# GeekAlexis/FastMOT

Measured on AMD Instinct MI355X. Metric: end-to-end tracker FPS @1080p/50 dets, higher is better.
Workload: dtype f16

## Files before the change

### fastmot_amd/csrc/common.h

```cpp
#pragma once
#include <hip/hip_runtime.h>
#include <atomic>
#include <cstdarg>
#include <cstdint>
#include <cstdio>
#include <cstring>
#include <string>
#include <vector>
#include "../../include/fastmot_hip.h"
#ifdef FM_DIAG
#include "../../include/fastmot_hip_diag.h"
#endif

#define FM_ERR_HIP (-1)
#define FM_ERR_ARG (-2)
#define FM_ERR_STATE (-3)

void fm_set_error(const char* fmt, ...);

#define FM_HIP(call)                                                                        \
    do {                                                                                    \
        hipError_t e_ = (call);                                                             \
        if (e_ != hipSuccess) {                                                             \
            fm_set_error("%s:%d %s -> %s", __FILE__, __LINE__, #call, hipGetErrorString(e_)); \
            return FM_ERR_HIP;                                                              \
        }                                                                                   \
    } while (0)

#define FM_CHECK_ARG(cond)                                                     \
    do {                                                                       \
        if (!(cond)) {                                                         \
            fm_set_error("%s:%d bad argument: %s", __FILE__, __LINE__, #cond); \
            return FM_ERR_ARG;                                                 \
        }                                                                      \
    } while (0)

bool fm_lap_host(const double* cost, int nr, int nc, long rs, long cs, int32_t* col4row_out);
#define FM_ZERO_COPY_TRACKS (ctx->opt_zero_copy_tracks)

struct DevBuf {
    void* d = nullptr;
    void* h = nullptr;
    size_t cap = 0;
    bool pinned_mirror = true;
    int reserve(size_t bytes) {
        if (bytes <= cap) return 0;
        size_t ncap = cap ? cap : 4096;
        while (ncap < bytes) ncap *= 2;
        if (d) (void)hipFree(d);
        if (h) (void)hipHostFree(h);
        d = h = nullptr;
        cap = 0;
        FM_HIP(hipMalloc(&d, ncap));
        if (pinned_mirror) FM_HIP(hipHostMalloc(&h, ncap, hipHostMallocDefault));
        cap = ncap;
        return 0;
    }
    void release() {
        if (d) (void)hipFree(d);
        if (h) (void)hipHostFree(h);
        d = h = nullptr;
        cap = 0;
    }
    template <typename T> T* dev() { return reinterpret_cast<T*>(d); }
    template <typename T> T* host() { return reinterpret_cast<T*>(h); }
};

struct KFConst {
    double F_pos_self;
    double F_pos_other;
    double F_vel;
    double q_pp, q_pv, q_vv;
    double std_factor_acc, std_offset_acc;
    double fac_det[2], fac_klt[2], min_det[2], min_klt[2];
    double init_pos_weight, init_vel_weight;
};

struct NetState;
struct DetState;
struct ExtState;
struct FlowState;
struct EncState;
struct OvlState;
struct YuvState;
struct GalleryState;
constexpr int FM_GALLERY_CHANNELS = 2;

struct fm_ctx {
    int device = 0;
    int opt_zero_copy_tracks = 2048;
    int opt_host_lap_elems = 262144;
    int opt_use_graphs = 1;
    int opt_fused_input = 1;
    int opt_net_timing = 0;
    int opt_nms_general = 0;
    int opt_lk_variant = 0;
    void* predict_worker = nullptr;
    hipStream_t s_main = nullptr;
    hipStream_t s_det = nullptr;
    hipStream_t s_up = nullptr;
    hipStream_t s_ext = nullptr;
    hipStream_t s_ext_x[FM_MAX_EXTRA_EXTRACTORS] = {};
    hipEvent_t ev_ext_in = nullptr, ev_ext_x_done[FM_MAX_EXTRA_EXTRACTORS] = {};
    hipStream_t s_flow = nullptr;
    hipStream_t s_flow2 = nullptr;
    hipEvent_t ev_pyr = nullptr;
    bool pyr_pending = false;
    hipEvent_t ev_prep = nullptr, ev_bg = nullptr;
    hipEvent_t ev_feat = nullptr;
    hipEvent_t ev_ext_net = nullptr;
    hipEvent_t ev_ext_done = nullptr;
    hipEvent_t ev_pair = nullptr;
    bool ext_net_recorded = false;
    size_t as_in_bytes = 0;
    bool as_in_device = true;
    bool as_mirror = false;

    int slot_cap = 0;
    double* mean = nullptr;
    double* cov = nullptr;
    int feat_dim = 512;
    float* feat_sum = nullptr;
    float* feat_avg = nullptr;
    int32_t* feat_cnt = nullptr;
    KFConst kf{};
    bool kf_set = false;
    double frame_rect[4] = {0, 0, 0, 0};

    float* emb = nullptr;
    float* emb_host = nullptr;
    int emb_cap = 0;
    int emb_n = 0;

    int as_nT = 0, as_nD = 0, as_metric = 0;
    size_t as_off[6] = {0, 0, 0, 0, 0, 0};
    DevBuf as_in;
    DevBuf as_pair;
    DevBuf as_stage_in;
    DevBuf as_cost;
    DevBuf as_work;
    DevBuf as_out;
    DevBuf io0, io1;
    DevBuf occ_in, occ_out;
    DevBuf feat_in;

    int frame_w = 0, frame_h = 0, ring_size = 0;
    uint8_t* frame_cur = nullptr;
    uint8_t* frame_own = nullptr;
    uint8_t* frame_own2 = nullptr;
    uint8_t* frame_next = nullptr;
    uint8_t* frame_pinned2 = nullptr;
    hipEvent_t ev_next_upload = nullptr;
    uint8_t* frame_ahead[FM_MAX_DET_BATCH + 1] = {};
    uint8_t* frame_up[FM_MAX_DET_BATCH + 1] = {};
    uint8_t* frame_up_pinned[FM_MAX_DET_BATCH + 1] = {};
    hipEvent_t ev_up[FM_MAX_DET_BATCH + 1] = {};
    uint8_t* frame_ring = nullptr;
    uint8_t* frame_pinned = nullptr;

    DetState* det = nullptr;
    ExtState* ext = nullptr;
    NetState* det_net = nullptr;
    NetState* ext_net = nullptr;
    NetState* ext_net_x[FM_MAX_EXTRA_EXTRACTORS] = {};
    FlowState* flow = nullptr;
    EncState* enc = nullptr;
    OvlState* ovl = nullptr;
    YuvState* yuv = nullptr;
    GalleryState* gallery[2] = {nullptr, nullptr};

    std::vector<hipEvent_t> trace_ev;
    std::vector<int> trace_tag;
    std::atomic<int> trace_n{0};
    std::atomic<bool> trace_on{false};
    std::atomic<int> trace_busy{0};
    hipEvent_t trace_base = nullptr;

    uint8_t* frame_nv12[FM_MAX_DET_BATCH + 2] = {};
    uint8_t* frame_planar[FM_MAX_DET_BATCH + 2] = {};
    uint8_t* frame_packed[FM_MAX_DET_BATCH + 2] = {};
    uint8_t* frame_bayer[FM_MAX_DET_BATCH + 2] = {};

    uint8_t* frame_jpeg[FM_MAX_DET_BATCH + 2] = {};
    uint8_t* frame_jpeg_pinned[FM_MAX_DET_BATCH + 2] = {};
    hipEvent_t ev_jpeg[FM_MAX_DET_BATCH + 2] = {};

    struct SrcStage {
        uint8_t* bgr = nullptr;
        uint8_t* dev = nullptr;
        uint8_t* pinned = nullptr;
        size_t bgr_cap = 0, dev_cap = 0, pinned_cap = 0;
        hipEvent_t ev = nullptr;
    };
    SrcStage frame_src[FM_MAX_DET_BATCH + 2];

    int32_t* remap_xy = nullptr;
    int remap_sw = 0, remap_sh = 0;
    uint32_t remap_border = 0;
};

inline void fm_trace_mark(fm_ctx* ctx, hipStream_t s, int tag) {
    if (!ctx->trace_on.load(std::memory_order_acquire)) return;
    ctx->trace_busy.fetch_add(1);
    if (ctx->trace_on.load()) {
        const int i = ctx->trace_n.fetch_add(1);
        if (i < (int)ctx->trace_ev.size()) {
            ctx->trace_tag[i] = tag;
            (void)hipEventRecord(ctx->trace_ev[i], s);
        }
    }
    ctx->trace_busy.fetch_sub(1);
}

int fm_ensure_slots(fm_ctx* ctx, int max_slot_plus_1);
int fm_nv12_to_bgr(const uint8_t* nv12, uint8_t* bgr, int w, int h, int matrix, hipStream_t s);
inline bool fm_yuv_chroma_dims(int w, int h, int chroma, int* cw, int* ch) {
    switch (chroma) {
    case FM_YUV_420: *cw = (w + 1) / 2, *ch = (h + 1) / 2; return true;
    case FM_YUV_422: *cw = (w + 1) / 2, *ch = h; return true;
    case FM_YUV_444: *cw = w, *ch = h; return true;
    case FM_YUV_MONO: *cw = *ch = 0; return true;
    }
    return false;
}
int fm_planar_to_bgr(const uint8_t* planes, uint8_t* bgr, int w, int h, int chroma, int matrix, hipStream_t s);
inline size_t fm_packed_row_bytes(int w, int format) {
    if (format < FM_PACKED_RGB || format > FM_PACKED_YVYU) return 0;
    if (format >= FM_PACKED_YUY2) return 4 * (size_t)((w + 1) / 2);
    return (size_t)w * (format <= FM_PACKED_BGR ? 3 : 4);
}
inline bool fm_packed_matrix_ok(int matrix) {
    return matrix == FM_PACKED_BT601 || matrix == FM_PACKED_BT709 || matrix == FM_PACKED_BT601_FULL || matrix == FM_PACKED_BT709_FULL;
}
int fm_packed_to_bgr(const uint8_t* src, uint8_t* bgr, int w, int h, int format, int matrix, hipStream_t s);
inline int fm_bayer_sample_bytes(int depth) {
    return depth == 8 ? 1 : depth == 10 || depth == 12 || depth == 14 || depth == 16 ? 2 : 0;
}
inline bool fm_bayer_gain_ok(int gain) { return gain >= 1 && gain <= 4096; }
int fm_bayer_to_bgr(const uint8_t* src, uint8_t* bgr, int w, int h, int pattern, int depth, int method, int black, int gain_r, int gain_g,
                    int gain_b, hipStream_t s);
void fm_yuv_free(fm_ctx* ctx);
int fm_resize_bgr(const uint8_t* src, int sw, int sh, uint8_t* dst, int dw, int dh, hipStream_t s);
int fm_remap_bgr(const uint8_t* src, int sw, int sh, const int32_t* xy, uint8_t* dst, int dw, int dh, uint32_t border, hipStream_t s);
void fm_frame_src_free(fm_ctx* ctx);
void fm_frame_remap_free(fm_ctx* ctx);
int fm_jpeg_to_bgr(const uint8_t* stage, uint8_t* bgr, const struct fm_jpeg_info* info, hipStream_t s);
int fm_jpeg_layout(int width, int height, int ncomp, int hsamp0, int vsamp0, struct fm_jpeg_info* out);
size_t fm_jpeg_sample_offset(long long coef_count);
void fm_ext_invalidate_export(fm_ctx* ctx);
void fm_predict_worker_free(fm_ctx* ctx);
void fm_gallery_free(fm_ctx* ctx);
void fm_jpegenc_free(fm_ctx* ctx);
int fm_jpegenc_ensure(fm_ctx* ctx, int mcus_x, int mcus_y);
hipStream_t fm_jpegenc_stream(fm_ctx* ctx);
int fm_jpegenc_encode_device(fm_ctx* ctx, const uint8_t* src, int width, int height, int quality, uint8_t* out, size_t capacity,
                             size_t* length);
void fm_overlay_free(fm_ctx* ctx);
```

### fastmot_amd/csrc/ctx.hip

```cpp
#include "common.h"
void convd_set_cfg(int code);
#include <sched.h>
#include <cstring>
#include <cstdlib>
#include <cmath>

static thread_local char g_err[1024] = "";

void fm_set_error(const char* fmt, ...) {
    va_list ap;
    va_start(ap, fmt);
    vsnprintf(g_err, sizeof(g_err), fmt, ap);
    va_end(ap);
}

extern "C" const char* fm_last_error(void) { return g_err; }

extern "C" int fm_ctx_set_option(fm_ctx* ctx, const char* key, int value) {
    FM_CHECK_ARG(ctx && key && value >= 0);
    if (!strcmp(key, "zero_copy_tracks")) ctx->opt_zero_copy_tracks = value;
    else if (!strcmp(key, "host_lap_elems")) ctx->opt_host_lap_elems = value;
    else if (!strcmp(key, "use_graphs")) ctx->opt_use_graphs = value;
    else if (!strcmp(key, "convd_cfg")) convd_set_cfg(value);
    else if (!strcmp(key, "nms_path")) {
        ctx->opt_nms_general = value != 0;
    }
    else if (!strcmp(key, "fused_input")) ctx->opt_fused_input = value != 0;
    else if (!strcmp(key, "net_timing")) ctx->opt_net_timing = value;
    else if (!strcmp(key, "lk_variant")) {
#ifndef FM_DIAG
        if (value != 0) {
            fm_set_error("option 'lk_variant' needs a diagnostic build of the library (-DFM_DIAG)");
            return FM_ERR_ARG;
        }
#endif
        ctx->opt_lk_variant = value;
    }
    else {
        fm_set_error("unknown option '%s'", key);
        return FM_ERR_ARG;
    }
    return 0;
}

extern "C" int fm_trace_start(fm_ctx* ctx, int cap, int64_t* host_ns) {
    FM_CHECK_ARG(ctx && cap > 0 && host_ns && !ctx->trace_on.load() && ctx->trace_ev.empty());
    FM_HIP(hipDeviceSynchronize());
    std::vector<hipEvent_t> evs(cap);
    for (auto& e : evs) FM_HIP(hipEventCreate(&e));
    if (!ctx->trace_base) FM_HIP(hipEventCreate(&ctx->trace_base));
    FM_HIP(hipEventRecord(ctx->trace_base, ctx->s_main));
    FM_HIP(hipEventSynchronize(ctx->trace_base));
    timespec ts;
    clock_gettime(CLOCK_MONOTONIC, &ts);
    *host_ns = (int64_t)ts.tv_sec * 1000000000ll + ts.tv_nsec;
    ctx->trace_tag.assign(cap, 0);
    ctx->trace_n = 0;
    ctx->trace_ev = std::move(evs);
    ctx->trace_on.store(true, std::memory_order_release);
    return 0;
}

extern "C" int fm_trace_read(fm_ctx* ctx, int cap, int32_t* tags, float* ms, int* n) {
    FM_CHECK_ARG(ctx && tags && ms && n);
    ctx->trace_on.store(false, std::memory_order_seq_cst);
    while (ctx->trace_busy.load(std::memory_order_seq_cst) > 0) sched_yield();
    FM_HIP(hipDeviceSynchronize());
    std::vector<hipEvent_t> evs = std::move(ctx->trace_ev);
    ctx->trace_ev.clear();
    int k = ctx->trace_n.load();
    if (k > (int)evs.size()) k = (int)evs.size();
    if (k > cap) k = cap;
    for (int i = 0; i < k; ++i) {
        tags[i] = ctx->trace_tag[i];
        FM_HIP(hipEventElapsedTime(&ms[i], ctx->trace_base, evs[i]));
    }
    *n = k;
    for (auto& e : evs) (void)hipEventDestroy(e);
    return 0;
}

extern "C" int fm_ctx_bind_thread(fm_ctx* ctx) {
    FM_CHECK_ARG(ctx);
    FM_HIP(hipSetDevice(ctx->device));
    return 0;
}

extern "C" int fm_device_pci_bus_id(int device, char* buf, int buflen) {
    FM_CHECK_ARG(buf && buflen >= 16);
    FM_HIP(hipDeviceGetPCIBusId(buf, buflen, device));
    return 0;
}

extern "C" int fm_device_count(void) {
    int n = 0;
    FM_HIP(hipGetDeviceCount(&n));
    return n;
}

void fm_net_free(NetState* n);
void fm_det_free(DetState* d);
void fm_ext_free(ExtState* e);
void fm_flow_free(FlowState* f);

extern "C" int fm_ctx_create(int device, fm_ctx** out) {
    FM_CHECK_ARG(out != nullptr);
    int n = 0;
    FM_HIP(hipGetDeviceCount(&n));
    if (device < 0 || device >= n) {
        fm_set_error("device %d out of range (%d visible)", device, n);
        return FM_ERR_ARG;
    }
    FM_HIP(hipSetDevice(device));
    fm_ctx* ctx = new fm_ctx();
    ctx->device = device;
    if (const char* e = getenv("FASTMOT_ZERO_COPY")) ctx->opt_zero_copy_tracks = atoi(e);
    if (const char* e = getenv("FASTMOT_HOST_LAP")) ctx->opt_host_lap_elems = atoi(e);
    if (const char* e = getenv("FASTMOT_GRAPHS")) ctx->opt_use_graphs = atoi(e);
    if (const char* e = getenv("FASTMOT_FUSED_INPUT")) ctx->opt_fused_input = atoi(e) != 0;
    int prio_lo = 0, prio_hi = 0;
    FM_HIP(hipDeviceGetStreamPriorityRange(&prio_lo, &prio_hi));
    const int prio_det = prio_lo, prio_ext = prio_hi;
    FM_HIP(hipStreamCreateWithPriority(&ctx->s_main, hipStreamNonBlocking, prio_hi));
    FM_HIP(hipStreamCreateWithPriority(&ctx->s_det, hipStreamNonBlocking, prio_det));
    FM_HIP(hipStreamCreateWithPriority(&ctx->s_up, hipStreamNonBlocking, prio_lo));
    FM_HIP(hipStreamCreateWithPriority(&ctx->s_ext, hipStreamNonBlocking, prio_ext));
    FM_HIP(hipEventCreateWithFlags(&ctx->ev_ext_in, hipEventDisableTiming));
    for (int i = 0; i < FM_MAX_EXTRA_EXTRACTORS; ++i) {
        FM_HIP(hipStreamCreateWithPriority(&ctx->s_ext_x[i], hipStreamNonBlocking, prio_hi));
        FM_HIP(hipEventCreateWithFlags(&ctx->ev_ext_x_done[i], hipEventDisableTiming));
    }
    FM_HIP(hipStreamCreateWithPriority(&ctx->s_flow, hipStreamNonBlocking, prio_hi));
    FM_HIP(hipStreamCreateWithPriority(&ctx->s_flow2, hipStreamNonBlocking, prio_hi));
    FM_HIP(hipEventCreateWithFlags(&ctx->ev_pyr, hipEventDisableTiming));
    FM_HIP(hipEventCreateWithFlags(&ctx->ev_prep, hipEventDisableTiming));
    FM_HIP(hipEventCreateWithFlags(&ctx->ev_bg, hipEventDisableTiming));
    FM_HIP(hipEventCreateWithFlags(&ctx->ev_feat, hipEventDisableTiming));
    FM_HIP(hipEventCreateWithFlags(&ctx->ev_ext_net, hipEventDisableTiming));
    FM_HIP(hipEventCreateWithFlags(&ctx->ev_pair, hipEventDisableTiming));
    FM_HIP(hipEventCreateWithFlags(&ctx->ev_ext_done, hipEventDisableTiming));
    int rc = fm_ensure_slots(ctx, 1024);
    if (rc) return rc;
    *out = ctx;
    return 0;
}

extern "C" int fm_ctx_destroy(fm_ctx* ctx) {
    if (!ctx) return 0;
    (void)hipSetDevice(ctx->device);
    fm_predict_worker_free(ctx);
    fm_gallery_free(ctx);
    (void)hipDeviceSynchronize();
    if (ctx->det) fm_det_free(ctx->det);
    if (ctx->ext) fm_ext_free(ctx->ext);
    for (void* p : {(void*)ctx->frame_own, (void*)ctx->frame_own2, (void*)ctx->frame_ring})
        if (p) (void)hipFree(p);
    if (ctx->frame_pinned) (void)hipHostFree(ctx->frame_pinned);
    if (ctx->frame_pinned2) (void)hipHostFree(ctx->frame_pinned2);
    for (int k = 2; k <= FM_MAX_DET_BATCH; ++k) {
        if (ctx->frame_up[k]) (void)hipFree(ctx->frame_up[k]);
        if (ctx->frame_up_pinned[k]) (void)hipHostFree(ctx->frame_up_pinned[k]);
        if (ctx->ev_up[k]) (void)hipEventDestroy(ctx->ev_up[k]);
    }
    for (uint8_t* p : ctx->frame_nv12)
        if (p) (void)hipFree(p);
    for (uint8_t* p : ctx->frame_planar)
        if (p) (void)hipFree(p);
    for (uint8_t* p : ctx->frame_packed)
        if (p) (void)hipFree(p);
    for (uint8_t* p : ctx->frame_bayer)
        if (p) (void)hipFree(p);
    for (uint8_t* p : ctx->frame_jpeg)
        if (p) (void)hipFree(p);
    for (uint8_t* p : ctx->frame_jpeg_pinned)
        if (p) (void)hipHostFree(p);
    for (hipEvent_t e : ctx->ev_jpeg)
        if (e) (void)hipEventDestroy(e);
    fm_frame_src_free(ctx);
    fm_frame_remap_free(ctx);
    fm_overlay_free(ctx);
    fm_yuv_free(ctx);
    fm_jpegenc_free(ctx);
    if (ctx->det_net) fm_net_free(ctx->det_net);
    if (ctx->ext_net) fm_net_free(ctx->ext_net);
    for (NetState* x : ctx->ext_net_x)
        if (x) fm_net_free(x);
    if (ctx->flow) fm_flow_free(ctx->flow);
    for (void* p : {(void*)ctx->mean, (void*)ctx->cov, (void*)ctx->feat_sum, (void*)ctx->feat_avg,
                    (void*)ctx->feat_cnt, (void*)ctx->emb})
        if (p) (void)hipFree(p);
    if (ctx->emb_host) (void)hipHostFree(ctx->emb_host);
    for (DevBuf* b : {&ctx->as_in, &ctx->as_pair, &ctx->as_stage_in, &ctx->as_cost, &ctx->as_work,
                      &ctx->as_out, &ctx->io0, &ctx->io1, &ctx->feat_in, &ctx->occ_in, &ctx->occ_out})
        b->release();
    for (hipStream_t s : {ctx->s_main, ctx->s_det, ctx->s_up, ctx->s_ext, ctx->s_flow, ctx->s_flow2})
        if (s) (void)hipStreamDestroy(s);
    for (hipEvent_t e : {ctx->ev_feat, ctx->ev_ext_in, ctx->ev_pyr, ctx->ev_prep, ctx->ev_bg, ctx->ev_ext_net, ctx->ev_pair, ctx->ev_ext_done})
        if (e) (void)hipEventDestroy(e);
    for (int i = 0; i < FM_MAX_EXTRA_EXTRACTORS; ++i) {
        if (ctx->s_ext_x[i]) (void)hipStreamDestroy(ctx->s_ext_x[i]);
        if (ctx->ev_ext_x_done[i]) (void)hipEventDestroy(ctx->ev_ext_x_done[i]);
    }
    delete ctx;
    return 0;
}

extern "C" int fm_ctx_synchronize(fm_ctx* ctx) {
    FM_CHECK_ARG(ctx);
    FM_HIP(hipStreamSynchronize(ctx->s_main));
    FM_HIP(hipStreamSynchronize(ctx->s_det));
    FM_HIP(hipStreamSynchronize(ctx->s_up));
    FM_HIP(hipStreamSynchronize(ctx->s_ext));
    for (hipStream_t x : ctx->s_ext_x) FM_HIP(hipStreamSynchronize(x));
    FM_HIP(hipStreamSynchronize(ctx->s_flow));
    FM_HIP(hipStreamSynchronize(ctx->s_flow2));
    return 0;
}

extern "C" int fm_device_info(fm_ctx* ctx, char* buf, int buflen) {
    FM_CHECK_ARG(ctx && buf && buflen > 0);
    hipDeviceProp_t p;
    FM_HIP(hipGetDeviceProperties(&p, ctx->device));
    snprintf(buf, buflen, "%s:%s:%d:%d:%zu", p.name, p.gcnArchName, p.multiProcessorCount,
             p.clockRate / 1000, (size_t)p.totalGlobalMem);
    return 0;
}

template <typename T>
static int grow(T** ptr, size_t old_elems, size_t new_elems, hipStream_t s, bool zero) {
    T* np_ = nullptr;
    FM_HIP(hipMalloc(&np_, new_elems * sizeof(T)));
    if (zero) FM_HIP(hipMemsetAsync(np_, 0, new_elems * sizeof(T), s));
    if (*ptr && old_elems)
        FM_HIP(hipMemcpyAsync(np_, *ptr, old_elems * sizeof(T), hipMemcpyDeviceToDevice, s));
    FM_HIP(hipStreamSynchronize(s));
    if (*ptr) FM_HIP(hipFree(*ptr));
    *ptr = np_;
    return 0;
}

int fm_ensure_slots(fm_ctx* ctx, int need) {
    if (need <= ctx->slot_cap) return 0;
    int ncap = ctx->slot_cap ? ctx->slot_cap : 1024;
    while (ncap < need) ncap *= 2;
    size_t o = ctx->slot_cap, n = ncap;
    int rc;
    if ((rc = grow(&ctx->mean, o * 8, n * 8, ctx->s_main, true))) return rc;
    if ((rc = grow(&ctx->cov, o * 64, n * 64, ctx->s_main, true))) return rc;
    if ((rc = grow(&ctx->feat_sum, o * ctx->feat_dim, n * ctx->feat_dim, ctx->s_main, true))) return rc;
    if ((rc = grow(&ctx->feat_avg, o * ctx->feat_dim, n * ctx->feat_dim, ctx->s_main, true))) return rc;
    if ((rc = grow(&ctx->feat_cnt, o, n, ctx->s_main, true))) return rc;
    ctx->slot_cap = ncap;
    return 0;
}

extern "C" int fm_kf_configure(fm_ctx* ctx, const fm_kf_params* p) {
    FM_CHECK_ARG(ctx && p);
    FM_CHECK_ARG(p->dt > 0 && p->vel_half_life > 0);
    KFConst& k = ctx->kf;
    const double dt = p->dt;
    k.F_pos_self = p->vel_coupling * dt;
    k.F_pos_other = (1. - p->vel_coupling) * dt;
    k.F_vel = std::pow(0.5, dt / p->vel_half_life);
    k.q_pp = 0.25 * std::pow(dt, 4);
    k.q_pv = 0.5 * std::pow(dt, 3);
    k.q_vv = dt * dt;
    k.std_factor_acc = p->std_factor_acc;
    k.std_offset_acc = p->std_offset_acc;
    for (int i = 0; i < 2; ++i) {
        k.fac_det[i] = p->std_factor_det[i];
        k.fac_klt[i] = p->std_factor_klt[i];
        k.min_det[i] = p->min_std_det[i];
        k.min_klt[i] = p->min_std_klt[i];
    }
    k.init_pos_weight = p->init_pos_weight;
    k.init_vel_weight = p->init_vel_weight;
    ctx->kf_set = true;
    return 0;
}

extern "C" int fm_set_frame_rect(fm_ctx* ctx, const double tlbr[4]) {
    FM_CHECK_ARG(ctx && tlbr);
    memcpy(ctx->frame_rect, tlbr, sizeof(double) * 4);
    return 0;
}

static int max_slot(int n, const int32_t* slots) {
    int m = -1;
    for (int i = 0; i < n; ++i) {
        if (slots[i] < 0) return -2;
        if (slots[i] > m) m = slots[i];
    }
    return m;
}

extern "C" int fm_trk_get_state(fm_ctx* ctx, int n, const int32_t* slots, double* mean, double* cov) {
    FM_CHECK_ARG(ctx && n >= 0);
    if (n == 0) return 0;
    FM_CHECK_ARG(slots && mean && cov);
    int m = max_slot(n, slots);
    FM_CHECK_ARG(m >= 0 && m < ctx->slot_cap);
    FM_HIP(hipStreamSynchronize(ctx->s_main));
    for (int i = 0; i < n; ++i) {
        FM_HIP(hipMemcpy(mean + (size_t)i * 8, ctx->mean + (size_t)slots[i] * 8, 64, hipMemcpyDeviceToHost));
        FM_HIP(hipMemcpy(cov + (size_t)i * 64, ctx->cov + (size_t)slots[i] * 64, 512, hipMemcpyDeviceToHost));
    }
    return 0;
}

extern "C" int fm_trk_set_state(fm_ctx* ctx, int n, const int32_t* slots, const double* mean, const double* cov) {
    FM_CHECK_ARG(ctx && n >= 0);
    if (n == 0) return 0;
    FM_CHECK_ARG(slots && mean && cov);
    int m = max_slot(n, slots);
    FM_CHECK_ARG(m >= 0);
    int rc = fm_ensure_slots(ctx, m + 1);
    if (rc) return rc;
    FM_HIP(hipStreamSynchronize(ctx->s_main));
    for (int i = 0; i < n; ++i) {
        FM_HIP(hipMemcpy(ctx->mean + (size_t)slots[i] * 8, mean + (size_t)i * 8, 64, hipMemcpyHostToDevice));
        FM_HIP(hipMemcpy(ctx->cov + (size_t)slots[i] * 64, cov + (size_t)i * 64, 512, hipMemcpyHostToDevice));
    }
    return 0;
}

extern "C" int fm_trk_copy_state(fm_ctx* ctx, int dst, int src) {
    FM_CHECK_ARG(ctx && dst >= 0 && src >= 0 && src < ctx->slot_cap);
    int rc = fm_ensure_slots(ctx, dst + 1);
    if (rc) return rc;
    FM_HIP(hipMemcpyAsync(ctx->mean + (size_t)dst * 8, ctx->mean + (size_t)src * 8, 64,
                          hipMemcpyDeviceToDevice, ctx->s_main));
    FM_HIP(hipMemcpyAsync(ctx->cov + (size_t)dst * 64, ctx->cov + (size_t)src * 64, 512,
                          hipMemcpyDeviceToDevice, ctx->s_main));
    return 0;
}

void fm_net_drop_graphs(NetState* net);

extern "C" int fm_feat_configure(fm_ctx* ctx, int dim) {
    FM_CHECK_ARG(ctx && dim > 0 && dim % 4 == 0);
    if (dim == ctx->feat_dim) return 0;
    FM_HIP(hipStreamSynchronize(ctx->s_main));
    if (ctx->feat_sum) FM_HIP(hipFree(ctx->feat_sum));
    if (ctx->feat_avg) FM_HIP(hipFree(ctx->feat_avg));
    ctx->feat_sum = ctx->feat_avg = nullptr;
    ctx->feat_dim = dim;
    size_t n = (size_t)ctx->slot_cap * dim;
    FM_HIP(hipMalloc(&ctx->feat_sum, n * sizeof(float)));
    FM_HIP(hipMalloc(&ctx->feat_avg, n * sizeof(float)));
    FM_HIP(hipMemset(ctx->feat_sum, 0, n * sizeof(float)));
    FM_HIP(hipMemset(ctx->feat_avg, 0, n * sizeof(float)));
    FM_HIP(hipMemset(ctx->feat_cnt, 0, (size_t)ctx->slot_cap * sizeof(int32_t)));
    fm_net_drop_graphs(ctx->ext_net);
    for (NetState* x : ctx->ext_net_x) fm_net_drop_graphs(x);
    if (ctx->emb) FM_HIP(hipFree(ctx->emb));
    if (ctx->emb_host) FM_HIP(hipHostFree(ctx->emb_host));
    ctx->emb = ctx->emb_host = nullptr;
    ctx->emb_cap = ctx->emb_n = 0;
    return 0;
}

void fm_net_drop_graphs(NetState* net);

int fm_emb_reserve(fm_ctx* ctx, int n) {
    if (n <= ctx->emb_cap) return 0;
    int ncap = ctx->emb_cap ? ctx->emb_cap : 64;
    while (ncap < n) ncap *= 2;
    fm_net_drop_graphs(ctx->ext_net);
    for (NetState* x : ctx->ext_net_x) fm_net_drop_graphs(x);
    if (ctx->emb) FM_HIP(hipFree(ctx->emb));
    if (ctx->emb_host) FM_HIP(hipHostFree(ctx->emb_host));
    ctx->emb = ctx->emb_host = nullptr;
    ctx->emb_cap = 0;
    FM_HIP(hipMalloc(&ctx->emb, (size_t)ncap * ctx->feat_dim * sizeof(float)));
    FM_HIP(hipHostMalloc(&ctx->emb_host, (size_t)ncap * ctx->feat_dim * sizeof(float), hipHostMallocDefault));
    ctx->emb_cap = ncap;
    return 0;
}

extern "C" int fm_emb_upload(fm_ctx* ctx, int n, const float* emb) {
    FM_CHECK_ARG(ctx && n >= 0);
    if (emb == nullptr) {
        FM_CHECK_ARG(n <= ctx->emb_cap || n == 0);
        ctx->emb_n = n;
        return 0;
    }
    FM_HIP(hipStreamSynchronize(ctx->s_main));
    fm_ext_invalidate_export(ctx);
    ctx->ext_net_recorded = false;
    int rc = fm_emb_reserve(ctx, n);
    if (rc) return rc;
    if (n)
        FM_HIP(hipMemcpyAsync(ctx->emb, emb, (size_t)n * ctx->feat_dim * sizeof(float),
                              hipMemcpyHostToDevice, ctx->s_main));
    ctx->emb_n = n;
    return 0;
}

__global__ void feat_update_kernel(int n, const int32_t* __restrict__ slots,
                                   const int32_t* __restrict__ rows, const float* __restrict__ emb,
                                   float* __restrict__ fsum, float* __restrict__ favg,
                                   int32_t* __restrict__ fcnt, int dim) {
    const int wave = (blockIdx.x * blockDim.x + threadIdx.x) >> 6;
    const int lane = threadIdx.x & 63;
    if (wave >= n) return;
    const int slot = slots[wave];
    const float* v = emb + (size_t)rows[wave] * dim;
    float* s = fsum + (size_t)slot * dim;
    float* a = favg + (size_t)slot * dim;
    const int cnt = fcnt[slot] + 1;
    if (cnt == 1) {
        for (int k = lane; k < dim; k += 64) {
            const float x = v[k];
            s[k] = x;
            a[k] = x;
        }
    } else {
        const float div = (float)(1.0 / (double)cnt);
        float nrm = 0.f;
        for (int k = lane; k < dim; k += 64) {
            const float x = s[k] + v[k];
            s[k] = x;
// ... 134 lines not shown
```

### fastmot_amd/csrc/detect.hip

```cpp
#include "pixel_source.h"
#include "remap_pixel.h"
#include <cmath>
#include <mutex>
#include <utility>

struct DetState {
    fm_yolo_cfg cfg{};
    bool configured = false;
    int cap = 8192;
    static constexpr int NSLOT = FM_MAX_DET_BATCH + 2;
    float* cand[NSLOT] = {};
    float* sorted[NSLOT] = {};
    int32_t* counters[NSLOT] = {};
    uint64_t* mask[NSLOT] = {};
    fm_det48* dets[NSLOT] = {};
    bool used[NSLOT] = {};
    hipEvent_t ev_dec[NSLOT] = {};
    int post_pending = -1;
    int post_pending_n = 0;
    bool general_post = false;
    static constexpr int GREEDY_RETRY = 1024;
    int general_passes = 0;
    int greedy_kmax = 2048, greedy_shrink = 0;
    bool sorted_valid[NSLOT] = {};
// ... 1582 lines not shown
    fm_trace_mark(ctx, cs, 30);
    int rc = enqueue_planar(ctx, k, buf, f, ahead_pinned(ctx, k), ev, cs, false);
    if (rc) return rc;
    fm_trace_mark(ctx, cs, 31);
    if (!ev) FM_HIP(hipEventCreateWithFlags(&ev, hipEventDisableTiming));
    FM_HIP(hipEventRecord(ev, cs));
    if (ctx->det && (rc = flush_post(ctx, ctx->det))) return rc;
    ahead_frame(ctx, k) = buf;
    return 0;
}

extern "C" int fm_frame_ring_store_planar(fm_ctx* ctx, int index, const struct fm_frame_planar* f) {
    FM_CHECK_ARG(ctx && index >= 0 && index < ctx->ring_size && planar_ok(f));
    FM_CHECK_ARG(remap_takes(ctx, f->width, f->height));
    int rc = enqueue_planar(ctx, FM_MAX_DET_BATCH + 1, ctx->frame_ring + (size_t)ctx->frame_w * ctx->frame_h * 3 * index, f, nullptr,
                            nullptr, nullptr, true);
    if (rc) return rc;
    FM_HIP(hipStreamSynchronize(nullptr));
    return 0;
}

static bool packed_ok(const struct fm_frame_packed* f) {
    if (!f || f->width < 1 || f->height < 1 || f->width > FM_SRC_MAX_DIM || f->height > FM_SRC_MAX_DIM) return false;
    const size_t rb = fm_packed_row_bytes(f->width, f->format);
    return rb && fm_packed_matrix_ok(f->matrix) && f->data && f->pitch > 0 && (size_t)f->pitch >= rb;
}

static int enqueue_packed(fm_ctx* ctx, int entry, uint8_t* dst, const struct fm_frame_packed* f, hipStream_t s, bool blocking) {
    const int w = f->width, h = f->height;
    const size_t rb = fm_packed_row_bytes(w, f->format), total = rb * h, npx = (size_t)w * h;
    const bool on_size = src_on_size(ctx, w, h);
    fm_ctx::SrcStage& st = ctx->frame_src[entry];
    uint8_t* stage = nullptr;
    int rc;
    if (on_size) {
        uint8_t*& p = ctx->frame_packed[entry];
        if (!p) FM_HIP(hipMalloc(&p, npx * 4));
        stage = p;
    } else {
        if ((rc = src_reserve(st.bgr, st.bgr_cap, npx * 3 + FM_FRAME_SLACK, false, s))) return rc;
        if ((rc = src_reserve(st.dev, st.dev_cap, total, false, s))) return rc;
        stage = st.dev;
    }
    if (blocking) {
        FM_HIP(hipMemcpy2D(stage, rb, f->data, f->pitch, rb, h, hipMemcpyHostToDevice));
    } else if ((size_t)f->pitch == rb && is_pinned_range(f->data, total)) {
        FM_HIP(hipMemcpyAsync(stage, f->data, total, hipMemcpyHostToDevice, s));
    } else {
        if ((rc = src_pinned(st, total, s))) return rc;
        for (int r = 0; r < h; ++r) memcpy(st.pinned + (size_t)r * rb, f->data + (size_t)r * f->pitch, rb);
        FM_HIP(hipMemcpyAsync(stage, st.pinned, total, hipMemcpyHostToDevice, s));
        if ((rc = src_pinned_copied(st, s))) return rc;
    }
    fm_trace_mark(ctx, s, 48);
    if (on_size) return fm_packed_to_bgr(stage, dst, w, h, f->format, f->matrix, s);
    if ((rc = fm_packed_to_bgr(stage, st.bgr, w, h, f->format, f->matrix, s))) return rc;
    return enqueue_src_tail(ctx, st.bgr, w, h, dst, s);
}

extern "C" int fm_frame_upload_packed(fm_ctx* ctx, const struct fm_frame_packed* f) {
    FM_CHECK_ARG(ctx && ctx->frame_own && packed_ok(f));
    FM_CHECK_ARG(remap_takes(ctx, f->width, f->height));
    FM_HIP(hipStreamSynchronize(ctx->s_det));
    FM_HIP(hipStreamSynchronize(ctx->s_ext));
    FM_HIP(hipStreamSynchronize(ctx->s_flow));
    FM_HIP(hipStreamSynchronize(ctx->s_flow2));
    int rc = enqueue_packed(ctx, 0, ctx->frame_own, f, ctx->s_det, false);
    if (rc) return rc;
    FM_HIP(hipStreamSynchronize(ctx->s_det));
    ctx->frame_cur = ctx->frame_own;
    return 0;
}

extern "C" int fm_frame_upload_ahead_packed(fm_ctx* ctx, int k, const struct fm_frame_packed* f) {
    FM_CHECK_ARG(ctx && ctx->frame_own2 && k >= 1 && k <= FM_MAX_DET_BATCH && packed_ok(f));
    FM_CHECK_ARG(remap_takes(ctx, f->width, f->height));
    const size_t bytes = (size_t)ctx->frame_w * ctx->frame_h * 3;
    if (!ahead_buf(ctx, k)) {
        FM_HIP(hipMalloc(&ahead_buf(ctx, k), bytes + FM_FRAME_SLACK));
        FM_HIP(hipHostMalloc(&ahead_pinned(ctx, k), bytes, hipHostMallocDefault));
    }
    uint8_t* const buf = ahead_buf(ctx, k);
    hipEvent_t& ev = ahead_event(ctx, k);
    hipStream_t cs = ctx->s_ext;
    fm_trace_mark(ctx, cs, 30);
    int rc = enqueue_packed(ctx, k, buf, f, cs, false);
    if (rc) return rc;
    fm_trace_mark(ctx, cs, 31);
    if (!ev) FM_HIP(hipEventCreateWithFlags(&ev, hipEventDisableTiming));
    FM_HIP(hipEventRecord(ev, cs));
    if (ctx->det && (rc = flush_post(ctx, ctx->det))) return rc;
    ahead_frame(ctx, k) = buf;
    return 0;
}

extern "C" int fm_frame_ring_store_packed(fm_ctx* ctx, int index, const struct fm_frame_packed* f) {
    FM_CHECK_ARG(ctx && index >= 0 && index < ctx->ring_size && packed_ok(f));
    FM_CHECK_ARG(remap_takes(ctx, f->width, f->height));
    int rc = enqueue_packed(ctx, FM_MAX_DET_BATCH + 1, ctx->frame_ring + (size_t)ctx->frame_w * ctx->frame_h * 3 * index, f, nullptr, true);
    if (rc) return rc;
    FM_HIP(hipStreamSynchronize(nullptr));
    return 0;
}

static bool bayer_ok(const struct fm_frame_bayer* f) {
    if (!f || f->width < 2 || f->height < 2 || f->width > FM_SRC_MAX_DIM || f->height > FM_SRC_MAX_DIM) return false;
    const int bps = fm_bayer_sample_bytes(f->depth);
    if (!bps || f->pattern < FM_BAYER_RGGB || f->pattern > FM_BAYER_BGGR) return false;
    if (f->method != FM_BAYER_BILINEAR && f->method != FM_BAYER_MHC) return false;
    if (f->black < 0 || f->black >= (1 << f->depth)) return false;
    if (!fm_bayer_gain_ok(f->gain_r) || !fm_bayer_gain_ok(f->gain_g) || !fm_bayer_gain_ok(f->gain_b)) return false;
    return f->data && f->pitch > 0 && (size_t)f->pitch >= (size_t)f->width * bps;
}

static int enqueue_bayer(fm_ctx* ctx, int entry, uint8_t* dst, const struct fm_frame_bayer* f, hipStream_t s, bool blocking) {
    const int w = f->width, h = f->height;
    const size_t rb = (size_t)w * fm_bayer_sample_bytes(f->depth), total = rb * h, npx = (size_t)w * h;
    const bool on_size = src_on_size(ctx, w, h);
    fm_ctx::SrcStage& st = ctx->frame_src[entry];
    uint8_t* stage = nullptr;
    int rc;
    if (on_size) {
        uint8_t*& p = ctx->frame_bayer[entry];
        if (!p) FM_HIP(hipMalloc(&p, npx * 2));
        stage = p;
    } else {
        if ((rc = src_reserve(st.bgr, st.bgr_cap, npx * 3 + FM_FRAME_SLACK, false, s))) return rc;
        if ((rc = src_reserve(st.dev, st.dev_cap, total, false, s))) return rc;
        stage = st.dev;
    }
    if (blocking) {
        FM_HIP(hipMemcpy2D(stage, rb, f->data, f->pitch, rb, h, hipMemcpyHostToDevice));
    } else if ((size_t)f->pitch == rb && is_pinned_range(f->data, total)) {
        FM_HIP(hipMemcpyAsync(stage, f->data, total, hipMemcpyHostToDevice, s));
    } else {
        if ((rc = src_pinned(st, total, s))) return rc;
        for (int r = 0; r < h; ++r) memcpy(st.pinned + (size_t)r * rb, f->data + (size_t)r * f->pitch, rb);
        FM_HIP(hipMemcpyAsync(stage, st.pinned, total, hipMemcpyHostToDevice, s));
        if ((rc = src_pinned_copied(st, s))) return rc;
    }
    fm_trace_mark(ctx, s, 49);
    uint8_t* const out = on_size ? dst : st.bgr;
    if ((rc = fm_bayer_to_bgr(stage, out, w, h, f->pattern, f->depth, f->method, f->black, f->gain_r, f->gain_g, f->gain_b, s))) return rc;
    if (on_size) return 0;
    return enqueue_src_tail(ctx, st.bgr, w, h, dst, s);
}

extern "C" int fm_frame_upload_bayer(fm_ctx* ctx, const struct fm_frame_bayer* f) {
    FM_CHECK_ARG(ctx && ctx->frame_own && bayer_ok(f));
    FM_CHECK_ARG(remap_takes(ctx, f->width, f->height));
    FM_HIP(hipStreamSynchronize(ctx->s_det));
    FM_HIP(hipStreamSynchronize(ctx->s_ext));
    FM_HIP(hipStreamSynchronize(ctx->s_flow));
    FM_HIP(hipStreamSynchronize(ctx->s_flow2));
    int rc = enqueue_bayer(ctx, 0, ctx->frame_own, f, ctx->s_det, false);
    if (rc) return rc;
    FM_HIP(hipStreamSynchronize(ctx->s_det));
    ctx->frame_cur = ctx->frame_own;
    return 0;
}

extern "C" int fm_frame_upload_ahead_bayer(fm_ctx* ctx, int k, const struct fm_frame_bayer* f) {
    FM_CHECK_ARG(ctx && ctx->frame_own2 && k >= 1 && k <= FM_MAX_DET_BATCH && bayer_ok(f));
    FM_CHECK_ARG(remap_takes(ctx, f->width, f->height));
    const size_t bytes = (size_t)ctx->frame_w * ctx->frame_h * 3;
    if (!ahead_buf(ctx, k)) {
        FM_HIP(hipMalloc(&ahead_buf(ctx, k), bytes + FM_FRAME_SLACK));
        FM_HIP(hipHostMalloc(&ahead_pinned(ctx, k), bytes, hipHostMallocDefault));
    }
    uint8_t* const buf = ahead_buf(ctx, k);
    hipEvent_t& ev = ahead_event(ctx, k);
    hipStream_t cs = ctx->s_ext;
    fm_trace_mark(ctx, cs, 30);
    int rc = enqueue_bayer(ctx, k, buf, f, cs, false);
    if (rc) return rc;
    fm_trace_mark(ctx, cs, 31);
    if (!ev) FM_HIP(hipEventCreateWithFlags(&ev, hipEventDisableTiming));
    FM_HIP(hipEventRecord(ev, cs));
    if (ctx->det && (rc = flush_post(ctx, ctx->det))) return rc;
    ahead_frame(ctx, k) = buf;
    return 0;
}

extern "C" int fm_frame_ring_store_bayer(fm_ctx* ctx, int index, const struct fm_frame_bayer* f) {
    FM_CHECK_ARG(ctx && index >= 0 && index < ctx->ring_size && bayer_ok(f));
    FM_CHECK_ARG(remap_takes(ctx, f->width, f->height));
    int rc = enqueue_bayer(ctx, FM_MAX_DET_BATCH + 1, ctx->frame_ring + (size_t)ctx->frame_w * ctx->frame_h * 3 * index, f, nullptr, true);
    if (rc) return rc;
    FM_HIP(hipStreamSynchronize(nullptr));
    return 0;
}

extern "C" int fm_detect_configure(fm_ctx* ctx, const fm_yolo_cfg* cfg) {
    FM_CHECK_ARG(ctx && cfg);
    FM_CHECK_ARG(cfg->n_heads >= 0 && cfg->n_heads <= FM_MAX_HEADS && cfg->num_classes > 0 && cfg->num_classes <= 128);
    {
        long long rows = 0;
        for (int i = 0; i < cfg->n_heads; ++i) {
            FM_CHECK_ARG(cfg->n_anchors[i] > 0 && cfg->n_anchors[i] <= FM_MAX_ANCHORS && cfg->grid_w[i] > 0 && cfg->grid_h[i] > 0);
            rows += (long long)cfg->grid_w[i] * cfg->grid_h[i] * cfg->n_anchors[i];
        }
        FM_CHECK_ARG(rows < (1ll << FM_SORT_INDEX_BITS));
    }
    int rc = ensure_det(ctx);
    if (rc) return rc;
    DetState* d = ctx->det;
    FM_HIP(hipStreamSynchronize(ctx->s_det));
    FM_HIP(hipStreamSynchronize(ctx->s_up));
    d->post_pending = -1;
    d->post_pending_n = 0;
    d->rd = d->wr;
    d->pending = 0;
    d->cfg = *cfg;
    d->general_post = ctx->opt_nms_general != 0;
    if ((rc = alloc_post(d, cfg->max_candidates > 0 ? cfg->max_candidates : 8192))) return rc;
    FM_HIP(hipMemcpy(d->label_mask, cfg->label_mask, 128, hipMemcpyHostToDevice));
    d->configured = true;
    return 0;
}

static StemSrc det_source(fm_ctx* ctx, DetState* d, const uint8_t* const* frames, int n) {
    const fm_yolo_cfg& c = d->cfg;
    StemSrc src{};
    src.kind = 1; src.fw = ctx->frame_w; src.fh = ctx->frame_h;
    src.roi_x = c.roi_x; src.roi_y = c.roi_y; src.roi_w = c.roi_w; src.roi_h = c.roi_h;
    for (int i = 0; i < n; ++i) {
        src.frame[i] = frames[i];
        src.zero4[i] = d->counters[(d->wr + i) % DetState::NSLOT];
    }
    return src;
}

static int enqueue_preprocess(fm_ctx* ctx, DetState* d, NetState* net, const StemSrc& src, int n) {
    const fm_yolo_cfg& c = d->cfg;
    for (int i = 0; i < n; ++i) FM_CHECK_ARG(src.frame[i] != nullptr);
    FM_CHECK_ARG(c.input_tensor >= 0 && c.input_tensor < (int)net->tensors.size());
    const fm_tensor& t = net->tensors[c.input_tensor];
    FM_CHECK_ARG(t.h == c.in_h && t.w == c.in_w && !t.f32);
    hipLaunchKernelGGL(preprocess_kernel, dim3((c.in_w + 255) / 256, c.in_h, n), dim3(256), 0, ctx->s_det,
                       src, (f16*)net->bufs[c.input_tensor], c.in_w, c.in_h, t.c);
    FM_HIP(hipGetLastError());
    return 0;
}

extern "C" int fm_detect_preprocess_only(fm_ctx* ctx) {
    FM_CHECK_ARG(ctx && ctx->det && ctx->det->configured && ctx->det_net);
    const uint8_t* f = ctx->frame_cur;
    return enqueue_preprocess(ctx, ctx->det, ctx->det_net, det_source(ctx, ctx->det, &f, 1), 1);
}

static int detect_pass(fm_ctx* ctx, const uint8_t* const* frames, const hipEvent_t* uploads, int n);

extern "C" int fm_detect_async(fm_ctx* ctx) {
    FM_CHECK_ARG(ctx);
    const uint8_t* f = ctx->frame_cur;
    const hipEvent_t none = nullptr;
    return detect_pass(ctx, &f, &none, 1);
}

extern "C" int fm_detect_async_next(fm_ctx* ctx) {
    FM_CHECK_ARG(ctx && ctx->frame_next);
    return fm_detect_async_ahead(ctx, 1);
}

extern "C" int fm_detect_async_ahead(fm_ctx* ctx, int n) {
    FM_CHECK_ARG(ctx && ctx->det_net && n >= 1 && n <= FM_MAX_DET_BATCH);
    if (n > ctx->det_net->max_batch) {
        fm_set_error("detector look-ahead of %d frames > the detector network's max_batch %d", n, ctx->det_net->max_batch);
        return FM_ERR_ARG;
    }
    const uint8_t* frames[FM_MAX_DET_BATCH];
    hipEvent_t uploads[FM_MAX_DET_BATCH];
    for (int k = 1; k <= n; ++k) {
        frames[k - 1] = ahead_frame(ctx, k);
        if (!frames[k - 1]) {
            fm_set_error("look-ahead slot %d holds no frame (fm_frame_upload_ahead / fm_frame_ring_select_ahead)", k);
            return FM_ERR_ARG;
        }
        uploads[k - 1] = frames[k - 1] == ahead_buf(ctx, k) ? ahead_event(ctx, k) : nullptr;
    }
    return detect_pass(ctx, frames, uploads, n);
}

static int detect_pass(fm_ctx* ctx, const uint8_t* const* frames, const hipEvent_t* uploads, int n) {
    FM_CHECK_ARG(ctx && ctx->det && ctx->det->configured && ctx->det_net);
    DetState* d = ctx->det;
    NetState* net = ctx->det_net;
    const fm_yolo_cfg& c = d->cfg;
    FM_CHECK_ARG(n >= 1 && n <= FM_MAX_DET_BATCH && n <= net->max_batch);
    hipStream_t s = ctx->s_det;
    fm_trace_mark(ctx, s, 10);
    for (int i = 0; i < n; ++i)
        if (uploads[i]) FM_HIP(hipStreamWaitEvent(s, uploads[i], 0));
    int rc = acquire_slots(ctx, d, s, n);
    if (rc) return rc;
    fm_trace_mark(ctx, s, 14);
    const StemSrc src = det_source(ctx, d, frames, n);
    const bool fused = ctx->opt_fused_input && fm_net_stem_fusable(net, c.input_tensor);
    const bool timing = ctx->opt_net_timing > 0 && d->n_passes++ % ctx->opt_net_timing == 0;
    for (int i = 0; i < n; ++i) d->timed[(d->wr + i) % DetState::NSLOT] = timing && i == 0;
    if (fused) {
        if (timing) FM_HIP(hipEventRecord(d->ev0[d->wr], s));
        fm_trace_mark(ctx, s, 11);
        if ((rc = fm_net_run_stem_from(ctx, net, src, n))) return rc;
        fm_trace_mark(ctx, s, 15);
        net->first = 1;
        rc = fm_net_run_internal(ctx, FM_NET_DETECTOR, n);
        net->first = 0;
        if (rc) return rc;
    } else {
        if ((rc = enqueue_preprocess(ctx, d, net, src, n))) return rc;
        if (timing) FM_HIP(hipEventRecord(d->ev0[d->wr], s));
        fm_trace_mark(ctx, s, 11);
        if ((rc = fm_net_run_internal(ctx, FM_NET_DETECTOR, n))) return rc;
    }
    if (timing) FM_HIP(hipEventRecord(d->ev1[d->wr], s));
    fm_trace_mark(ctx, s, 12);
    FilterArgs fa = filter_args(d, d->wr);
    HeadSet hs{};
    for (int i = 0; i < n; ++i) {
        const int slot = (d->wr + i) % DetState::NSLOT;
        hs.cand[i] = d->cand[slot];
        hs.counters[i] = d->counters[slot];
    }
    int base = 0, blocks = 0;
    for (int i = 0; i < FM_MAX_HEADS + 1; ++i) hs.first_block[i] = 0x7fffffff;
    for (int i = 0; i < c.n_heads; ++i) {
        FM_CHECK_ARG(c.head_tensor[i] >= 0 && c.head_tensor[i] < (int)net->tensors.size());
        const fm_tensor& t = net->tensors[c.head_tensor[i]];
        FM_CHECK_ARG(t.f32 && t.h == c.grid_h[i] && t.w == c.grid_w[i] && c.n_anchors[i] <= FM_MAX_ANCHORS);
        HeadArgs& h = hs.h[i];
        h.data = (const float*)net->bufs[c.head_tensor[i]];
        h.cs = t.c; h.gw = c.grid_w[i]; h.gh = c.grid_h[i]; h.na = c.n_anchors[i];
        h.base_index = base;
        memcpy(h.anchors, c.anchors[i], sizeof(float) * 2 * FM_MAX_ANCHORS);
        h.scale_xy = c.scale_xy[i];
        const int cnt = h.gw * h.gh * h.na;
        hs.first_block[i] = blocks;
        blocks += (cnt + 255) / 256;
        base += cnt;
    }
    if (blocks) hipLaunchKernelGGL(decode_kernel, dim3(blocks, n), dim3(256), 0, s, hs, fa, c.in_w, c.in_h, c.new_coords);
    FM_HIP(hipGetLastError());
    fm_trace_mark(ctx, s, 13);
    return enqueue_post(ctx, d, s, n);
}

extern "C" int fm_detect_sync(fm_ctx* ctx, fm_det48* out, int cap, int* n) {
    FM_CHECK_ARG(ctx && ctx->det && ctx->det->configured && out && n);
    return collect(ctx, ctx->det, ctx->s_det, out, cap, n);
}

extern "C" int fm_filter_dets(fm_ctx* ctx, const float* rows, int n, fm_det48* out, int cap, int* n_out) {
    FM_CHECK_ARG(ctx && ctx->det && ctx->det->configured && n >= 0 && out && n_out);
    FM_CHECK_ARG(n < (1 << FM_SORT_INDEX_BITS));
    DetState* d = ctx->det;
    hipStream_t s = ctx->s_det;
    FM_HIP(hipStreamSynchronize(s));
    FM_HIP(hipStreamSynchronize(ctx->s_up));
    d->post_pending = -1;
    d->post_pending_n = 0;
    d->rd = d->wr;
    d->pending = 0;
    if (n > d->rows_cap) {
        if (d->rows_in) FM_HIP(hipFree(d->rows_in));
        d->rows_in = nullptr;
        FM_HIP(hipMalloc(&d->rows_in, sizeof(float) * 7 * (size_t)n));
        d->rows_cap = n;
    }
    if (n) FM_HIP(hipMemcpyAsync(d->rows_in, rows, sizeof(float) * 7 * (size_t)n, hipMemcpyHostToDevice, s));
    FM_HIP(hipMemsetAsync(d->counters[d->wr], 0, sizeof(int32_t) * 4, s));
    if (n) hipLaunchKernelGGL(rows_filter_kernel, dim3((n + 255) / 256), dim3(256), 0, s, d->rows_in, n, filter_args(d, d->wr));
    int rc = enqueue_post(ctx, d, s);
    if (rc) return rc;
    return collect(ctx, d, s, out, cap, n_out);
}

extern "C" int fm_detect_last_counts(fm_ctx* ctx, int* n_candidates, int* n_detections) {
    FM_CHECK_ARG(ctx && ctx->det && n_candidates && n_detections);
    const DetState* d = ctx->det;
    if (d->last < 0) {
        *n_candidates = *n_detections = 0;
        return 0;
    }
    *n_candidates = d->counters_host[d->last][0];
    *n_detections = d->counters_host[d->last][2];
    return 0;
}

extern "C" int fm_detect_raw_candidates(fm_ctx* ctx, float* rows, int cap, int* n) {
    FM_CHECK_ARG(ctx && ctx->det && rows && n);
    DetState* d = ctx->det;
    int rc_f = flush_post(ctx, d);
    if (rc_f) return rc_f;
    FM_HIP(hipStreamSynchronize(ctx->s_det));
    FM_HIP(hipStreamSynchronize(ctx->s_up));
    const int slot = (d->wr + DetState::NSLOT - 1) % DetState::NSLOT;
    int32_t cnt[4];
    FM_HIP(hipMemcpy(cnt, d->counters[slot], sizeof(cnt), hipMemcpyDeviceToHost));
    const int k = cnt[0] < d->cap ? cnt[0] : d->cap;
    FM_CHECK_ARG(k <= cap);
    FM_HIP(hipMemcpy(rows, d->sorted[slot], sizeof(float) * 8 * k, hipMemcpyDeviceToHost));
    *n = k;
    return 0;
}

extern "C" int fm_detect_net_ms(fm_ctx* ctx, float* ms) {
    FM_CHECK_ARG(ctx && ctx->det && ms && ctx->det->last >= 0);
    const int slot = ctx->det->last;
    if (!ctx->det->timed[slot]) { *ms = -1.f; return 0; }
    FM_HIP(hipEventSynchronize(ctx->det->ev1[slot]));
    FM_HIP(hipEventElapsedTime(ms, ctx->det->ev0[slot], ctx->det->ev1[slot]));
    return 0;
}
```

### fastmot_amd/csrc/extract.hip

```cpp
#include "pixel_source.h"
#include <cmath>

struct ExtState {
    int input_tensor = -1, in_w = 0, in_h = 0;
    double* boxes = nullptr;
    double* boxes_host = nullptr;
    int cap = 0;
    DevBuf emb_out;
    int exported_n = -1;
    bool mirror_export = false;
};

void fm_ext_invalidate_export(fm_ctx* ctx) {
    if (ctx->ext) ctx->ext->exported_n = -1;
}

void fm_ext_free(ExtState* e) {
    if (!e) return;
    e->emb_out.release();
    if (e->boxes) (void)hipFree(e->boxes);
    if (e->boxes_host) (void)hipHostFree(e->boxes_host);
    delete e;
}

namespace {

__global__ __launch_bounds__(256) void export_kernel(const float4* __restrict__ src, float4* __restrict__ dst, int n4) {
    for (int i = blockIdx.x * 256 + threadIdx.x; i < n4; i += gridDim.x * 256) dst[i] = src[i];
}

__global__ void crop_resize_kernel(const uint8_t* __restrict__ frame, int fw, int fh,
                                   const double* __restrict__ boxes, int n, f16* __restrict__ out,
                                   int ow, int oh, int cs) {
    const int x = blockIdx.x * blockDim.x + threadIdx.x;
    const int y = blockIdx.y, b = blockIdx.z;
    if (x >= ow) return;
    f16x8 o;
    crop_input_pixel(frame, fw, fh, boxes + (size_t)b * 4, x, y, ow, oh, o);
    *reinterpret_cast<f16x8*>(out + (((size_t)b * oh + y) * ow + x) * cs) = o;
}

}

extern "C" int fm_extract_configure(fm_ctx* ctx, int input_tensor, int in_w, int in_h) {
    FM_CHECK_ARG(ctx && ctx->ext_net && input_tensor >= 0 && input_tensor < (int)ctx->ext_net->tensors.size());
    const fm_tensor& t = ctx->ext_net->tensors[input_tensor];
    FM_CHECK_ARG(t.h == in_h && t.w == in_w && !t.f32);
    if (!ctx->ext) ctx->ext = new ExtState();
    ctx->ext->input_tensor = input_tensor;
    ctx->ext->in_w = in_w;
    ctx->ext->in_h = in_h;
    return 0;
}

int fm_emb_reserve(fm_ctx* ctx, int n);

static int export_embeddings(fm_ctx* ctx, ExtState* e, int n, hipStream_t s) {
    const size_t bytes = sizeof(float) * (size_t)n * ctx->feat_dim;
    e->exported_n = -1;
    if (ctx->emb_host) {
        e->exported_n = n;
        e->mirror_export = true;
        FM_HIP(hipEventRecord(ctx->ev_ext_done, s));
        return 0;
    }
    e->mirror_export = false;
    if (bytes > e->emb_out.cap) {
        FM_HIP(hipStreamSynchronize(s));
        int rc = e->emb_out.reserve(bytes);
        if (rc) return rc;
    }
    const int n4 = (int)(bytes / 16);
    hipLaunchKernelGGL(export_kernel, dim3((n4 + 255) / 256 < 64 ? (n4 + 255) / 256 : 64), dim3(256), 0, s,
                       (const float4*)ctx->emb, (float4*)e->emb_out.h, n4);
    FM_HIP(hipGetLastError());
    e->exported_n = n;
    FM_HIP(hipEventRecord(ctx->ev_ext_done, s));
    return 0;
}

static int front_end(fm_ctx* ctx, ExtState* e, NetState* ni, hipStream_t si, int off, int b, int cs) {
    ni->first = 0;
    if (ctx->opt_fused_input && fm_net_stem_fusable(ni, e->input_tensor)) {
        StemSrc src{};
        src.kind = 2; src.frame[0] = ctx->frame_cur; src.fw = ctx->frame_w; src.fh = ctx->frame_h;
        src.boxes = e->boxes_host + (size_t)off * 4;
        int rc = fm_net_run_stem_from(ctx, ni, src, b);
        if (rc) return rc;
        ni->first = 1;
        return 0;
    }
    hipLaunchKernelGGL(crop_resize_kernel, dim3((e->in_w + 127) / 128, e->in_h, b), dim3(128), 0, si,
                       ctx->frame_cur, ctx->frame_w, ctx->frame_h, e->boxes + (size_t)off * 4, b,
                       (f16*)ni->bufs[e->input_tensor], e->in_w, e->in_h, cs);
    FM_HIP(hipGetLastError());
    return 0;
}

extern "C" int fm_extract_async(fm_ctx* ctx, int n, const double* tlbr) {
    FM_CHECK_ARG(ctx && ctx->ext && ctx->ext_net && n >= 0 && ctx->frame_cur);
    ctx->emb_n = 0;
    ctx->ext_net_recorded = false;
    int rc_exp = 0;
    if (ctx->ext) ctx->ext->exported_n = -1;
    if (n == 0) return 0;
    FM_CHECK_ARG(tlbr);
    ExtState* e = ctx->ext;
    NetState* net = ctx->ext_net;
    hipStream_t s = ctx->s_ext;
    if (n > e->cap) {
        FM_HIP(hipStreamSynchronize(s));
        if (e->boxes) FM_HIP(hipFree(e->boxes));
        if (e->boxes_host) FM_HIP(hipHostFree(e->boxes_host));
        e->boxes = e->boxes_host = nullptr;
        int cap = e->cap ? e->cap : 64;
        while (cap < n) cap *= 2;
        FM_HIP(hipMalloc(&e->boxes, sizeof(double) * 4 * cap));
        FM_HIP(hipHostMalloc(&e->boxes_host, sizeof(double) * 4 * cap, hipHostMallocDefault));
        e->cap = cap;
    }
    if (hipEventQuery(ctx->ev_feat) != hipSuccess) {
        (void)hipGetLastError();
        FM_HIP(hipStreamWaitEvent(s, ctx->ev_feat, 0));
    }
    if (n > ctx->emb_cap) {
        FM_HIP(hipStreamSynchronize(ctx->s_main));
        FM_HIP(hipStreamSynchronize(s));
        int rc = fm_emb_reserve(ctx, n);
        if (rc) return rc;
    }
    FM_HIP(hipStreamSynchronize(s));
    memcpy(e->boxes_host, tlbr, sizeof(double) * 4 * n);
    const bool zero_copy_boxes = ctx->opt_fused_input && fm_net_stem_fusable(net, e->input_tensor);
    if (!zero_copy_boxes)
        FM_HIP(hipMemcpyAsync(e->boxes, e->boxes_host, sizeof(double) * 4 * n, hipMemcpyHostToDevice, s));
    fm_trace_mark(ctx, s, 32);
    const fm_tensor& t = net->tensors[e->input_tensor];
    int parts = 1;
    while (parts <= FM_MAX_EXTRA_EXTRACTORS && ctx->ext_net_x[parts - 1]) ++parts;
    while (parts > 1 && n < 4 * parts) --parts;
    if (parts > 1 && (n + parts - 1) / parts <= net->max_batch) {
        FM_HIP(hipEventRecord(ctx->ev_ext_in, s));
        int off = 0;
        for (int i = 0; i < parts; ++i) {
            const int b = n / parts + (i < n % parts ? 1 : 0);
            NetState* ni = i == 0 ? net : ctx->ext_net_x[i - 1];
            hipStream_t si = i == 0 ? s : ctx->s_ext_x[i - 1];
            FM_CHECK_ARG(b <= ni->max_batch);
            if (i) FM_HIP(hipStreamWaitEvent(si, ctx->ev_ext_in, 0));
            int rc = front_end(ctx, e, ni, si, off, b, t.c);
            if (rc) return rc;
            ni->emb_offset = off;
            rc = fm_net_run_internal(ctx, i == 0 ? FM_NET_EXTRACTOR : FM_NET_EXTRACTOR_B + i - 1, b);
            ni->emb_offset = 0;
            ni->first = 0;
            if (rc) return rc;
            if (i) {
                FM_HIP(hipEventRecord(ctx->ev_ext_x_done[i - 1], si));
                FM_HIP(hipStreamWaitEvent(s, ctx->ev_ext_x_done[i - 1], 0));
            }
            off += b;
        }
        FM_HIP(hipEventRecord(ctx->ev_ext_net, s));
        ctx->ext_net_recorded = true;
        if ((rc_exp = export_embeddings(ctx, e, n, s))) return rc_exp;
        fm_trace_mark(ctx, s, 33);
        ctx->emb_n = n;
        return 0;
    }
    for (int off = 0; off < n; off += net->max_batch) {
        const int b = n - off < net->max_batch ? n - off : net->max_batch;
        int rc = front_end(ctx, e, net, s, off, b, t.c);
        if (rc) return rc;
        fm_trace_mark(ctx, s, 34);
        net->emb_offset = off;
        rc = fm_net_run_internal(ctx, FM_NET_EXTRACTOR, b);
        net->emb_offset = 0;
        net->first = 0;
        if (rc) return rc;
    }
    fm_trace_mark(ctx, s, 35);
    FM_HIP(hipEventRecord(ctx->ev_ext_net, s));
    ctx->ext_net_recorded = true;
    if ((rc_exp = export_embeddings(ctx, e, n, s))) return rc_exp;
    fm_trace_mark(ctx, s, 33);
    ctx->emb_n = n;
    return 0;
}

extern "C" int fm_extract_sync(fm_ctx* ctx, int n, float* emb) {
    FM_CHECK_ARG(ctx && n >= 0 && n <= ctx->emb_cap);
    if (n == 0) {
        FM_HIP(hipStreamSynchronize(ctx->s_ext));
        return 0;
    }
    FM_CHECK_ARG(emb && ctx->ext);
    const size_t bytes = sizeof(float) * (size_t)n * ctx->feat_dim;
    if (ctx->ext->exported_n != n) {
        int rc = ctx->ext->emb_out.reserve(bytes);
        if (rc) return rc;
        FM_HIP(hipMemcpyAsync(ctx->ext->emb_out.h, ctx->emb, bytes, hipMemcpyDeviceToHost, ctx->s_ext));
        FM_HIP(hipStreamSynchronize(ctx->s_ext));
    } else {
        FM_HIP(hipEventSynchronize(ctx->ev_ext_done));
        if (ctx->ext->mirror_export) {
            memcpy(emb, ctx->emb_host, bytes);
            return 0;
        }
    }
    memcpy(emb, ctx->ext->emb_out.h, bytes);
    return 0;
}

extern "C" int fm_extract_read_input(fm_ctx* ctx, int n, float* out) {
    FM_CHECK_ARG(ctx && ctx->ext && ctx->ext_net && n > 0 && n <= ctx->ext_net->max_batch && out);
    ExtState* e = ctx->ext;
    NetState* net = ctx->ext_net;
    const fm_tensor& t = net->tensors[e->input_tensor];
    if (ctx->opt_fused_input && fm_net_stem_fusable(net, e->input_tensor)) {
        FM_CHECK_ARG(ctx->frame_cur && n <= e->cap);
        hipLaunchKernelGGL(crop_resize_kernel, dim3((e->in_w + 127) / 128, e->in_h, n), dim3(128), 0, ctx->s_ext,
                           ctx->frame_cur, ctx->frame_w, ctx->frame_h, e->boxes_host, n, (f16*)net->bufs[e->input_tensor],
                           e->in_w, e->in_h, t.c);
        FM_HIP(hipGetLastError());
    }
    FM_HIP(hipStreamSynchronize(ctx->s_ext));
    std::vector<f16> tmp((size_t)n * t.h * t.w * t.c);
    FM_HIP(hipMemcpy(tmp.data(), net->bufs[e->input_tensor], tmp.size() * 2, hipMemcpyDeviceToHost));
    for (size_t p = 0; p < (size_t)n * t.h * t.w; ++p)
        for (int c = 0; c < 3; ++c) out[p * 3 + c] = (float)tmp[p * t.c + c];
    return 0;
}
```

### fastmot_amd/csrc/net.h

```cpp
#pragma once
#include "common.h"
#include <hip/hip_fp16.h>

typedef _Float16 f16;
typedef f16 f16x8 __attribute__((ext_vector_type(8)));
typedef f16 f16x4 __attribute__((ext_vector_type(4)));
typedef float f32x16 __attribute__((ext_vector_type(16)));
typedef float f32x4 __attribute__((ext_vector_type(4)));

enum { ACT_LINEAR = 0, ACT_LEAKY = 1, ACT_MISH = 2, ACT_RELU = 3, ACT_LOGISTIC = 4, ACT_SWISH = 5 };
enum { RES_NONE = 0, RES_AFTER_ACT = 1, RES_BEFORE_ACT = 2 };

struct ConvParams {
    const f16* in;  int in_cs, in_coff;
    const f16* w;
    const float* bias;
    f16* out;       int out_cs, out_coff;
    float* out32;
    const f16* res; int res_cs, res_coff;
    int N, H, W, Cin, Ho, Wo, Cout, KH, KW, stride, pad;
    int K, Kpad, P;
    int cout_store;
    int act, res_mode;
    int grid_p, grid_c, grid_z, weight_major;
    int up;
    int batch_inv;
};

int launch_conv(const ConvParams& p, float* ws, size_t ws_floats, hipStream_t s);

struct NetState {
    int which = 0, max_batch = 0;
    std::vector<fm_tensor> tensors;
    std::vector<void*> bufs;
    std::vector<fm_layer> layers;
    char* weights = nullptr;
    size_t weight_bytes = 0;
    float* gates = nullptr;
    int n_gates = 0, gate_c = 0;
    hipStream_t stream = nullptr;
    char* arena = nullptr;
    float* ws = nullptr;
    size_t ws_floats = 0;
    std::vector<std::pair<long, hipGraphExec_t>> graphs;
    bool use_graphs = true;
    int emb_offset = 0;
    int batch_offset = 0;
    int first = 0;
};

NetState* fm_net_get(fm_ctx* ctx, int which);
int fm_net_run_internal(fm_ctx* ctx, int which, int batch);

__device__ __forceinline__ void unpack8(const uint4& v, float* f) {
    const f16x8 h = *reinterpret_cast<const f16x8*>(&v);
#pragma unroll
    for (int e = 0; e < 8; ++e) f[e] = (float)h[e];
}
__device__ __forceinline__ uint4 pack8(const float* f) {
    f16x8 h;
#pragma unroll
    for (int e = 0; e < 8; ++e) h[e] = (f16)f[e];
    return *reinterpret_cast<const uint4*>(&h);
}

__device__ __forceinline__ int idiv_small(int i, int d, float inv) {
    (void)d;
    return (int)(((float)i + 0.5f) * inv);
}

template <int HI>
__device__ __forceinline__ float fma_mix_h(uint32_t packed, float k, float acc) {
    float d;
    if constexpr (HI) asm("v_fma_mix_f32 %0, %1, %2, %3 op_sel:[1,0,0] op_sel_hi:[1,0,0]" : "=v"(d) : "v"(packed), "v"(k), "v"(acc));
    else asm("v_fma_mix_f32 %0, %1, %2, %3 op_sel:[0,0,0] op_sel_hi:[1,0,0]" : "=v"(d) : "v"(packed), "v"(k), "v"(acc));
    return d;
}
template <int HI>
__device__ __forceinline__ float fma_mix_hh(uint32_t packed, uint32_t kpacked, float acc) {
    float d;
    if constexpr (HI) asm("v_fma_mix_f32 %0, %1, %2, %3 op_sel:[1,1,0] op_sel_hi:[1,1,0]" : "=v"(d) : "v"(packed), "v"(kpacked), "v"(acc));
    else asm("v_fma_mix_f32 %0, %1, %2, %3 op_sel:[0,0,0] op_sel_hi:[1,1,0]" : "=v"(d) : "v"(packed), "v"(kpacked), "v"(acc));
    return d;
}
template <int N>
__device__ __forceinline__ void fma_mix_nh(const uint32_t* raw, const uint32_t* k, float* acc) {
#pragma unroll
    for (int e = 0; e < N; e += 2) {
        acc[e] = fma_mix_hh<0>(raw[e >> 1], k[e >> 1], acc[e]);
        acc[e + 1] = fma_mix_hh<1>(raw[e >> 1], k[e >> 1], acc[e + 1]);
    }
}
template <int N>
__device__ __forceinline__ void fma_mix_n(const uint32_t* raw, const float* k, float* acc) {
#pragma unroll
    for (int e = 0; e < N; e += 2) {
        acc[e] = fma_mix_h<0>(raw[e >> 1], k[e], acc[e]);
        acc[e + 1] = fma_mix_h<1>(raw[e >> 1], k[e + 1], acc[e + 1]);
    }
}

__device__ __forceinline__ void store_out(const ConvParams& p, long pix, int co, f16x4 o) {
    if (p.up == 2) {
        const int hw = p.Ho * p.Wo, rem = (int)(pix % hw);
        const size_t o00 = ((size_t)(pix / hw) * 2 * p.Ho + 2 * (rem / p.Wo)) * (2 * p.Wo) + 2 * (rem % p.Wo);
        f16* dst = p.out + o00 * p.out_cs + p.out_coff + co;
        *reinterpret_cast<f16x4*>(dst) = o;
        *reinterpret_cast<f16x4*>(dst + p.out_cs) = o;
        *reinterpret_cast<f16x4*>(dst + (size_t)2 * p.Wo * p.out_cs) = o;
        *reinterpret_cast<f16x4*>(dst + (size_t)(2 * p.Wo + 1) * p.out_cs) = o;
    } else {
        *reinterpret_cast<f16x4*>(p.out + (size_t)pix * p.out_cs + p.out_coff + co) = o;
    }
}

__device__ __forceinline__ float act_rcp(float x) { return __builtin_amdgcn_rcpf(x); }
__device__ __forceinline__ float act_leaky(float x) { return x > 0.f ? x : 0.1f * x; }
__device__ __forceinline__ float act_relu(float x) { return x > 0.f ? x : 0.f; }
__device__ __forceinline__ float act_mish(float x) {
    const float n = __expf(x);
    const float t = n * (n + 2.f);
    return x > 20.f ? x : x * (t * act_rcp(t + 2.f));
}
__device__ __forceinline__ float act_logistic(float x) { return act_rcp(1.f + __expf(-x)); }
__device__ __forceinline__ float act_swish(float x) { return x * act_rcp(1.f + __expf(-x)); }

__device__ __forceinline__ float apply_act(float x, int act) {
    switch (act) {
        case ACT_LEAKY: return act_leaky(x);
        case ACT_MISH: return act_mish(x);
        case ACT_RELU: return act_relu(x);
        case ACT_LOGISTIC: return act_logistic(x);
        case ACT_SWISH: return act_swish(x);
        default: return x;
    }
}

template <int N>
__device__ __forceinline__ void apply_act_n(float* v, int act) {
    switch (act) {
        case ACT_LEAKY:
#pragma unroll
            for (int e = 0; e < N; ++e) v[e] = act_leaky(v[e]);
            break;
        case ACT_MISH:
#pragma unroll
            for (int e = 0; e < N; ++e) v[e] = act_mish(v[e]);
            break;
        case ACT_RELU:
#pragma unroll
            for (int e = 0; e < N; ++e) v[e] = act_relu(v[e]);
            break;
        case ACT_LOGISTIC:
#pragma unroll
            for (int e = 0; e < N; ++e) v[e] = act_logistic(v[e]);
            break;
        case ACT_SWISH:
#pragma unroll
            for (int e = 0; e < N; ++e) v[e] = act_swish(v[e]);
            break;
        default: break;
    }
}
```

### fastmot_amd/csrc/net.hip

```cpp
#include "pixel_source.h"
#include <algorithm>
#include <memory>

int launch_dwconv3(const f16* in, int in_cs, int in_coff, f16* out, int out_cs, int out_coff, const f16* w,
                   const float* bias, int N, int H, int W, int C, int act, hipStream_t s);
int launch_liteconv(int G, const f16* const* in, const int* in_cs, const int* in_coff, f16* out, int out_cs,
                    int out_coff, const f16* wpw, int kpad, const f16* wdw, const float* bias, int N, int H,
                    int W, int C, int act, float* gap_out, hipStream_t s);
void liteconv_tiling(int C, int W, int H, int* th, int* tw, int* tiles_x, int* tiles_y);
int launch_litechain(const f16* in, int in_cs, int in_coff, f16* out, int out_cs, int out_coff, const f16* wpw,
                     int kpad, const f16* wdw, const float* bias, int N, int H, int W, int C, int act,
                     float* const* gap, hipStream_t s);
int launch_gated_sum(int nstreams, const f16* const* in, const int* in_cs, const int* in_coff, int N, int HW,
                     int C, int hid, const f16* w1, const float* b1, const f16* w2, const float* b2, f16* out,
                     int out_cs, int out_coff, const float* const* part, int tiles, hipStream_t s);
constexpr int GATE_SLOT_TILES = 32;
int launch_pair11(const f16* xa, int xa_cs, int xa_coff, const f16* xc, int xc_cs, int xc_coff, f16* out, int out_cs,
                  int out_coff, const f16* w1, const float* b1, const f16* w2, const float* b2, long P, int cout, int act1,
                  int act2, hipStream_t s, long p_choice);
bool pair11_supported(int cin, int mid, int extra, int cout);
int launch_ostail(const f16* in, int in_cs, int in_coff, const f16* ph, const float* pf, int N, float* out, float* raw_out,
                  float* mirror, hipStream_t s);
bool ostail_supported(int in_h, int in_w, int cin, int mid, int cout, int feat, int n_halfs, int n_floats);
int launch_stemconv(const f16* in, int in_cs, int in_coff, f16* out, int out_cs, int out_coff, const f16* w,
                    const float* bias, int N, int H, int W, int Ho, int Wo, int k, int stride, int pad, int cout,
                    int act, hipStream_t s);
int launch_spp(const f16* in, int in_cs, int in_coff, f16* out, int out_cs, int out_coff, int N, int H, int W,
               int C, hipStream_t s);
int launch_pool(const f16* in, int in_cs, int in_coff, f16* out, int out_cs, int out_coff, int N, int H,
                int W, int C, int Ho, int Wo, int k, int stride, int pad, int avg, hipStream_t s);
int launch_upsample2(const f16* in, int in_cs, int in_coff, f16* out, int out_cs, int out_coff, int N, int H,
                     int W, int C, hipStream_t s);
int launch_conv_streamed(const ConvParams& p, hipStream_t s);
int launch_convd(const ConvParams& p, hipStream_t s);
bool resblock_supported(int C, int M);
int launch_resblock(const f16* x, int x_cs, int x_coff, f16* out, int out_cs, int out_coff, const f16* w1,
                    const float* b1, const f16* w2, const float* b2, int N, int H, int W, int C, int M, int act1,
                    int act2, hipStream_t s);
int launch_add(const f16* a, int a_cs, int a_coff, const f16* b, int b_cs, int b_coff, f16* out, int out_cs,
               int out_coff, long npix, int C, hipStream_t s);
int launch_copy(const f16* in, int in_cs, int in_coff, f16* out, int out_cs, int out_coff, long npix, int C,
                hipStream_t s);
int launch_gate(const f16* in, int in_cs, int in_coff, int N, int HW, int C, int hid, const f16* w1,
                const float* b1, const f16* w2, const float* b2, float* gate, hipStream_t s);
int launch_gate_sum(int nstreams, const f16* const* in, const int* in_cs, const int* in_coff,
                    const float* const* gate, f16* out, int out_cs, int out_coff, int N, int HW, int C,
                    hipStream_t s);
int launch_head(const f16* in, int in_cs, int in_coff, int N, int HW, int C, int D, const f16* w,
                const float* b, float* out, float* raw_out, hipStream_t s, float* mirror = nullptr);
int fm_emb_reserve(fm_ctx* ctx, int n);


void fm_net_free(NetState* n) {
    if (!n) return;
    for (size_t i = 0; i < n->bufs.size(); ++i)
        if (n->bufs[i] && n->tensors[i].offset < 0) (void)hipFree(n->bufs[i]);
    if (n->arena) (void)hipFree(n->arena);
    if (n->weights) (void)hipFree(n->weights);
    if (n->gates) (void)hipFree(n->gates);
    if (n->ws) (void)hipFree(n->ws);
    for (auto& g : n->graphs) (void)hipGraphExecDestroy(g.second);
    delete n;
}

static NetState*& net_slot(fm_ctx* ctx, int which) {
    return which == FM_NET_DETECTOR ? ctx->det_net : which == FM_NET_EXTRACTOR ? ctx->ext_net
                                                    : ctx->ext_net_x[which - FM_NET_EXTRACTOR_B];
}
NetState* fm_net_get(fm_ctx* ctx, int which) { return net_slot(ctx, which); }
int fm_net_run_internal(fm_ctx* ctx, int which, int batch) { return fm_net_run(ctx, which, batch); }

void fm_net_drop_graphs(NetState* net) {
    if (!net) return;
    (void)hipStreamSynchronize(net->stream);
    for (auto& g : net->graphs) (void)hipGraphExecDestroy(g.second);
    net->graphs.clear();
}

static size_t elem_size(const fm_tensor& t) { return t.f32 ? 4 : 2; }

extern "C" int fm_net_destroy(fm_ctx* ctx, int which) {
    FM_CHECK_ARG(ctx && (which >= 0 && which < FM_NET_EXTRACTOR_B + FM_MAX_EXTRA_EXTRACTORS));
    NetState*& slot = net_slot(ctx, which);
    if (slot) {
        FM_HIP(hipStreamSynchronize(slot->stream));
        fm_net_free(slot);
        slot = nullptr;
    }
    return 0;
}

extern "C" int fm_net_create(fm_ctx* ctx, int which, int max_batch, int n_tensors, const fm_tensor* tensors,
                             int n_layers, const fm_layer* layers, const void* weights, size_t weight_bytes,
                             int n_gates, int gate_channels, size_t arena_bytes) {
    FM_CHECK_ARG(ctx && (which >= 0 && which < FM_NET_EXTRACTOR_B + FM_MAX_EXTRA_EXTRACTORS) && max_batch > 0 && n_tensors > 0 && n_layers > 0);
    FM_CHECK_ARG(tensors && layers && weights && weight_bytes > 0);
    int rc = fm_net_destroy(ctx, which);
    if (rc) return rc;
    std::unique_ptr<NetState, void (*)(NetState*)> net(new NetState(), fm_net_free);
    net->which = which;
    net->max_batch = max_batch;
    net->stream = which == FM_NET_DETECTOR ? ctx->s_det : which == FM_NET_EXTRACTOR ? ctx->s_ext
                                                        : ctx->s_ext_x[which - FM_NET_EXTRACTOR_B];
    net->tensors.assign(tensors, tensors + n_tensors);
    net->layers.assign(layers, layers + n_layers);
    if (arena_bytes) {
        FM_HIP(hipMalloc(&net->arena, arena_bytes));
        FM_HIP(hipMemset(net->arena, 0, arena_bytes));
    }
    for (const fm_tensor& t : net->tensors) {
        FM_CHECK_ARG(t.h > 0 && t.w > 0 && t.c > 0 && t.c % 8 == 0);
        void* b = nullptr;
        const size_t bytes = (size_t)max_batch * t.h * t.w * t.c * elem_size(t);
        if (t.offset >= 0) {
            FM_CHECK_ARG(t.offset % 256 == 0 && (size_t)t.offset + bytes <= arena_bytes);
            b = net->arena + t.offset;
        } else {
            FM_HIP(hipMalloc(&b, bytes));
            FM_HIP(hipMemset(b, 0, bytes));
        }
        net->bufs.push_back(b);
    }
    for (const fm_layer& L : net->layers) {
        FM_CHECK_ARG(L.out >= 0 && L.out < n_tensors && L.n_in >= 1 && L.n_in <= 4);
        for (int i = 0; i < L.n_in; ++i) FM_CHECK_ARG(L.in[i] >= 0 && L.in[i] < n_tensors);
        FM_CHECK_ARG(L.res_mode == FM_RES_NONE || (L.res >= 0 && L.res < n_tensors));
        FM_CHECK_ARG(L.w_off >= 0 && (size_t)L.w_off <= weight_bytes && L.w_off % 16 == 0 && L.b_off % 16 == 0);
        if (L.op == FM_OP_OSTAIL)
            FM_CHECK_ARG(L.stride > 0 && L.pad > 0 && L.b_off >= 0 && (size_t)L.w_off + (size_t)L.stride * 2 <= weight_bytes &&
                         (size_t)L.b_off + (size_t)L.pad * 4 <= weight_bytes);
    }
    FM_HIP(hipMalloc(&net->weights, weight_bytes));
    FM_HIP(hipMemcpy(net->weights, weights, weight_bytes, hipMemcpyHostToDevice));
    net->weight_bytes = weight_bytes;
    net->n_gates = n_gates;
    net->gate_c = gate_channels;
    net->ws_floats = ((size_t)16 << 20) * (which == FM_NET_DETECTOR ? (size_t)std::min(max_batch, FM_MAX_DET_BATCH) : 1);
    FM_HIP(hipMalloc(&net->ws, net->ws_floats * sizeof(float)));
    if (n_gates > 0) {
        FM_CHECK_ARG(gate_channels > 0);
        FM_HIP(hipMalloc(&net->gates, sizeof(float) * (size_t)n_gates * max_batch * gate_channels * GATE_SLOT_TILES));
    }
    if (which != FM_NET_DETECTOR) {
        FM_HIP(hipStreamSynchronize(ctx->s_main));
        if ((rc = fm_emb_reserve(ctx, max_batch))) return rc;
    }
    net_slot(ctx, which) = net.release();
    return 0;
}

static int run_layer(fm_ctx* ctx, NetState* net, const fm_layer& L, int B) {
    const fm_tensor& ti = net->tensors[L.in[0]];
    const fm_tensor& to = net->tensors[L.out];
    hipStream_t s = net->stream;
    float* ws = net->ws;
    const f16* in0 = (const f16*)net->bufs[L.in[0]];
    f16* out = (f16*)net->bufs[L.out];
    switch (L.op) {
        case FM_OP_CONV:
        case FM_OP_CONVS:
        case FM_OP_CONVD: {
            ConvParams p{};
            p.in = in0; p.in_cs = ti.c; p.in_coff = L.in_coff[0];
            p.w = (const f16*)(net->weights + L.w_off);
            p.bias = (const float*)(net->weights + L.b_off);
            p.out = to.f32 ? nullptr : out;
            p.out32 = to.f32 ? (float*)net->bufs[L.out] : nullptr;
            p.out_cs = to.c; p.out_coff = L.out_coff;
            if (L.res_mode != FM_RES_NONE) {
                p.res = (const f16*)net->bufs[L.res];
                p.res_cs = net->tensors[L.res].c;
                p.res_coff = L.res_coff;
            }
            p.up = L.up == 2 ? 2 : 1;
            FM_CHECK_ARG(L.up <= 2 && (p.up == 1 || (!to.f32 && to.h % 2 == 0 && to.w % 2 == 0)));
            p.N = B; p.H = ti.h; p.W = ti.w; p.Cin = L.cin; p.Ho = to.h / p.up; p.Wo = to.w / p.up; p.Cout = L.cout;
            p.KH = p.KW = L.k; p.stride = L.stride; p.pad = L.pad;
            p.K = L.k * L.k * L.cin; p.Kpad = (p.K + 63) & ~63; p.P = B * p.Ho * p.Wo;
            p.cout_store = (L.cout + 7) & ~7;
            p.act = L.act; p.res_mode = L.res_mode;
            p.batch_inv = net->which == FM_NET_DETECTOR ? 1 : 0;
            FM_CHECK_ARG((ti.h + 2 * L.pad - L.k) / L.stride + 1 == p.Ho);
            FM_CHECK_ARG(L.out_coff + p.cout_store <= to.c && L.in_coff[0] + L.cin <= ti.c);
            if (L.op == FM_OP_CONVS) return launch_conv_streamed(p, s);
            if (L.op == FM_OP_CONVD) return launch_convd(p, s);
            return launch_conv(p, ws, net->ws_floats, s);
        }
        case FM_OP_DWCONV3:
            return launch_dwconv3(in0, ti.c, L.in_coff[0], out, to.c, L.out_coff,
                                  (const f16*)(net->weights + L.w_off), (const float*)(net->weights + L.b_off),
                                  B, ti.h, ti.w, L.cin, L.act, s);
        case FM_OP_LITECONV: {
            FM_CHECK_ARG(L.cin == ((L.cout + 7) & ~7) && L.n_in >= 1 && L.n_in <= 4);
            FM_CHECK_ARG(L.out_coff + L.n_in * L.cin <= to.c);
            const f16* ins[4];
            int cs[4], co[4];
            for (int i = 0; i < L.n_in; ++i) {
                const fm_tensor& tg = net->tensors[L.in[i]];
                FM_CHECK_ARG(tg.h == to.h && tg.w == to.w && L.in_coff[i] + L.cin <= tg.c);
                ins[i] = (const f16*)net->bufs[L.in[i]];
                cs[i] = tg.c;
                co[i] = L.in_coff[i];
            }
            float* gap_out = nullptr;
            if (L.gate[0] >= 0) {
                int th, tw, tx, ty;
                liteconv_tiling(L.cin, ti.w, ti.h, &th, &tw, &tx, &ty);
                FM_CHECK_ARG(L.gate[0] < net->n_gates && L.cin <= net->gate_c && tx * ty <= GATE_SLOT_TILES);
                gap_out = net->gates + (size_t)L.gate[0] * net->max_batch * net->gate_c * GATE_SLOT_TILES;
            }
            return launch_liteconv(L.n_in, ins, cs, co, out, to.c, L.out_coff,
                                   (const f16*)(net->weights + L.w_off), (L.cin + 63) & ~63,
                                   (const f16*)(net->weights + L.w2_off), (const float*)(net->weights + L.b_off),
                                   B, ti.h, ti.w, L.cin, L.act, gap_out, s);
        }
        case FM_OP_LITECHAIN: {
            FM_CHECK_ARG(L.cin == ((L.cout + 7) & ~7) && to.h == ti.h && to.w == ti.w && L.in_coff[0] + L.cin <= ti.c &&
                         L.out_coff + 4 * L.cin <= to.c);
            int th, tw, tx, ty;
            liteconv_tiling(L.cin, ti.w, ti.h, &th, &tw, &tx, &ty);
            FM_CHECK_ARG(L.cin <= net->gate_c && tx * ty <= GATE_SLOT_TILES);
            float* gaps[4];
            for (int i = 0; i < 4; ++i) {
                FM_CHECK_ARG(L.gate[i] >= 0 && L.gate[i] < net->n_gates);
                gaps[i] = net->gates + (size_t)L.gate[i] * net->max_batch * net->gate_c * GATE_SLOT_TILES;
            }
            return launch_litechain(in0, ti.c, L.in_coff[0], out, to.c, L.out_coff,
                                    (const f16*)(net->weights + L.w_off), (L.cin + 63) & ~63,
                                    (const f16*)(net->weights + L.w2_off), (const float*)(net->weights + L.b_off),
                                    B, ti.h, ti.w, L.cin, L.act, gaps, s);
        }
        case FM_OP_GATED_SUM: {
            const f16* ins[4];
            int cs[4], co[4];
            FM_CHECK_ARG(L.n_in >= 1 && L.n_in <= 4);
            for (int i = 0; i < L.n_in; ++i) {
                ins[i] = (const f16*)net->bufs[L.in[i]];
                cs[i] = net->tensors[L.in[i]].c;
                co[i] = L.in_coff[i];
            }
            const float* parts[4] = {nullptr, nullptr, nullptr, nullptr};
            int tiles = 0;
            if (L.gate[0] >= 0) {
                int th, tw, tx, ty;
                liteconv_tiling(L.cin, ti.w, ti.h, &th, &tw, &tx, &ty);
                tiles = tx * ty;
                for (int i = 0; i < L.n_in; ++i) {
                    FM_CHECK_ARG(L.gate[i] >= 0 && L.gate[i] < net->n_gates);
                    parts[i] = net->gates + (size_t)L.gate[i] * net->max_batch * net->gate_c * GATE_SLOT_TILES;
                }
            }
            return launch_gated_sum(L.n_in, ins, cs, co, B, ti.h * ti.w, L.cin, L.hid,
                                    (const f16*)(net->weights + L.w_off), (const float*)(net->weights + L.b_off),
                                    (const f16*)(net->weights + L.w2_off), (const float*)(net->weights + L.b2_off),
                                    out, to.c, L.out_coff, L.gate[0] >= 0 ? parts : nullptr, tiles, s);
        }
        case FM_OP_STEMCONV:
            FM_CHECK_ARG(!to.f32 && (ti.h + 2 * L.pad - L.k) / L.stride + 1 == to.h &&
                         (ti.w + 2 * L.pad - L.k) / L.stride + 1 == to.w && L.out_coff + ((L.cout + 7) & ~7) <= to.c);
            return launch_stemconv(in0, ti.c, L.in_coff[0], out, to.c, L.out_coff,
                                   (const f16*)(net->weights + L.w_off), (const float*)(net->weights + L.b_off),
                                   B, ti.h, ti.w, to.h, to.w, L.k, L.stride, L.pad, L.cout, L.act, s);
        case FM_OP_PAIR11: {
            FM_CHECK_ARG(L.n_in == 2 && !to.f32 && pair11_supported(L.cin, L.hid, L.cin, L.cout));
            const fm_tensor& tc = net->tensors[L.in[1]];
            FM_CHECK_ARG(tc.h == ti.h && tc.w == ti.w && to.h == ti.h && to.w == ti.w && L.in_coff[0] + 64 <= ti.c &&
                         L.in_coff[1] + 64 <= tc.c && L.out_coff + L.cout <= to.c);
            return launch_pair11(in0, ti.c, L.in_coff[0], (const f16*)net->bufs[L.in[1]], tc.c, L.in_coff[1], out, to.c, L.out_coff,
                                 (const f16*)(net->weights + L.w_off), (const float*)(net->weights + L.b_off),
                                 (const f16*)(net->weights + L.w2_off), (const float*)(net->weights + L.b2_off),
                                 (long)B * ti.h * ti.w, L.cout, L.gate[0], L.act, s,
                                 net->which == FM_NET_DETECTOR ? (long)ti.h * ti.w : (long)B * ti.h * ti.w);
        }
        case FM_OP_STEM2:
            return launch_stem2_layer(L, StemSrc{}, net, B, s);
        case FM_OP_SPP:
            FM_CHECK_ARG(to.h == ti.h && to.w == ti.w && L.out_coff + 3 * L.cin <= to.c);
            return launch_spp(in0, ti.c, L.in_coff[0], out, to.c, L.out_coff, B, ti.h, ti.w, L.cin, s);
        case FM_OP_MAXPOOL:
        case FM_OP_AVGPOOL:
            return launch_pool(in0, ti.c, L.in_coff[0], out, to.c, L.out_coff, B, ti.h, ti.w, L.cin, to.h, to.w,
                               L.k, L.stride, L.pad, L.op == FM_OP_AVGPOOL, s);
        case FM_OP_UPSAMPLE2:
            FM_CHECK_ARG(to.h == 2 * ti.h && to.w == 2 * ti.w);
            return launch_upsample2(in0, ti.c, L.in_coff[0], out, to.c, L.out_coff, B, ti.h, ti.w, L.cin, s);
        case FM_OP_RESBLOCK:
            FM_CHECK_ARG(!to.f32 && to.h == ti.h && to.w == ti.w && L.cin == L.cout &&
                         L.in_coff[0] + L.cin <= ti.c && L.out_coff + L.cout <= to.c);
            return launch_resblock(in0, ti.c, L.in_coff[0], out, to.c, L.out_coff,
                                   (const f16*)(net->weights + L.w_off), (const float*)(net->weights + L.b_off),
                                   (const f16*)(net->weights + L.w2_off), (const float*)(net->weights + L.b2_off),
                                   B, ti.h, ti.w, L.cin, L.hid, L.act, L.act, s);
        case FM_OP_ADD: {
            FM_CHECK_ARG(L.n_in == 2);
            const fm_tensor& tb = net->tensors[L.in[1]];
            FM_CHECK_ARG(tb.h == ti.h && tb.w == ti.w && to.h == ti.h && to.w == ti.w);
            return launch_add(in0, ti.c, L.in_coff[0], (const f16*)net->bufs[L.in[1]], tb.c, L.in_coff[1], out, to.c,
                              L.out_coff, (long)B * ti.h * ti.w, L.cin, s);
        }
        case FM_OP_COPY:
            return launch_copy(in0, ti.c, L.in_coff[0], out, to.c, L.out_coff, (long)B * ti.h * ti.w, L.cin, s);
        case FM_OP_GATE:
            FM_CHECK_ARG(L.gate[0] >= 0 && L.gate[0] < net->n_gates && L.cin <= net->gate_c);
            return launch_gate(in0, ti.c, L.in_coff[0], B, ti.h * ti.w, L.cin, L.hid,
                               (const f16*)(net->weights + L.w_off), (const float*)(net->weights + L.b_off),
                               (const f16*)(net->weights + L.w2_off), (const float*)(net->weights + L.b2_off),
                               net->gates + (size_t)L.gate[0] * net->max_batch * net->gate_c * GATE_SLOT_TILES, s);
        case FM_OP_GATE_SUM: {
            const f16* ins[4];
            int cs[4], co[4];
            const float* gs[4];
            for (int i = 0; i < L.n_in; ++i) {
                ins[i] = (const f16*)net->bufs[L.in[i]];
                cs[i] = net->tensors[L.in[i]].c;
                co[i] = L.in_coff[i];
                FM_CHECK_ARG(L.gate[i] >= 0 && L.gate[i] < net->n_gates);
                gs[i] = net->gates + (size_t)L.gate[i] * net->max_batch * net->gate_c * GATE_SLOT_TILES;
            }
            return launch_gate_sum(L.n_in, ins, cs, co, gs, out, to.c, L.out_coff, B, ti.h * ti.w, L.cin, s);
        }
        case FM_OP_HEAD:
            FM_CHECK_ARG(L.cout == ctx->feat_dim && net->emb_offset + B <= ctx->emb_cap);
            return launch_head(in0, ti.c, L.in_coff[0], B, ti.h * ti.w, L.cin, L.cout,
                               (const f16*)(net->weights + L.w_off), (const float*)(net->weights + L.b_off),
                               ctx->emb + (size_t)net->emb_offset * ctx->feat_dim, nullptr, s,
                               ctx->emb_host ? ctx->emb_host + (size_t)net->emb_offset * ctx->feat_dim : nullptr);
        case FM_OP_OSTAIL:
            FM_CHECK_ARG(L.cout == ctx->feat_dim && net->emb_offset + B <= ctx->emb_cap && L.in_coff[0] + L.cin <= ti.c &&
                         ostail_supported(ti.h, ti.w, L.cin, L.hid, L.k, L.cout, L.stride, L.pad));
            return launch_ostail(in0, ti.c, L.in_coff[0], (const f16*)(net->weights + L.w_off),
                                 (const float*)(net->weights + L.b_off), B, ctx->emb + (size_t)net->emb_offset * ctx->feat_dim,
                                 nullptr, ctx->emb_host ? ctx->emb_host + (size_t)net->emb_offset * ctx->feat_dim : nullptr, s);
        default:
            fm_set_error("unknown layer op %d", L.op);
            return FM_ERR_ARG;
    }
}

static int run_layers_eager(fm_ctx* ctx, NetState* net, int batch) {
    for (size_t i = (size_t)net->first; i < net->layers.size(); ++i) {
        int rc = run_layer(ctx, net, net->layers[i], batch);
        if (rc) return rc;
    }
    return 0;
}

bool fm_net_stem_fusable(const NetState* net, int input_tensor) {
    if (!net || net->layers.empty()) return false;
    const fm_layer& L = net->layers[0];
    if ((L.op != FM_OP_STEMCONV && L.op != FM_OP_STEM2) || L.n_in != 1 || L.in[0] != input_tensor || L.in_coff[0] != 0) return false;
    for (size_t i = 1; i < net->layers.size(); ++i) {
        const fm_layer& M = net->layers[i];
        for (int k = 0; k < M.n_in; ++k)
            if (M.in[k] == input_tensor) return false;
        if (M.res_mode != FM_RES_NONE && M.res == input_tensor) return false;
        if (M.out == input_tensor) return false;
    }
    return true;
}

int launch_stem2_layer(const fm_layer& L, const StemSrc& src, const NetState* net, int batch, hipStream_t s) {
    const fm_tensor& ti = net->tensors[L.in[0]];
    const fm_tensor& to = net->tensors[L.out];
    const bool three = L.gate[1] > 0;
    const int cout2 = three ? L.gate[1] : L.cout, act2 = three ? L.gate[2] : L.act;
    FM_CHECK_ARG(!to.f32 && L.hid == 32 && stem2_supported(L.hid, cout2) && L.in_coff[0] == 0 && L.out_coff + L.cout <= to.c);
    FM_CHECK_ARG(!three || stem3_supported(cout2, L.cout));
    const char* w2 = net->weights + L.w2_off;
    const char* b2 = net->weights + L.b2_off;
    return launch_stem2(src, (const f16*)net->bufs[L.in[0]], ti.c, (f16*)net->bufs[L.out], to.c, L.out_coff,
                        (const f16*)(net->weights + L.w_off), (const float*)(net->weights + L.b_off), (const f16*)w2,
                        (const float*)b2, batch, ti.h, ti.w, to.h / 1, to.w / 1, cout2, L.gate[0], act2, s, three ? L.cout : 0,
                        three ? (const f16*)(w2 + (size_t)cout2 * 288 * 2) : nullptr,
                        three ? (const float*)(b2 + (size_t)cout2 * 4) : nullptr, L.act);
}

int fm_net_run_stem_from(fm_ctx* ctx, NetState* net, const StemSrc& src, int batch) {
    FM_CHECK_ARG(ctx && net && !net->layers.empty() && batch >= 1 && batch <= net->max_batch);
    const fm_layer& L = net->layers[0];
    FM_CHECK_ARG(L.op == FM_OP_STEMCONV || L.op == FM_OP_STEM2);
    const fm_tensor& ti = net->tensors[L.in[0]];
    const fm_tensor& to = net->tensors[L.out];
    if (L.op == FM_OP_STEM2) {
        FM_CHECK_ARG(src.kind != 2);
        return launch_stem2_layer(L, src, net, batch, net->stream);
    }
    return launch_stemconv_src(src, (const f16*)net->bufs[L.in[0]], ti.c, 0, (f16*)net->bufs[L.out], to.c, L.out_coff,
                               (const f16*)(net->weights + L.w_off), (const float*)(net->weights + L.b_off), batch, ti.h,
                               ti.w, to.h, to.w, L.k, L.stride, L.pad, L.cout, L.act, net->stream);
}

extern "C" int fm_net_run(fm_ctx* ctx, int which, int batch) {
    FM_CHECK_ARG(ctx && (which >= 0 && which < FM_NET_EXTRACTOR_B + FM_MAX_EXTRA_EXTRACTORS));
    NetState* net = net_slot(ctx, which);
    FM_CHECK_ARG(net != nullptr && batch >= 0 && batch <= net->max_batch);
    if (batch == 0) return 0;
    if (!net->use_graphs || !ctx->opt_use_graphs) return run_layers_eager(ctx, net, batch);
    const long key = (((long)batch << 32) | (unsigned)net->emb_offset) ^ ((long)net->first << 60);
    for (auto& g : net->graphs)
        if (g.first == key) {
            FM_HIP(hipGraphLaunch(g.second, net->stream));
            return 0;
        }
    int rc = run_layers_eager(ctx, net, batch);
    if (rc) return rc;
    FM_HIP(hipStreamSynchronize(net->stream));
    hipGraph_t graph = nullptr;
    hipGraphExec_t exec = nullptr;
    if (hipStreamBeginCapture(net->stream, hipStreamCaptureModeThreadLocal) != hipSuccess) {
        (void)hipGetLastError();
        net->use_graphs = false;
        return 0;
    }
    rc = run_layers_eager(ctx, net, batch);
    const hipError_t ec = hipStreamEndCapture(net->stream, &graph);
    if (rc != 0 || ec != hipSuccess || graph == nullptr ||
        hipGraphInstantiate(&exec, graph, nullptr, nullptr, 0) != hipSuccess) {
        (void)hipGetLastError();
        if (graph) (void)hipGraphDestroy(graph);
        net->use_graphs = false;
        return rc;
    }
    (void)hipGraphDestroy(graph);
    net->graphs.emplace_back(key, exec);
    return 0;
}

extern "C" int fm_net_tensor_write(fm_ctx* ctx, int which, int tensor, const void* host, size_t bytes) {
    FM_CHECK_ARG(ctx && (which >= 0 && which < FM_NET_EXTRACTOR_B + FM_MAX_EXTRA_EXTRACTORS) && host);
    NetState* net = net_slot(ctx, which);
    FM_CHECK_ARG(net && tensor >= 0 && tensor < (int)net->tensors.size());
    const fm_tensor& t = net->tensors[tensor];
    FM_CHECK_ARG(bytes <= (size_t)net->max_batch * t.h * t.w * t.c * elem_size(t));
    FM_HIP(hipStreamSynchronize(net->stream));
    FM_HIP(hipMemcpy(net->bufs[tensor], host, bytes, hipMemcpyHostToDevice));
    return 0;
}

extern "C" int fm_net_tensor_read(fm_ctx* ctx, int which, int tensor, void* host, size_t bytes) {
    FM_CHECK_ARG(ctx && (which >= 0 && which < FM_NET_EXTRACTOR_B + FM_MAX_EXTRA_EXTRACTORS) && host);
    NetState* net = net_slot(ctx, which);
    FM_CHECK_ARG(net && tensor >= 0 && tensor < (int)net->tensors.size());
    const fm_tensor& t = net->tensors[tensor];
    FM_CHECK_ARG(bytes <= (size_t)net->max_batch * t.h * t.w * t.c * elem_size(t));
    FM_HIP(hipStreamSynchronize(net->stream));
    FM_HIP(hipMemcpy(host, net->bufs[tensor], bytes, hipMemcpyDeviceToHost));
    return 0;
}

extern "C" int fm_net_read_embeddings(fm_ctx* ctx, int n, float* host) {
    FM_CHECK_ARG(ctx && n >= 0 && n <= ctx->emb_cap);
    if (n == 0) return 0;
    FM_CHECK_ARG(host);
    FM_HIP(hipStreamSynchronize(ctx->s_ext));
    FM_HIP(hipMemcpy(host, ctx->emb, sizeof(float) * (size_t)n * ctx->feat_dim, hipMemcpyDeviceToHost));
    ctx->emb_n = n;
    return 0;
}

static void layer_cost(const NetState* net, const fm_layer& L, int B, double* flops, double* bytes) {
    const fm_tensor& ti = net->tensors[L.in[0]];
    const fm_tensor& to = net->tensors[L.out];
    const double pin = (double)B * ti.h * ti.w, pout = (double)B * to.h * to.w;
    *flops = 0;
    *bytes = 0;
    switch (L.op) {
        case FM_OP_CONV:
        case FM_OP_CONVS:
        case FM_OP_CONVD:
            *flops = 2.0 * L.k * L.k * L.cin * L.cout * pout;
            *bytes = pin * L.cin * 2 + pout * L.cout * (to.f32 ? 4 : 2) + (double)L.k * L.k * L.cin * L.cout * 2 +
                     (L.res_mode != FM_RES_NONE ? pout * L.cout * 2 : 0);
            break;
        case FM_OP_DWCONV3:
            *flops = 2.0 * 9 * L.cin * pout;
            *bytes = (pin + pout) * L.cin * 2;
            break;
        case FM_OP_LITECONV:
            *flops = 2.0 * (L.cin + 9) * L.cout * pout * L.n_in;
            *bytes = ((pin + pout) * L.cin * 2 + (double)L.cin * L.cout * 2) * L.n_in;
            break;
        case FM_OP_LITECHAIN:
            *flops = 2.0 * (L.cin + 9) * L.cout * pout * 10;
            *bytes = (pin + 4 * pout) * L.cin * 2 + 10.0 * L.cin * L.cout * 2;
            break;
        case FM_OP_GATED_SUM: *bytes = (pin * L.n_in + pout) * L.cin * 2; break;
        case FM_OP_STEMCONV:
            *flops = 2.0 * L.k * L.k * 3 * L.cout * pout;
            *bytes = pin * 8 + pout * L.cout * 2;
            break;
        case FM_OP_PAIR11:
            *flops = 2.0 * L.cin * L.hid * pout + 2.0 * (L.hid + L.cin) * L.cout * pout;
            *bytes = (pin * L.cin + pout * L.hid + (double)L.cin * L.hid) * 2 + (pout * (L.hid + L.cin) + pout * L.cout + (double)(L.hid + L.cin) * L.cout) * 2;
            break;
        case FM_OP_STEM2:
            *flops = 2.0 * 9 * 3 * L.hid * pin + 2.0 * 9 * L.hid * (L.gate[1] > 0 ? L.gate[1] : L.cout) * pout +
                     (L.gate[1] > 0 ? 2.0 * L.gate[1] * L.cout * pout : 0.);
            *bytes = pin * 8 + pout * L.cout * 2 + 9.0 * L.hid * (L.gate[1] > 0 ? L.gate[1] : L.cout) * 2;
            break;
        case FM_OP_RESBLOCK:
            *flops = 2.0 * 10 * L.cin * L.hid * pout;
            *bytes = (pin + pout) * L.cin * 2 + 10.0 * L.cin * L.hid * 2;
            break;
        case FM_OP_SPP: *bytes = (pin + 3 * pout) * L.cin * 2; break;
        case FM_OP_GATE: *bytes = pin * L.cin * 2; break;
        case FM_OP_GATE_SUM: *bytes = (pin * L.n_in + pout) * L.cin * 2; break;
        case FM_OP_OSTAIL: {
            const double px = 128.0 * B, m = L.hid, c = L.k, lite = 10.0 * (m + 9) * m;
            *flops = 2.0 * px * (L.cin * m + lite + (m + L.cin) * c + c * m + lite + m * c + c * c) + 2.0 * c * L.cout * B;
            *bytes = pin * L.cin * 2 + ((double)L.stride) * 2 + (double)B * L.cout * 4;
            break;
        }
        case FM_OP_HEAD:
            *flops = 2.0 * L.cin * L.cout * B;
            *bytes = pin * L.cin * 2 + (double)L.cin * L.cout * 2;
            break;
        default: *bytes = (pin + pout) * L.cin * 2; break;
    }
}

extern "C" int fm_net_cost(fm_ctx* ctx, int which, int batch, double* flops, double* bytes) {
    FM_CHECK_ARG(ctx && (which >= 0 && which < FM_NET_EXTRACTOR_B + FM_MAX_EXTRA_EXTRACTORS) && flops && bytes);
    NetState* net = net_slot(ctx, which);
    FM_CHECK_ARG(net != nullptr);
    double f = 0, b = 0;
    for (const fm_layer& L : net->layers)
        if (L.op == FM_OP_CONV || L.op == FM_OP_CONVS || L.op == FM_OP_CONVD || L.op == FM_OP_RESBLOCK || L.op == FM_OP_PAIR11) {
            double lf, lb;
            layer_cost(net, L, batch, &lf, &lb);
            f += lf;
            b += lb;
        } else if (L.op == FM_OP_STEM2) {
            const fm_tensor& ti = net->tensors[L.in[0]];
            const fm_tensor& to = net->tensors[L.out];
            const double pmid = (double)batch * ti.h * ti.w, pout = (double)batch * to.h * to.w;
            const int c2 = L.gate[1] > 0 ? L.gate[1] : L.cout;
            f += 2.0 * 9 * L.hid * c2 * pout;
            b += pmid * L.hid * 2 + pout * c2 * 2 + 9.0 * L.hid * c2 * 2;
            if (L.gate[1] > 0) {
                f += 2.0 * c2 * L.cout * pout;
                b += pout * c2 * 2 + pout * L.cout * 2 + (double)c2 * L.cout * 2;
            }
        }
    *flops = f;
    *bytes = b;
    return 0;
}

extern "C" int fm_net_profile(fm_ctx* ctx, int which, int batch, int iters, double* conv_ms,
                              double* other_ms, int* n_conv, int* n_other) {
    FM_CHECK_ARG(ctx && (which >= 0 && which < FM_NET_EXTRACTOR_B + FM_MAX_EXTRA_EXTRACTORS) && iters > 0);
    NetState* net = net_slot(ctx, which);
    FM_CHECK_ARG(net != nullptr && batch > 0 && batch <= net->max_batch);
    hipEvent_t e0, e1;
    FM_HIP(hipEventCreate(&e0));
    FM_HIP(hipEventCreate(&e1));
    double tc = 0, to = 0;
    int nc = 0, no = 0;
    for (int it = 0; it < iters; ++it)
        for (const fm_layer& L : net->layers) {
            FM_HIP(hipEventRecord(e0, net->stream));
            int rc = run_layer(ctx, net, L, batch);
            if (rc) return rc;
            FM_HIP(hipEventRecord(e1, net->stream));
            FM_HIP(hipEventSynchronize(e1));
            float ms = 0;
            FM_HIP(hipEventElapsedTime(&ms, e0, e1));
            if (L.op == FM_OP_CONV || L.op == FM_OP_CONVS || L.op == FM_OP_CONVD || L.op == FM_OP_RESBLOCK || L.op == FM_OP_STEM2 || L.op == FM_OP_PAIR11) { tc += ms; ++nc; } else { to += ms; ++no; }
        }
    FM_HIP(hipEventDestroy(e0));
    FM_HIP(hipEventDestroy(e1));
    if (conv_ms) *conv_ms = tc / iters;
    if (other_ms) *other_ms = to / iters;
    if (n_conv) *n_conv = nc / iters;
    if (n_other) *n_other = no / iters;
    return 0;
}

extern "C" int fm_net_profile_layers(fm_ctx* ctx, int which, int batch, int iters, double* out) {
    FM_CHECK_ARG(ctx && (which >= 0 && which < FM_NET_EXTRACTOR_B + FM_MAX_EXTRA_EXTRACTORS) && iters > 0 && out);
    NetState* net = net_slot(ctx, which);
    FM_CHECK_ARG(net != nullptr && batch > 0 && batch <= net->max_batch);
    hipEvent_t e0, e1;
    FM_HIP(hipEventCreate(&e0));
    FM_HIP(hipEventCreate(&e1));
    const size_t n = net->layers.size();
    for (size_t i = 0; i < n; ++i) out[i] = 0;
    for (int it = 0; it < iters; ++it)
        for (size_t i = 0; i < n; ++i) {
            FM_HIP(hipEventRecord(e0, net->stream));
            int rc = run_layer(ctx, net, net->layers[i], batch);
            if (rc) return rc;
            FM_HIP(hipEventRecord(e1, net->stream));
            FM_HIP(hipEventSynchronize(e1));
            float ms = 0;
            FM_HIP(hipEventElapsedTime(&ms, e0, e1));
            out[i] += ms / iters;
        }
    FM_HIP(hipEventDestroy(e0));
    FM_HIP(hipEventDestroy(e1));
    return 0;
}
```

### fastmot_amd/csrc/pixel_source.h

```cpp
#pragma once
#include "net.h"

#define FM_FRAME_SLACK 16
typedef uint64_t fm_u64_unaligned __attribute__((aligned(1)));
__device__ __forceinline__ uint64_t load_px2(const uint8_t* p) { return *reinterpret_cast<const fm_u64_unaligned*>(p); }

__device__ __forceinline__ void det_input_pixel(const uint8_t* __restrict__ frame, int fw, int fh, int x, int y,
                                                int roi_x, int roi_y, int roi_w, int roi_h, float rgb[3]) {
    const int rx0 = x - roi_x, ry0 = y - roi_y;
    const bool in_roi = !(rx0 < 0 || ry0 < 0 || rx0 >= roi_w || ry0 >= roi_h);
    const int rx = min(max(rx0, 0), roi_w - 1), ry = min(max(ry0, 0), roi_h - 1);
    const double zy = (double)fh / roi_h, zx = (double)fw / roi_w;
    const double sy = ry * zy + (zy - 1.) / 2., sx = rx * zx + (zx - 1.) / 2.;
    const double fy = floor(sy), fx = floor(sx);
    const double wy = sy - fy, wx = sx - fx;
    int y0 = (int)fy, x0 = (int)fx, y1 = y0 + 1, x1 = x0 + 1;
    y0 = min(max(y0, 0), fh - 1); y1 = min(max(y1, 0), fh - 1);
    x0 = min(max(x0, 0), fw - 1); x1 = min(max(x1, 0), fw - 1);
    const uint64_t q0 = load_px2(frame + ((size_t)y0 * fw + x0) * 3), q1 = load_px2(frame + ((size_t)y1 * fw + x0) * 3);
    const int sh = x1 == x0 ? 0 : 24;
#pragma unroll
    for (int c = 0; c < 3; ++c) {
        const int p00 = (int)((q0 >> (8 * c)) & 255), p01 = (int)((q0 >> (sh + 8 * c)) & 255);
        const int p10 = (int)((q1 >> (8 * c)) & 255), p11 = (int)((q1 >> (sh + 8 * c)) & 255);
        const double top = (1. - wx) * p00 + wx * p01;
        const double bot = (1. - wx) * p10 + wx * p11;
        const double v = rint((1. - wy) * top + wy * bot);
        const double u8 = fmin(fmax(v, 0.), 255.);
        rgb[2 - c] = in_roi ? (float)(u8 * (1. / 255.)) : 0.5f;
    }
}

struct ResizeCoef { int s; short a0, a1; };

__device__ __forceinline__ ResizeCoef lin_coef(int d, double scale, int ssize) {
    float f = (float)((d + 0.5) * scale - 0.5);
    int s = (int)floorf(f);
    f -= s;
    if (s < 0) { f = 0.f; s = 0; }
    if (s >= ssize - 1) { f = 0.f; s = ssize - 1; }
    ResizeCoef c;
    c.s = s;
    c.a0 = (short)__float2int_rn((1.f - f) * 2048.f);
    c.a1 = (short)__float2int_rn(f * 2048.f);
    return c;
}

__device__ __forceinline__ bool crop_u8_pixel(const uint8_t* __restrict__ frame, int fw, int fh,
                                              const double* __restrict__ bx, int x, int y, int ow, int oh, int bgr[3]) {
    int x1 = max((int)bx[0], 0), y1 = max((int)bx[1], 0);
    int x2 = max((int)bx[2], 0), y2 = max((int)bx[3], 0);
    x2 = min(x2 + 1, fw); y2 = min(y2 + 1, fh);
    const int cw = x2 - x1, ch = y2 - y1;
    if (!(cw > 0 && ch > 0)) return false;
    const ResizeCoef cx = lin_coef(x, (double)cw / ow, cw);
    const ResizeCoef cy = lin_coef(y, (double)ch / oh, ch);
    const int sx1 = min(cx.s + 1, cw - 1), sy1 = min(cy.s + 1, ch - 1);
    const bool area2 = cw == 2 * ow && ch == 2 * oh;
    const int ax = area2 ? 2 * x : cx.s, ay0 = area2 ? 2 * y : cy.s, ay1 = area2 ? 2 * y + 1 : sy1;
    const uint64_t q0 = load_px2(frame + ((size_t)(y1 + ay0) * fw + x1 + ax) * 3);
    const uint64_t q1 = load_px2(frame + ((size_t)(y1 + ay1) * fw + x1 + ax) * 3);
    const int sh = (area2 || sx1 != cx.s) ? 24 : 0;
#pragma unroll
    for (int c = 0; c < 3; ++c) {
        const int a0 = (int)((q0 >> (8 * c)) & 255), a1 = (int)((q0 >> (sh + 8 * c)) & 255);
        const int b0 = (int)((q1 >> (8 * c)) & 255), b1 = (int)((q1 >> (sh + 8 * c)) & 255);
        if (area2) {
            bgr[c] = (a0 + a1 + b0 + b1 + 2) >> 2;
        } else {
            const int S0 = a0 * cx.a0 + a1 * cx.a1;
            const int S1 = b0 * cx.a0 + b1 * cx.a1;
            const int v = (((cy.a0 * (S0 >> 4)) >> 16) + ((cy.a1 * (S1 >> 4)) >> 16) + 2) >> 2;
            bgr[c] = min(max(v, 0), 255);
        }
    }
    return true;
}

__device__ __forceinline__ f16 crop_normalise(int u8, int rc) {
    const double mean[3] = {0.485, 0.456, 0.406}, stdv[3] = {0.229, 0.224, 0.225};
    return (f16)(float)(((double)u8 / 255. - mean[rc]) / stdv[rc]);
}

__device__ __forceinline__ void crop_input_pixel(const uint8_t* __restrict__ frame, int fw, int fh,
                                                 const double* __restrict__ bx, int x, int y, int ow, int oh, f16x8& o) {
#pragma unroll
    for (int e = 0; e < 8; ++e) o[e] = (f16)0.f;
    int bgr[3];
    if (crop_u8_pixel(frame, fw, fh, bx, x, y, ow, oh, bgr)) {
#pragma unroll
        for (int c = 0; c < 3; ++c) o[2 - c] = crop_normalise(bgr[c], 2 - c);
    }
}

struct StemSrc {
    int kind;
    const uint8_t* frame[FM_MAX_DET_BATCH];
    int fw, fh;
    int roi_x, roi_y, roi_w, roi_h;
    const double* boxes;
    int32_t* zero4[FM_MAX_DET_BATCH];
};

template <typename T>
__device__ __forceinline__ T pick_sample(const T (&a)[FM_MAX_DET_BATCH], int i) {
    T r = a[0];
#pragma unroll
    for (int k = 1; k < FM_MAX_DET_BATCH; ++k) r = i == k ? a[k] : r;
    return r;
}

int launch_stemconv_src(const StemSrc& src, const f16* in, int in_cs, int in_coff, f16* out, int out_cs, int out_coff,
                        const f16* w, const float* bias, int N, int H, int W, int Ho, int Wo, int k, int stride, int pad,
                        int cout, int act, hipStream_t s);
int launch_stem2(const StemSrc& src, const f16* in, int in_cs, f16* out, int out_cs, int out_coff, const f16* w1,
                 const float* b1, const f16* w2, const float* b2, int N, int H, int W, int Ho, int Wo, int cout, int act1,
                 int act2, hipStream_t s, int cout3 = 0, const f16* w3 = nullptr, const float* b3 = nullptr, int act3 = 0);
bool stem2_supported(int mid, int cout);
bool stem3_supported(int cout2, int cout3);
int launch_stem2_layer(const fm_layer& L, const StemSrc& src, const NetState* net, int batch, hipStream_t s);
bool fm_net_stem_fusable(const NetState* net, int input_tensor);
int fm_net_run_stem_from(fm_ctx* ctx, NetState* net, const StemSrc& src, int batch);
```

### fastmot_amd/engine.py

```python
import ctypes as C

import numpy as np

from . import _lib

NET_DETECTOR, NET_EXTRACTOR, NET_EXTRACTOR_B = 0, 1, 2


class HipNet:
    def __init__(self, ctx, which, graph, max_batch, reuse_buffers=False):
        self.ctx, self.which, self.graph, self.max_batch = ctx, which, graph, max_batch
        ts, ls, blob = graph.tables(max_batch, reuse_buffers)
        self._keep = (ts, ls, blob)
        _lib.check(ctx.lib.fm_net_create(ctx.handle, C.c_int(which), C.c_int(max_batch), C.c_int(len(ts)), ts,
                                         C.c_int(len(ls)), ls, blob, C.c_size_t(len(blob)),
                                         C.c_int(graph.n_gates), C.c_int(graph.gate_c),
                                         C.c_size_t(graph.arena_bytes)))

    def run(self, batch):
        _lib.check(self.ctx.lib.fm_net_run(self.ctx.handle, C.c_int(self.which), C.c_int(batch)))

    def write(self, view, array):
        h, w, cpad, f32 = self.graph.tensors[view.tid]
        assert view.coff == 0 and not f32
        a = np.asarray(array)
        full = np.zeros((a.shape[0], h, w, cpad), np.float16)
        full[..., :a.shape[-1]] = a
        _lib.check(self.ctx.lib.fm_net_tensor_write(self.ctx.handle, C.c_int(self.which), C.c_int(view.tid),
                                                    full.ctypes.data_as(C.c_void_p), C.c_size_t(full.nbytes)))

    def read(self, view, batch):
        h, w, cpad, f32 = self.graph.tensors[view.tid]
        full = np.empty((batch, h, w, cpad), np.float32 if f32 else np.float16)
        _lib.check(self.ctx.lib.fm_net_tensor_read(self.ctx.handle, C.c_int(self.which), C.c_int(view.tid),
                                                   full.ctypes.data_as(C.c_void_p), C.c_size_t(full.nbytes)))
        return full[..., view.coff:view.coff + view.c].astype(np.float32)

    def read_embeddings(self, n):
        out = np.empty((n, self.ctx.feat_dim), np.float32)
        _lib.check(self.ctx.lib.fm_net_read_embeddings(self.ctx.handle, C.c_int(n), out.ctypes.data_as(C.c_void_p)))
        return out

    def cost(self, batch):
        f, b = C.c_double(0), C.c_double(0)
        _lib.check(self.ctx.lib.fm_net_cost(self.ctx.handle, C.c_int(self.which), C.c_int(batch), C.byref(f), C.byref(b)))
        return f.value, b.value

    def profile(self, batch, iters=3):
        conv_ms, other_ms = C.c_double(0), C.c_double(0)
        n_conv, n_other = C.c_int(0), C.c_int(0)
        _lib.check(self.ctx.lib.fm_net_profile(self.ctx.handle, C.c_int(self.which), C.c_int(batch), C.c_int(iters),
                                               C.byref(conv_ms), C.byref(other_ms), C.byref(n_conv), C.byref(n_other)))
        return dict(conv_ms=conv_ms.value, other_ms=other_ms.value, n_conv=n_conv.value, n_other=n_other.value)

    def profile_layers(self, batch, iters=5):
        out = np.zeros(len(self.graph.layers))
        _lib.check(self.ctx.lib.fm_net_profile_layers(self.ctx.handle, C.c_int(self.which), C.c_int(batch), C.c_int(iters),
                                                      out.ctypes.data_as(C.c_void_p)))
        return out

    def close(self):
        _lib.check(self.ctx.lib.fm_net_destroy(self.ctx.handle, C.c_int(self.which)))
```

### fastmot_amd/models/graph.py

```python
import ctypes as C
import logging
import os

import numpy as np

LOGGER = logging.getLogger(__name__)

(OP_CONV, OP_DWCONV3, OP_MAXPOOL, OP_AVGPOOL, OP_UPSAMPLE2, OP_COPY, OP_GATE, OP_GATE_SUM, OP_HEAD,
 OP_LITECONV, OP_SPP, OP_GATED_SUM, OP_STEMCONV, OP_ADD, OP_RESBLOCK, OP_CONVS, OP_LITECHAIN, OP_CONVD, OP_STEM2, OP_PAIR11,
 OP_OSTAIL) = range(21)
CONV_OPS = (OP_CONV, OP_CONVS, OP_CONVD)
SPP_MAX_HW = 2048
ACT = {'linear': 0, 'leaky': 1, 'mish': 2, 'relu': 3, 'logistic': 4, 'swish': 5}
RES_NONE, RES_AFTER_ACT, RES_BEFORE_ACT = 0, 1, 2


class fm_tensor(C.Structure):
    _fields_ = [('h', C.c_int32), ('w', C.c_int32), ('c', C.c_int32), ('f32', C.c_int32), ('offset', C.c_int64)]


class fm_layer(C.Structure):
    _fields_ = [('op', C.c_int32), ('n_in', C.c_int32),
                ('in_', C.c_int32 * 4), ('in_coff', C.c_int32 * 4),
                ('out', C.c_int32), ('out_coff', C.c_int32),
# ... 260 lines not shown
    def _stem3_applies(self, x, cout, k, stride, pad, res, f32_out, up):
        if not (self.use_stem2 and self.use_stem3 and len(self.layers) == 1 and k == 1 and stride == 1 and pad == 0 and res is None and
                not f32_out and up == 1 and cout in (64, 128)):
            return False
        pair = self.layers[0]
        return (pair['op'] == OP_STEM2 and len(pair['gates']) == 1 and pair['cout'] == 64 and pair['out'].tid == x.tid and
                x.coff == 0 and x.c == 64 and pair['out'].coff == 0 and x.tid not in [v.tid for v in self.outputs])

    def check_fusions(self):
        for li, tid, coff, c in getattr(self, '_pair11_dropped', []):
            for d in self.layers[li + 1:]:
                for v in d['ins'] + ([d['res']] if d['res'] is not None else []):
                    if v.tid == tid and v.coff < coff + c and coff < v.coff + v.c:
                        raise ValueError('a fused 1x1 pair dropped a concat slice that a later layer reads: build with use_pair11 = False')
        t = getattr(self, '_stem2_dropped', None)
        if t is None:
            return
        dropped = t if isinstance(t, list) else [t]
        for d in self.layers:
            used = [v.tid for v in d['ins']] + ([d['res'].tid] if d['res'] is not None else [])
            if any(t in used or t in [v.tid for v in self.outputs] for t in dropped):
                raise ValueError('the stem\'s output is read by another layer: build this network with use_stem2 = False')

    def fuse_ostail(self, first):
        sub = self.layers[first:]
        if not self.use_ostail or len(sub) != 11:
            return False
        pool, c1a, cha, ga, c3a, c1b, chb, gb, c3b, c5, head = sub
        relu = ACT['relu']

        def conv(d, cin, cout, res=False):
            return (d['op'] in CONV_OPS and d['k'] == 1 and d['stride'] == 1 and d['ins'][0].c == cin and d['cout'] == cout and
                    d['act'] == relu and (d['res'] is not None) == res and d['up'] == 1)

        def streams(ch, g, x1):
            return (ch['op'] == OP_LITECHAIN and ch['cout'] == 32 and ch['act'] == relu and ch['ins'][0].tid == x1['out'].tid and
                    g['op'] == OP_GATED_SUM and g['hid'] == 2 and len(g['ins']) == 4 and all(v.tid == ch['out'].tid for v in g['ins']))
        x = pool['ins'][0]
        ok = (pool['op'] == OP_AVGPOOL and (pool['k'], pool['stride'], pool['pad']) == (2, 2, 0) and (x.h, x.w, x.c) == (32, 16, 96) and
              x.coff % 8 == 0 and conv(c1a, 96, 32) and c1a['ins'][0].tid == pool['out'].tid and streams(cha, ga, c1a) and
              conv(c3a, 128, 128) and c3a['ins'][0].tid == pool['out'].tid == ga['out'].tid and
              (ga['out'].coff, pool['out'].coff) == (c3a['ins'][0].coff, c3a['ins'][0].coff + 32) and
              conv(c1b, 128, 32) and c1b['ins'][0].tid == c3a['out'].tid and streams(chb, gb, c1b) and
              conv(c3b, 32, 128, res=True) and c3b['res_mode'] == RES_BEFORE_ACT and c3b['res'].tid == c3a['out'].tid and
              c3b['ins'][0].tid == gb['out'].tid and conv(c5, 128, 128) and c5['ins'][0].tid == c3b['out'].tid and
              head['op'] == OP_HEAD and head['cout'] == 512 and head['ins'][0].tid == c5['out'].tid and
              (head['ins'][0].h, head['ins'][0].w) == (16, 8))
        if not ok:
            return False
        cp = {i: (w, b) for i, w, b in self.conv_params}

        def frag(w):
            w = np.asarray(w, np.float32)
            return self._pack_frag(w.reshape(w.shape[0], -1, 1, 1).astype(np.float16)).reshape(-1)

        def chain(ch):
            refs = ch['lite_ref']
            return (np.concatenate([frag(pw) for pw, _, _ in refs]),
                    np.concatenate([np.asarray(wd, np.float16).reshape(32, 9).T.reshape(-1) for _, wd, _ in refs]),
                    np.concatenate([np.asarray(bd, np.float32) for _, _, bd in refs]))

        def gate(g):
            w1, b1, w2, b2 = (np.asarray(a, np.float32) for a in g['gate_ref'])
            return np.concatenate([w1.reshape(-1), b1, np.zeros(2, np.float32), w2.reshape(-1), b2])
        (w1a, b1a), (w3a, b3a), (w1b, b1b), (w3b, b3b), (w5, b5) = (cp[first + i] for i in (1, 4, 5, 8, 9))
        pwa, dwa, bca = chain(cha)
        pwb, dwb, bcb = chain(chb)
        wfc, bfc = head['head_ref']
        halfs = np.concatenate([frag(w1a), pwa, dwa, frag(w3a), frag(w1b), pwb, dwb, frag(w3b), frag(w5),
                                np.asarray(wfc, np.float16).reshape(-1)])
        floats = np.concatenate([np.asarray(a, np.float32).reshape(-1) for a in
                                 (b1a, bca, gate(ga), b3a, b1b, bcb, gate(gb), b3b, b5, bfc)])
        assert halfs.dtype == np.float16 and floats.dtype == np.float32 and (len(halfs), len(floats)) == (135808, 1928)
        del self.layers[first:]
        self.conv_params = [(i, w, b) for i, w, b in self.conv_params if i < first]
        self._layer(op=OP_OSTAIL, ins=[x], out=View(x.tid, x.coff, x.c, x.h, x.w), cin=96, hid=32, k=128, cout=512, stride=len(halfs), pad=len(floats),
                    w_off=self._push(halfs), b_off=self._push(floats), name='ostail',
                    sub=[(d, cp.get(first + i)) for i, d in enumerate(sub)])
        return True

    @staticmethod
    def resblock_supported(c, mid):
        return c in (64, 128, 256) and mid in (c, c // 2)

    def resblock_pays(self, c, mid, h, w):
        return not (self.convd_level >= 1 and c >= 128 and mid % 64 == 0 and h * w * c >= 1500000)

    @staticmethod
    def _pack_frag(w16):
        cout, cin, k, _ = w16.shape
        K = k * k * cin
        assert cout % 32 == 0 and K % 16 == 0
        rows = w16.transpose(0, 2, 3, 1).reshape(cout // 32, 32, K // 16, 2, 8)
        return np.ascontiguousarray(rows.transpose(0, 2, 3, 1, 4))

    @staticmethod
    def _pack_tile64(wmat):
        cout, K = wmat.shape
        assert cout % 32 == 0 and K % 64 == 0
        rows = wmat.reshape(cout // 32, 32, K // 64, 8, 8).transpose(0, 2, 1, 3, 4)
        r = np.arange(32)[:, None]
        src = np.arange(8)[None, :] ^ ((r >> 1) & 7)
        return np.ascontiguousarray(rows[:, :, r, src, :])

    def resblock(self, name1, name2, x, mid, act='mish', dst=None, wb1=None, wb2=None, bn1=True, bn2=True):
        c = x.c
        assert self.resblock_supported(c, mid) and x.cpad == c
        if dst is None:
            dst = self.new(x.h, x.w, c)
        w1, b1 = wb1 if wb1 is not None else fold_bn(self.wsrc.conv(name1, mid, c, 1, bn=bn1))
        w2, b2 = wb2 if wb2 is not None else fold_bn(self.wsrc.conv(name2, c, mid, 3, bn=bn2))
        w1, b1, w2, b2 = (np.asarray(a, np.float32) for a in (w1, b1, w2, b2))
        w1h, w2h = w1.astype(np.float16), w2.astype(np.float16)
        self._layer(op=OP_RESBLOCK, ins=[x], out=dst, cin=c, cout=c, k=3, stride=1, pad=1, act=ACT[act], hid=mid,
                    w_off=self._push(self._pack_frag(w1h)), b_off=self._push(b1),
                    w2_off=self._push(self._pack_frag(w2h)), b2_off=self._push(b2), name=name2,
                    res_ref=(w1h.astype(np.float32), b1, w2h.astype(np.float32), b2))
        return dst

    def dwconv3(self, name, x, act='relu', dst=None):
        c = x.c
        if dst is None:
            dst = self.new(x.h, x.w, c)
        p = self.wsrc.conv(name, c, c, 3, bn=True, groups=c)
        w, b = fold_bn(p)
        w16 = w.astype(np.float16)
        wk = np.zeros((9, x.cpad), np.float16)
        wk[:, :c] = w16.reshape(c, 9).T
        bias = np.zeros(x.cpad, np.float32)
        bias[:c] = b
        self._layer(op=OP_DWCONV3, ins=[x], out=dst, cin=x.cpad, cout=c, k=3, stride=1, pad=1, act=ACT[act],
                    w_off=self._push(wk), b_off=self._push(bias), name=name)
        self.conv_params.append((len(self.layers) - 1, w16.astype(np.float32), b))
        return dst

    def lightconv_params(self, name, c):
        cp = ceil_to(c, 8)
        pw = self.wsrc.conv(name + '.pw', c, c, 1, bn=False)['w'].astype(np.float16)
        packed = np.zeros((ceil_to(c, 32), ceil_to(cp, 64)), np.float16)
        packed[:c, :c] = pw.reshape(c, c)
        wd, bd = fold_bn(self.wsrc.conv(name + '.dw', c, c, 3, bn=True, groups=c))
        wd16 = wd.astype(np.float16)
        wk = np.zeros((9, cp), np.float16)
        wk[:, :c] = wd16.reshape(c, 9).T
        bias = np.zeros(cp, np.float32)
        bias[:c] = bd
        return dict(pw=packed, dw=wk, bias=bias, ref=(pw.astype(np.float32), wd16.astype(np.float32), bd))

    def lightconv_group(self, name, xs, params, act='relu', dst=None, gap_slot=False):
        G, c = len(xs), xs[0].c
        assert 1 <= G <= 4 and c <= 128 and all(x.c == c and x.coff % 8 == 0 and (x.h, x.w) == (xs[0].h, xs[0].w) for x in xs)
        assert G == 1 or c % 8 == 0
        if dst is None:
            dst = self.new(xs[0].h, xs[0].w, G * c)
        assert dst.c == G * c
        gates = []
        if gap_slot:
            gates = [self.n_gates]
            self.n_gates += 1
            self.gate_c = max(self.gate_c, xs[0].cpad)
        self.last_gap_slot = gates[0] if gates else None
        self._layer(op=OP_LITECONV, ins=list(xs), out=dst, cin=xs[0].cpad, cout=c, k=3, stride=1, pad=1, act=ACT[act],
                    gates=gates,
                    w_off=self._push(np.stack([p['pw'] for p in params])),
                    w2_off=self._push(np.stack([p['dw'] for p in params])),
                    b_off=self._push(np.stack([p['bias'] for p in params])), name=name,
                    lite_ref=[p['ref'] for p in params])
        return dst

    @staticmethod
    def lightchain_fits(c, h, w):
        if c % 8 or not 8 <= c <= 128:
            return False
        nt = (c + 31) // 32
        th, tw = (16, 16 if w > 8 else 8) if nt == 1 else ((8, 16) if w > 8 else (16, 8))
        s = c + (0 if (c >> 3) & 1 else 8)
        ys = max((th + 8) * (tw + 8) * s, (256 // (c // 8)) * c * 2)
        return (ys + (th + 6) * (tw + 6) * s + 4 * 9 * 32 * nt + 4 * 2 * 32 * nt) * 2 <= 64 * 1024

    def lightchain(self, name, x, params, act='relu', dst=None):
        c = x.c
        assert len(params) == 10 and x.coff % 8 == 0 and self.lightchain_fits(c, x.h, x.w)
        if dst is None:
            dst = self.new(x.h, x.w, 4 * c)
        assert dst.c == 4 * c
        gates = list(range(self.n_gates, self.n_gates + 4))
        self.n_gates += 4
        self.gate_c = max(self.gate_c, x.cpad)
        self.last_gap_slots = gates
        self._layer(op=OP_LITECHAIN, ins=[x], out=dst, cin=x.cpad, cout=c, k=3, stride=1, pad=1, act=ACT[act],
                    gates=gates, w_off=self._push(np.stack([p['pw'] for p in params])),
                    w2_off=self._push(np.stack([p['dw'] for p in params])),
                    b_off=self._push(np.stack([p['bias'] for p in params])), name=name,
                    lite_ref=[p['ref'] for p in params])
        return dst

    def lightconv(self, name, x, cout, act='relu', fuse=True):
        if not (fuse and x.c == cout and cout <= 128 and x.coff % 8 == 0):
            y = self.conv(name + '.pw', x, cout, 1, 1, 'linear', bn=False, bias=False)
            return self.dwconv3(name + '.dw', y, act)
        return self.lightconv_group(name, [x], [self.lightconv_params(name, cout)], act)

    def pool(self, x, k, stride, pad, avg=False, dst=None, pad_end=None):
        pad_end = pad if pad_end is None else pad_end
        assert avg is False or pad_end == pad
        ho = (x.h + pad + pad_end - k) // stride + 1
        wo = (x.w + pad + pad_end - k) // stride + 1
        if dst is None:
            dst = self.new(ho, wo, x.c)
        assert dst.h == ho and dst.w == wo
        self._layer(op=OP_AVGPOOL if avg else OP_MAXPOOL, ins=[x], out=dst, cin=x.cpad, cout=x.c, k=k,
                    stride=stride, pad=pad, pad_end=pad_end)
        return dst

    def spp(self, x, dst):
        c = x.c
        assert dst.c == 3 * c and dst.h == x.h and dst.w == x.w and c % 8 == 0
        if x.h * x.w > SPP_MAX_HW:
            for i, k in enumerate((13, 9, 5)):
                self.pool(x, k, 1, k // 2, dst=dst.slice(i * c, c))
            return dst
        self._layer(op=OP_SPP, ins=[x], out=dst, cin=x.cpad, cout=c, k=5, stride=1, pad=2)
        return dst

    def upsample2(self, x, dst=None):
        if dst is None:
            dst = self.new(2 * x.h, 2 * x.w, x.c)
        self._layer(op=OP_UPSAMPLE2, ins=[x], out=dst, cin=x.cpad, cout=x.c)
        return dst

    def add(self, a, b, dst=None):
        assert a.c == b.c and (a.h, a.w) == (b.h, b.w)
        if dst is None:
            dst = self.new(a.h, a.w, a.c)
        self._layer(op=OP_ADD, ins=[a, b], out=dst, cin=a.cpad, cout=a.c)
        return dst

    def copy(self, x, dst):
        self._layer(op=OP_COPY, ins=[x], out=dst, cin=x.cpad, cout=x.c)
        return dst

    def gate(self, name, x, hid, gate_params=None):
        c = x.c
        if gate_params is None:
            p1 = self.wsrc.conv(name + '.fc1', hid, c, 1, bn=False)
            p2 = self.wsrc.conv(name + '.fc2', c, hid, 1, bn=False)
            w1 = np.zeros((hid, x.cpad), np.float16)
            w1[:, :c] = p1['w'].reshape(hid, c).astype(np.float16)
            w2 = np.zeros((x.cpad, hid), np.float16)
            w2[:c] = p2['w'].reshape(c, hid).astype(np.float16)
            b2 = np.zeros(x.cpad, np.float32)
            b2[:c] = p2['bias']
            gate_params = dict(w_off=self._push(w1), b_off=self._push(p1['bias'].astype(np.float32)),
                               w2_off=self._push(w2), b2_off=self._push(b2),
                               ref=(w1[:, :c].astype(np.float32), p1['bias'], w2[:c].astype(np.float32), p2['bias']))
        gid = self.n_gates
        self.n_gates += 1
        self.gate_c = max(self.gate_c, x.cpad)
        self._layer(op=OP_GATE, ins=[x], out=x, cin=x.cpad, cout=c, hid=hid, gates=[gid], name=name,
                    gate_ref=gate_params['ref'],
                    **{k: gate_params[k] for k in ('w_off', 'b_off', 'w2_off', 'b2_off')})
        return gid, gate_params

    def gated_sum(self, name, xs, hid, dst=None, parts=None):
        x = xs[0]
        c = x.c
        assert 1 <= len(xs) <= 4 and all(v.c == c and v.coff % 8 == 0 for v in xs)
        p1 = self.wsrc.conv(name + '.fc1', hid, c, 1, bn=False)
        p2 = self.wsrc.conv(name + '.fc2', c, hid, 1, bn=False)
        w1 = np.zeros((hid, x.cpad), np.float16)
        w1[:, :c] = p1['w'].reshape(hid, c).astype(np.float16)
        w2 = np.zeros((x.cpad, hid), np.float16)
        w2[:c] = p2['w'].reshape(c, hid).astype(np.float16)
        b2 = np.zeros(x.cpad, np.float32)
        b2[:c] = p2['bias']
        if dst is None:
            dst = self.new(x.h, x.w, c)
        assert parts is None or len(parts) == len(xs)
        self._layer(op=OP_GATED_SUM, ins=list(xs), out=dst, cin=x.cpad, cout=c, hid=hid, name=name,
                    gates=list(parts) if parts is not None else [],
                    w_off=self._push(w1), b_off=self._push(p1['bias'].astype(np.float32)),
                    w2_off=self._push(w2), b2_off=self._push(b2),
                    gate_ref=(w1[:, :c].astype(np.float32), p1['bias'], w2[:c].astype(np.float32), p2['bias']))
        return dst

    def gate_sum(self, xs, gids, dst=None):
        x = xs[0]
        if dst is None:
            dst = self.new(x.h, x.w, x.c)
        self._layer(op=OP_GATE_SUM, ins=list(xs), out=dst, cin=x.cpad, cout=x.c, gates=list(gids))
        return dst

    def head(self, name, x, dim):
        p = self.wsrc.linear(name, dim, x.c, bn=True)
        w, b = fold_bn(p)
        w16 = np.zeros((dim, x.cpad), np.float16)
        w16[:, :x.c] = w.astype(np.float16)
        dst = View(x.tid, x.coff, x.c, x.h, x.w)
        self._layer(op=OP_HEAD, ins=[x], out=dst, cin=x.cpad, cout=dim, w_off=self._push(w16),
                    b_off=self._push(b.astype(np.float32)), name=name,
                    head_ref=(w16[:, :x.c].astype(np.float32), b))
        return dst

    def plan_arena(self, max_batch, reuse):
        n = len(self.tensors)
        size = [ceil_to(max_batch * h * w * c * (4 if f32 else 2), 256) for (h, w, c, f32) in self.tensors]
        first, last = [10**9] * n, [-1] * n
        for li, d in enumerate(self.layers):
            touched = [v.tid for v in d['ins']] + [d['out'].tid] + ([d['res'].tid] if d['res'] is not None else [])
            for t in touched:
                first[t], last[t] = min(first[t], li), max(last[t], li)
        persistent = {self.input.tid} | {v.tid for v in self.outputs}
        for t in range(n):
            if t in persistent or not reuse or last[t] < 0:
                first[t], last[t] = -1, 10**9

        def disjoint(t, u):
            if first[t] < 0 or first[u] < 0:
                return False
            return last[t] < first[u] or last[u] < first[t]
        offsets = [0] * n
        placed = []
        for t in sorted(range(n), key=lambda i: -size[i]):
            cands = sorted((o, s) for (o, s, u) in placed if not disjoint(t, u))
            off = 0
            for o, s in cands:
                if off + size[t] <= o:
                    break
                off = max(off, o + s)
            offsets[t] = off
            placed.append((off, size[t], t))
        total = max((o + s for (o, s, _) in placed), default=0)
        return offsets, total

    def tables(self, max_batch=1, reuse=False):
        self.check_fusions()
        offsets, arena = self.plan_arena(max_batch, reuse)
        self.arena_bytes = arena
        ts = (fm_tensor * len(self.tensors))()
        for i, (h, w, c, f32) in enumerate(self.tensors):
            ts[i] = fm_tensor(h, w, c, f32, offsets[i])
        ls = (fm_layer * len(self.layers))()
        for i, d in enumerate(self.layers):
            L = fm_layer()
            L.op = d['op']
            L.n_in = len(d['ins'])
            for j, v in enumerate(d['ins']):
                L.in_[j] = v.tid
                L.in_coff[j] = v.coff
            L.out, L.out_coff = d['out'].tid, d['out'].coff
            if d['res'] is not None:
                L.res, L.res_coff = d['res'].tid, d['res'].coff
            else:
                L.res, L.res_coff = -1, 0
            L.res_mode = d['res_mode']
            for key in ('cin', 'cout', 'k', 'stride', 'pad', 'act', 'hid', 'up', 'w_off', 'b_off', 'w2_off', 'b2_off'):
                setattr(L, key, d[key])
            for j in range(4):
                L.gate[j] = d['gates'][j] if j < len(d['gates']) else -1
            ls[i] = L
        blob = bytes(self.blob) + b'\0' * 64
        return ts, ls, blob

    def conv_flops(self, batch=1):
        total = 0
        for d in self.layers:
            if d['op'] in CONV_OPS + (OP_STEMCONV,):
                o = d['out']
                total += 2 * d['k'] * d['k'] * d['ins'][0].c * d['cout'] * o.h * o.w * batch
            elif d['op'] == OP_RESBLOCK:
                o = d['out']
                total += 2 * 10 * d['cin'] * d['hid'] * o.h * o.w * batch
            elif d['op'] == OP_PAIR11:
                o = d['out']
                total += (2 * d['cin'] * d['hid'] + 2 * (d['hid'] + d['cin']) * d['cout']) * o.h * o.w * batch
            elif d['op'] == OP_STEM2:
                o, i = d['out'], d['ins'][0]
                c2 = d['gates'][1] if len(d['gates']) > 1 else d['cout']
                total += (2 * 9 * i.c * d['hid'] * i.h * i.w + 2 * 9 * d['hid'] * c2 * o.h * o.w) * batch
                if len(d['gates']) > 1:
                    total += 2 * c2 * d['cout'] * o.h * o.w * batch
        return total
```

### include/fastmot_hip.h

```cpp
#ifndef FASTMOT_HIP_H
#define FASTMOT_HIP_H

#include <stddef.h>
#include <stdint.h>

#ifdef __cplusplus
extern "C" {
#endif

typedef struct fm_ctx fm_ctx;

int fm_ctx_create(int device, fm_ctx** out);
int fm_ctx_destroy(fm_ctx* ctx);
const char* fm_last_error(void);
int fm_device_count(void);
int fm_device_pci_bus_id(int device, char* buf, int buflen);
int fm_ctx_synchronize(fm_ctx* ctx);
int fm_ctx_bind_thread(fm_ctx* ctx);
int fm_ctx_set_option(fm_ctx* ctx, const char* key, int value);
int fm_trace_start(fm_ctx* ctx, int cap, int64_t* host_ns);
int fm_trace_read(fm_ctx* ctx, int cap, int32_t* tags, float* ms, int* n);
int fm_device_info(fm_ctx* ctx, char* buf, int buflen);

typedef struct fm_kf_params {
    double dt;
    double std_factor_acc, std_offset_acc;
    double std_factor_det[2], std_factor_klt[2];
    double min_std_det[2], min_std_klt[2];
    double init_pos_weight, init_vel_weight;
    double vel_coupling, vel_half_life;
} fm_kf_params;

int fm_kf_configure(fm_ctx* ctx, const fm_kf_params* p);
int fm_set_frame_rect(fm_ctx* ctx, const double tlbr[4]);

int fm_trk_create(fm_ctx* ctx, int n, const int32_t* slots, const double* det_tlbr);

int fm_trk_step(fm_ctx* ctx, int n, const int32_t* slots, const double* H,
                const double* klt_tlbr, const uint8_t* has_klt, const double* mult,
                double* tlbr_out, uint8_t* lost_out);

enum { FM_KF_WARP = 1, FM_KF_PREDICT = 2, FM_KF_UPDATE_KLT = 4 };
int fm_trk_step_ops(fm_ctx* ctx, int ops, int n, const int32_t* slots, const double* H,
                    const double* klt_tlbr, const uint8_t* has_klt, const double* mult,
                    double* tlbr_out, uint8_t* lost_out);

int fm_trk_update_det(fm_ctx* ctx, int n, const int32_t* slots, const double* det_tlbr,
                      double* tlbr_out, uint8_t* lost_out);

int fm_trk_get_state(fm_ctx* ctx, int n, const int32_t* slots, double* mean, double* cov);
int fm_trk_set_state(fm_ctx* ctx, int n, const int32_t* slots, const double* mean, const double* cov);
int fm_trk_copy_state(fm_ctx* ctx, int dst_slot, int src_slot);

int fm_feat_configure(fm_ctx* ctx, int dim);
int fm_emb_upload(fm_ctx* ctx, int n, const float* emb);
int fm_feat_update(fm_ctx* ctx, int n, const int32_t* slots, const int32_t* emb_rows);
int fm_feat_merge(fm_ctx* ctx, int dst_slot, int src_slot);
int fm_feat_reset(fm_ctx* ctx, int n, const int32_t* slots);
int fm_feat_get(fm_ctx* ctx, int slot, float* sum, float* avg, int32_t* count);
int fm_feat_read(fm_ctx* ctx, int n, const int32_t* slots, float* avg_out, int32_t* count_out);
int fm_feat_write(fm_ctx* ctx, int n, const int32_t* slots, const float* avg, const int32_t* count);

enum { FM_METRIC_EUCLIDEAN = 0, FM_METRIC_COSINE = 1 };

int fm_find_occluded(fm_ctx* ctx, int n, const double* tlbr, double thresh, uint8_t* out);

int fm_assoc_prepare(fm_ctx* ctx, int metric,
                     int nT, const int32_t* slots, const double* trk_tlbr, const int64_t* trk_label,
                     int nD, const double* det_tlbr, const int64_t* det_label,
                     const uint8_t* det_occluded, const uint8_t* trk_feat_f32);

int fm_assoc_get_pairwise(fm_ctx* ctx, double* feat, double* maha, double* iou);

enum {
    FM_STAGE_MATCHING = 0,
    FM_STAGE_IOU      = 1,
    FM_STAGE_REID     = 2
};

int fm_assoc_stage(fm_ctx* ctx, int stage, int solver,
                   int nr, const int32_t* rows, int nc, const int32_t* cols,
                   double motion_weight, double max_cost, double fill_val,
                   const int64_t* row_label_override,
                   int32_t* m_rows, int32_t* m_cols, uint8_t* match_gated, int* n_match,
                   double* cost_out);

int fm_assoc_prepare2(fm_ctx* ctx, int metric,
                      int nT, const int32_t* slots, const double* trk_tlbr, const int64_t* trk_label,
                      int nD, const double* det_tlbr, const int64_t* det_label,
                      const uint8_t* det_occluded, const uint8_t* trk_feat_f32, int after_extractor, int* host_cascade);

#define FM_CASCADE_HEADER 16
typedef struct fm_cascade_in {
    int32_t n_groups;
    int32_t n_unconf, n_hist;
    int32_t reserved;
    const int32_t* group_off;
    const int32_t* conf_rows;
    const uint8_t* conf_active;
    const int32_t* unconf_rows;
    const int32_t* hist_rows;
    const int64_t* hist_labels;
    const double* det_conf;
    double motion_weight, max_assoc_cost, fill_val, max_iou_cost, conf_thresh, max_reid_cost;
} fm_cascade_in;
int fm_assoc_cascade(fm_ctx* ctx, const fm_cascade_in* in, int32_t* out, int out_cap);
int fm_cascade_host(int nT, int nD, const double* feat, const double* maha, const double* iou,
                    const uint8_t* row_has_feat, const int64_t* trk_label, const int64_t* det_label,
                    const uint8_t* det_occluded, const fm_cascade_in* in, int32_t* out, int out_cap);

int fm_lap(fm_ctx* ctx, const double* cost, int nr, int nc,
           int32_t* m_rows, int32_t* m_cols, int* n_match);
int fm_greedy(fm_ctx* ctx, const double* cost, int nr, int nc, double max_cost,
              int32_t* m_rows, int32_t* m_cols, int* n_match);
int fm_iou_dist(fm_ctx* ctx, int na, const double* a, int nb, const double* b, double* out);

enum { FM_NET_DETECTOR = 0, FM_NET_EXTRACTOR = 1,
       FM_NET_EXTRACTOR_B = 2  };
#define FM_MAX_EXTRA_EXTRACTORS 3
enum {
    FM_OP_CONV = 0,
    FM_OP_DWCONV3 = 1,
    FM_OP_MAXPOOL = 2,
    FM_OP_AVGPOOL = 3,
    FM_OP_UPSAMPLE2 = 4,
    FM_OP_COPY = 5,
    FM_OP_GATE = 6,
    FM_OP_GATE_SUM = 7,
    FM_OP_HEAD = 8,
    FM_OP_SPP = 10,
    FM_OP_LITECONV = 9,
    FM_OP_STEMCONV = 12,
    FM_OP_ADD = 13,
    FM_OP_RESBLOCK = 14,
    FM_OP_CONVS = 15,
    FM_OP_LITECHAIN = 16,
    FM_OP_CONVD = 17,
    FM_OP_STEM2 = 18,
    FM_OP_PAIR11 = 19,
    FM_OP_OSTAIL = 20,
    FM_OP_GATED_SUM = 11
};
enum { FM_ACT_LINEAR = 0, FM_ACT_LEAKY = 1, FM_ACT_MISH = 2, FM_ACT_RELU = 3, FM_ACT_LOGISTIC = 4,
       FM_ACT_SWISH = 5 };
enum { FM_RES_NONE = 0, FM_RES_AFTER_ACT = 1, FM_RES_BEFORE_ACT = 2 };

typedef struct fm_tensor {
    int32_t h, w, c;
    int32_t f32;
    int64_t offset;
} fm_tensor;

typedef struct fm_layer {
    int32_t op;
    int32_t n_in;
    int32_t in[4], in_coff[4];
    int32_t out, out_coff;
    int32_t res, res_coff, res_mode;
    int32_t cin, cout, k, stride, pad, act;
    int32_t hid;
    int32_t up;
    int32_t gate[4];
    int64_t w_off, b_off, w2_off, b2_off;
} fm_layer;

int fm_net_create(fm_ctx* ctx, int which, int max_batch, int n_tensors, const fm_tensor* tensors,
                  int n_layers, const fm_layer* layers, const void* weights, size_t weight_bytes,
                  int n_gates, int gate_channels, size_t arena_bytes);
int fm_net_destroy(fm_ctx* ctx, int which);
int fm_net_run(fm_ctx* ctx, int which, int batch);
int fm_net_tensor_write(fm_ctx* ctx, int which, int tensor, const void* host, size_t bytes);
int fm_net_tensor_read(fm_ctx* ctx, int which, int tensor, void* host, size_t bytes);
int fm_net_read_embeddings(fm_ctx* ctx, int n, float* host);
int fm_net_cost(fm_ctx* ctx, int which, int batch, double* flops, double* bytes);
int fm_net_profile(fm_ctx* ctx, int which, int batch, int iters, double* conv_ms, double* other_ms,
                   int* n_conv, int* n_other);

int fm_net_profile_layers(fm_ctx* ctx, int which, int batch, int iters, double* out);

int fm_frame_configure(fm_ctx* ctx, int width, int height, int ring_size);
int fm_frame_upload(fm_ctx* ctx, const uint8_t* bgr);
int fm_host_alloc(size_t bytes, void** out);
int fm_host_free(void* p);
int fm_frame_upload_next(fm_ctx* ctx, const uint8_t* bgr);
int fm_frame_ring_select_next(fm_ctx* ctx, int index);
int fm_frame_promote_next(fm_ctx* ctx);
int fm_detect_async_next(fm_ctx* ctx);
#define FM_MAX_DET_BATCH 4
int fm_frame_upload_ahead(fm_ctx* ctx, int k, const uint8_t* bgr);
int fm_frame_ring_select_ahead(fm_ctx* ctx, int k, int index);
int fm_detect_async_ahead(fm_ctx* ctx, int n);
int fm_frame_ring_store(fm_ctx* ctx, int index, const uint8_t* bgr);
int fm_frame_ring_select(fm_ctx* ctx, int index);
int fm_frame_read(fm_ctx* ctx, uint8_t* bgr);
#define FM_NV12_BT601 0
#define FM_NV12_BT709 1
int fm_frame_upload_nv12(fm_ctx* ctx, const uint8_t* y, const uint8_t* uv, int pitch, int matrix);
int fm_frame_upload_ahead_nv12(fm_ctx* ctx, int k, const uint8_t* y, const uint8_t* uv, int pitch, int matrix);
int fm_frame_ring_store_nv12(fm_ctx* ctx, int index, const uint8_t* y, const uint8_t* uv, int pitch, int matrix);

#define FM_ERR_UNSUPPORTED (-4)
#define FM_JPEG_UNSUPPORTED_PROGRESSIVE 1
#define FM_JPEG_UNSUPPORTED_ARITHMETIC 2
#define FM_JPEG_UNSUPPORTED_PROCESS 3
#define FM_JPEG_UNSUPPORTED_PRECISION 4
#define FM_JPEG_UNSUPPORTED_COMPONENTS 5
#define FM_JPEG_UNSUPPORTED_COLORSPACE 6
#define FM_JPEG_UNSUPPORTED_SAMPLING 7
#define FM_JPEG_UNSUPPORTED_SCANS 8
struct fm_jpeg_info {
    int32_t width, height;
    int32_t ncomp;
    int32_t hsamp[3], vsamp[3];
    int32_t mcu_w, mcu_h;
    int32_t mcus_x, mcus_y;
    int32_t restart_interval;
    int32_t blocks_w[3], blocks_h[3];
    int32_t unsupported;
    int64_t coef_offset[3];
    int64_t coef_count;
};
int fm_jpeg_info(const uint8_t* data, size_t n, struct fm_jpeg_info* out);
int fm_jpeg_entropy_decode(const uint8_t* data, size_t n, const struct fm_jpeg_info* info, int16_t* coef, uint16_t* qt);
int fm_frame_upload_jpeg(fm_ctx* ctx, const struct fm_jpeg_info* info, const int16_t* coef, const uint16_t* qt);
int fm_frame_upload_ahead_jpeg(fm_ctx* ctx, int k, const struct fm_jpeg_info* info, const int16_t* coef, const uint16_t* qt);
int fm_frame_ring_store_jpeg(fm_ctx* ctx, int index, const struct fm_jpeg_info* info, const int16_t* coef, const uint16_t* qt);

#define FM_SRC_BGR 0
#define FM_SRC_NV12 1
#define FM_SRC_JPEG 2
#define FM_SRC_MAX_DIM 16384
struct fm_frame_src {
    int32_t kind, width, height;
    const uint8_t* bgr;
    const uint8_t *y, *uv;
    int32_t pitch, matrix;
    const struct fm_jpeg_info* info;
    const int16_t* coef;
    const uint16_t* qt;
};
int fm_frame_upload_src(fm_ctx* ctx, const struct fm_frame_src* src);
int fm_frame_upload_ahead_src(fm_ctx* ctx, int k, const struct fm_frame_src* src);
int fm_frame_ring_store_src(fm_ctx* ctx, int index, const struct fm_frame_src* src);

#define FM_YUV_420 0
#define FM_YUV_422 1
#define FM_YUV_444 2
#define FM_YUV_MONO 3
struct fm_frame_planar {
    int32_t width, height, chroma, matrix;
    const uint8_t *y, *u, *v;
    int32_t pitch_y, pitch_c;
};
int fm_frame_upload_planar(fm_ctx* ctx, const struct fm_frame_planar* f);
int fm_frame_upload_ahead_planar(fm_ctx* ctx, int k, const struct fm_frame_planar* f);
int fm_frame_ring_store_planar(fm_ctx* ctx, int index, const struct fm_frame_planar* f);

#define FM_PACKED_RGB 0
#define FM_PACKED_BGR 1
#define FM_PACKED_RGBX 2
#define FM_PACKED_BGRX 3
#define FM_PACKED_XRGB 4
#define FM_PACKED_XBGR 5
#define FM_PACKED_YUY2 6
#define FM_PACKED_UYVY 7
#define FM_PACKED_YVYU 8
#define FM_PACKED_BT601 0
#define FM_PACKED_BT709 1
#define FM_PACKED_BT601_FULL 16
#define FM_PACKED_BT709_FULL 17
struct fm_frame_packed {
    int32_t format, width, height, pitch, matrix;
    const uint8_t* data;
};
int fm_frame_upload_packed(fm_ctx* ctx, const struct fm_frame_packed* f);
int fm_frame_upload_ahead_packed(fm_ctx* ctx, int k, const struct fm_frame_packed* f);
int fm_frame_ring_store_packed(fm_ctx* ctx, int index, const struct fm_frame_packed* f);

#define FM_BAYER_RGGB 0
#define FM_BAYER_GRBG 1
#define FM_BAYER_GBRG 2
#define FM_BAYER_BGGR 3
#define FM_BAYER_BILINEAR 0
#define FM_BAYER_MHC 1
struct fm_frame_bayer {
    int32_t pattern, width, height, pitch, depth, method, black, gain_r, gain_g, gain_b;
    const uint8_t* data;
};
int fm_frame_upload_bayer(fm_ctx* ctx, const struct fm_frame_bayer* f);
int fm_frame_upload_ahead_bayer(fm_ctx* ctx, int k, const struct fm_frame_bayer* f);
int fm_frame_ring_store_bayer(fm_ctx* ctx, int index, const struct fm_frame_bayer* f);

int fm_frame_remap_set(fm_ctx* ctx, int src_w, int src_h, const int32_t* xy, const uint8_t border_bgr[3]);
int fm_frame_remap_clear(fm_ctx* ctx);
int fm_remap_bgr_host(const uint8_t* src, int src_w, int src_h, const int32_t* xy, uint8_t* dst, int width, int height,
                      const uint8_t border_bgr[3]);

size_t fm_jpeg_encode_bound(int width, int height);
int fm_jpeg_encode_tables(int quality, uint16_t* qt);
int fm_jpeg_encode_header(int width, int height, int quality, uint8_t* out, size_t capacity, size_t* length);
int fm_jpeg_encode_assemble(int width, int height, int quality, const uint32_t* seg_len, const uint8_t* segs, size_t segs_bytes,
                            uint8_t* out, size_t capacity, size_t* length);
int fm_frame_encode_jpeg(fm_ctx* ctx, int quality, uint8_t* out, size_t capacity, size_t* length);
int fm_jpeg_encode_bgr(fm_ctx* ctx, const uint8_t* pixels, int width, int height, size_t pitch, int quality, uint8_t* out,
                       size_t capacity, size_t* length);
int fm_jpeg_encode_stream_ms(fm_ctx* ctx, float* ms);

#define FM_OVL_RECT_FILL 0
#define FM_OVL_RECT_OUTLINE 1
#define FM_OVL_LINE 2
#define FM_OVL_DOT 3
#define FM_OVL_MASK 4
#define FM_OVERLAY_MAX_CMDS 65536
#define FM_OVERLAY_MAX_MASK_BYTES (4u << 20)
#define FM_OVERLAY_MAX_COORD (1 << 20)
typedef struct fm_overlay_cmd {
    int32_t kind;
    int32_t x0, y0, x1, y1;
    uint8_t b, g, r;
    uint8_t thickness;
    uint32_t mask_off;
    int32_t reserved;
} fm_overlay_cmd;
int fm_overlay_check(const fm_overlay_cmd* cmds, int n, const uint8_t* masks, size_t mask_bytes, int width, int height);
int fm_overlay_render_host(uint8_t* pixels, int width, int height, size_t pitch, const fm_overlay_cmd* cmds, int n,
                           const uint8_t* masks, size_t mask_bytes);
int fm_frame_render_overlay(fm_ctx* ctx, const fm_overlay_cmd* cmds, int n, const uint8_t* masks, size_t mask_bytes);
int fm_overlay_read(fm_ctx* ctx, uint8_t* out);
int fm_overlay_encode_jpeg(fm_ctx* ctx, int quality, uint8_t* out, size_t capacity, size_t* length);
int fm_overlay_stream_ms(fm_ctx* ctx, float* ms);

#define FM_EXPORT_FRAME 0
#define FM_EXPORT_OVERLAY 1
size_t fm_i420_bound(int width, int height);
int fm_frame_export_i420(fm_ctx* ctx, int which, uint8_t* out, size_t capacity, size_t* length);
int fm_i420_from_bgr(fm_ctx* ctx, const uint8_t* pixels, int width, int height, size_t pitch, uint8_t* out, size_t capacity,
                     size_t* length);

#define FM_MAX_HEADS 4
#define FM_MAX_ANCHORS 6
typedef struct fm_det48 {
    double tlbr[4];
    int64_t label;
    double conf;
} fm_det48;

typedef struct fm_yolo_cfg {
    int32_t in_w, in_h;
    int32_t roi_x, roi_y, roi_w, roi_h;
    int32_t input_tensor;
    int32_t n_heads;
    int32_t head_tensor[FM_MAX_HEADS];
    int32_t grid_w[FM_MAX_HEADS], grid_h[FM_MAX_HEADS], n_anchors[FM_MAX_HEADS];
    float anchors[FM_MAX_HEADS][2 * FM_MAX_ANCHORS];
    float scale_xy[FM_MAX_HEADS];
    int32_t num_classes, new_coords;
    uint8_t label_mask[128];
    double conf_thresh, nms_thresh, max_area, min_aspect_ratio;
    double size[2], offset[2];
    int32_t max_candidates;
} fm_yolo_cfg;

int fm_detect_configure(fm_ctx* ctx, const fm_yolo_cfg* cfg);
int fm_detect_async(fm_ctx* ctx);
int fm_detect_sync(fm_ctx* ctx, fm_det48* out, int cap, int* n);
int fm_detect_last_counts(fm_ctx* ctx, int* n_candidates, int* n_detections);
int fm_detect_preprocess_only(fm_ctx* ctx);
int fm_filter_dets(fm_ctx* ctx, const float* rows, int n, fm_det48* out, int cap, int* n_out);
int fm_detect_raw_candidates(fm_ctx* ctx, float* rows, int cap, int* n);
int fm_detect_net_ms(fm_ctx* ctx, float* ms);

int fm_extract_configure(fm_ctx* ctx, int input_tensor, int in_w, int in_h);
int fm_extract_async(fm_ctx* ctx, int n, const double* tlbr);
int fm_extract_sync(fm_ctx* ctx, int n, float* emb);
int fm_extract_read_input(fm_ctx* ctx, int n, float* out);

typedef struct fm_flow_cfg {
    int32_t small_w, small_h;
    int32_t bg_w, bg_h;
    int32_t win_size, max_level, max_count;
    double epsilon;
    int32_t fast_thresh;
    int32_t max_corners, block_size;
    double quality_level;
    int32_t gray_coeff_bits;
} fm_flow_cfg;
int fm_flow_configure(fm_ctx* ctx, const fm_flow_cfg* cfg);
int fm_flow_init(fm_ctx* ctx);
int fm_flow_begin(fm_ctx* ctx);
int fm_flow_targets(fm_ctx* ctx, int nT, const double* inside_tlbr, const float* kps, const int32_t* kp_off,
                    int32_t* area_out, uint8_t* keep_out);
int fm_flow_detect(fm_ctx* ctx, int n, const int32_t* track_idx, const double* track_tlbr,
                   const int32_t* min_dist, int cap, float* pts_out, int32_t* counts_out);
int fm_flow_background(fm_ctx* ctx, int cap, float* pts_out, int* n_out);
int fm_flow_prepare(fm_ctx* ctx, int nT, const double* inside_tlbr, const double* full_tlbr,
                    const float* kps, const int32_t* kp_off, double feat_density, double feat_dist_factor,
                    int32_t* area_out, uint8_t* keep_out, uint8_t* needy_out, int pts_cap,
                    float* new_pts_out, int32_t* new_off_out, int32_t* new_cnt_out, int* n_new_out,
                    int bg_cap, float* bg_pts_out, int* n_bg_out);
int fm_flow_lk(fm_ctx* ctx, int n, const float* prev_pts, float* next_pts, uint8_t* status, float* err);
int fm_flow_swap(fm_ctx* ctx);
int fm_flow_estimate(fm_ctx* ctx, int n_pts, const float* prev_pts, const float* cur_pts,
                     const uint8_t* status, int nT, const int32_t* begins, const int32_t* ends,
                     int bg_begin, int bg_end, const double* track_tlbr, int frame_w, int frame_h,
                     int ransac_max_iter, double ransac_conf, int inlier_thresh,
                     double* H_out, int* ok_out, int32_t* result_out, double* est_tlbr_out,
                     int32_t* n_matched_out, uint8_t* inlier_out);
typedef struct fm_flow_predict_params {
    double feat_density, feat_dist_factor;
    float opt_scale[2], bg_scale[2];
    double max_error;
    int32_t ransac_max_iter;
    double ransac_conf;
    int32_t inlier_thresh;
    int32_t frame_w, frame_h;
} fm_flow_predict_params;
enum { FM_FLOW_OK = 0, FM_FLOW_NO_BACKGROUND = 1, FM_FLOW_NO_HOMOGRAPHY = 2 };
int fm_flow_predict(fm_ctx* ctx, int nT, const double* inside_tlbr, const double* full_tlbr, const float* kps,
                    const int32_t* kp_off, const fm_flow_predict_params* prm, int pts_cap, float* prev_out,
                    float* cur_out, int32_t* trk_off_out, int32_t* bg_range_out, double* H_out, int* status_out,
                    int32_t* result_out, double* est_tlbr_out, int32_t* n_matched_out);
int fm_track_predict_async(fm_ctx* ctx, int nT, const double* inside_tlbr, const double* full_tlbr, const float* kps,
                           const int32_t* kp_off, const fm_flow_predict_params* prm, int pts_cap, float* prev_out,
                           float* cur_out, int32_t* trk_off_out, int32_t* bg_range_out, double* H_out,
                           int32_t* result_out, double* est_tlbr_out, int32_t* n_matched_out, int nK,
                           const int32_t* slots, const int32_t* ages, const int32_t* sorted_idx, double age_penalty,
                           double* tlbr_out, uint8_t* lost_out);
int fm_track_predict_wait(fm_ctx* ctx, int* status_out, int* kalman_done_out);
size_t fm_litechain_lds_bytes(int c, int w, int h);
int fm_resblock_supported(int c, int mid);
int fm_flow_timing(double* out5, int reset);
int fm_flow_read_image(fm_ctx* ctx, int which, uint8_t* out, int* w, int* h);

int fm_gallery_unique_id(char* out128);
int fm_gallery_init(fm_ctx* ctx, int channel, int world, int rank, const char* id128, size_t row_bytes);
int fm_gallery_allgather_async(fm_ctx* ctx, int channel, const void* send_row);
int fm_gallery_allgather_wait(fm_ctx* ctx, int channel, void* recv_rows, float* stream_ms_out);
int fm_gallery_destroy(fm_ctx* ctx, int channel);

#ifdef __cplusplus
}
#endif
#endif
```

Measured before the change: 1024.

## Fuse chains of pointwise convs and pools into single kernels via a layer plan

Builds an execution plan that groups consecutive 1x1 convs, 2x2 avgpools and a stem conv+maxpool+conv into fused steps. Each group runs as one kernel that keeps intermediates in LDS. The detector is excluded, so only the extractor networks use it. The arena planner extends tensor lifetimes across fused runs so buffers cannot alias, at the cost of more arena memory. The aim is fewer kernel launches and less intermediate global-memory traffic, in exchange for added complexity and possible register or LDS pressure in the fused kernels.

After: 987.7. 3.6% lower.

```diff
diff --git a/fastmot_amd/csrc/common.h b/fastmot_amd/csrc/common.h
--- a/fastmot_amd/csrc/common.h
+++ b/fastmot_amd/csrc/common.h
@@ -92,6 +92,7 @@
     int opt_host_lap_elems = 262144;
     int opt_use_graphs = 1;
     int opt_fused_input = 1;
+    int opt_net_plan = 1;
     int opt_net_timing = 0;
     int opt_nms_general = 0;
     int opt_lk_variant = 0;
diff --git a/fastmot_amd/csrc/ctx.hip b/fastmot_amd/csrc/ctx.hip
--- a/fastmot_amd/csrc/ctx.hip
+++ b/fastmot_amd/csrc/ctx.hip
@@ -1,5 +1,6 @@
 #include "common.h"
 void convd_set_cfg(int code);
+void fm_net_plan_changed(fm_ctx* ctx);
 #include <sched.h>
 #include <cstring>
 #include <cstdlib>
@@ -27,6 +28,10 @@
     }
     else if (!strcmp(key, "fused_input")) ctx->opt_fused_input = value != 0;
     else if (!strcmp(key, "net_timing")) ctx->opt_net_timing = value;
+    else if (!strcmp(key, "net_plan")) {
+        if (ctx->opt_net_plan != value) fm_net_plan_changed(ctx);
+        ctx->opt_net_plan = value;
+    }
     else if (!strcmp(key, "lk_variant")) {
 #ifndef FM_DIAG
         if (value != 0) {
@@ -118,6 +123,7 @@
     if (const char* e = getenv("FASTMOT_HOST_LAP")) ctx->opt_host_lap_elems = atoi(e);
     if (const char* e = getenv("FASTMOT_GRAPHS")) ctx->opt_use_graphs = atoi(e);
     if (const char* e = getenv("FASTMOT_FUSED_INPUT")) ctx->opt_fused_input = atoi(e) != 0;
+    if (const char* e = getenv("FASTMOT_NET_PLAN")) ctx->opt_net_plan = atoi(e) < 0 ? 0 : atoi(e);
     int prio_lo = 0, prio_hi = 0;
     FM_HIP(hipDeviceGetStreamPriorityRange(&prio_lo, &prio_hi));
     const int prio_det = prio_lo, prio_ext = prio_hi;
diff --git a/fastmot_amd/csrc/detect.hip b/fastmot_amd/csrc/detect.hip
--- a/fastmot_amd/csrc/detect.hip
+++ b/fastmot_amd/csrc/detect.hip
@@ -1908,9 +1908,10 @@
     if (fused) {
         if (timing) FM_HIP(hipEventRecord(d->ev0[d->wr], s));
         fm_trace_mark(ctx, s, 11);
-        if ((rc = fm_net_run_stem_from(ctx, net, src, n))) return rc;
+        int covered = 1;
+        if ((rc = fm_net_run_stem_from(ctx, net, src, n, &covered))) return rc;
         fm_trace_mark(ctx, s, 15);
-        net->first = 1;
+        net->first = covered;
         rc = fm_net_run_internal(ctx, FM_NET_DETECTOR, n);
         net->first = 0;
         if (rc) return rc;
diff --git a/fastmot_amd/csrc/extract.hip b/fastmot_amd/csrc/extract.hip
--- a/fastmot_amd/csrc/extract.hip
+++ b/fastmot_amd/csrc/extract.hip
@@ -85,9 +85,10 @@
         StemSrc src{};
         src.kind = 2; src.frame[0] = ctx->frame_cur; src.fw = ctx->frame_w; src.fh = ctx->frame_h;
         src.boxes = e->boxes_host + (size_t)off * 4;
-        int rc = fm_net_run_stem_from(ctx, ni, src, b);
-        if (rc) return rc;
-        ni->first = 1;
+        int covered = 1;
+        int rc = fm_net_run_stem_from(ctx, ni, src, b, &covered);
+        if (rc) return rc;
+        ni->first = covered;
         return 0;
     }
     hipLaunchKernelGGL(crop_resize_kernel, dim3((e->in_w + 127) / 128, e->in_h, b), dim3(128), 0, si,
diff --git a/fastmot_amd/csrc/net.h b/fastmot_amd/csrc/net.h
--- a/fastmot_amd/csrc/net.h
+++ b/fastmot_amd/csrc/net.h
@@ -29,11 +29,14 @@
 
 int launch_conv(const ConvParams& p, float* ws, size_t ws_floats, hipStream_t s);
 
+struct PlanStep { int first, count, level; };
+
 struct NetState {
     int which = 0, max_batch = 0;
     std::vector<fm_tensor> tensors;
     std::vector<void*> bufs;
     std::vector<fm_layer> layers;
+    std::vector<PlanStep> plan;
     char* weights = nullptr;
     size_t weight_bytes = 0;
     float* gates = nullptr;
diff --git a/fastmot_amd/csrc/net.hip b/fastmot_amd/csrc/net.hip
--- a/fastmot_amd/csrc/net.hip
+++ b/fastmot_amd/csrc/net.hip
@@ -1,4 +1,5 @@
 #include "pixel_source.h"
+#include "ptrun.h"
 #include <algorithm>
 #include <memory>
 
@@ -77,6 +78,144 @@
     net->graphs.clear();
 }
 
+namespace {
+
+struct ByteRange { long lo, hi; int tensor, c0, c1; };
+
+ByteRange view_range(const fm_tensor* ts, int t, int coff, int c, int max_batch) {
+    ByteRange r{-1, -1, t, coff, coff + c};
+    if (ts[t].offset >= 0) {
+        r.lo = ts[t].offset;
+        r.hi = r.lo + (long)max_batch * ts[t].h * ts[t].w * ts[t].c * (ts[t].f32 ? 4 : 2);
+    }
+    return r;
+}
+bool ranges_clash(const ByteRange& a, const ByteRange& b) {
+    if (a.tensor == b.tensor) return a.c0 < b.c1 && b.c0 < a.c1;
+    return a.lo >= 0 && b.lo >= 0 && a.lo < b.hi && b.lo < a.hi;
+}
+
+bool plan_conv_ok(const fm_tensor* ts, int n_tensors, const fm_layer& L) {
+    if (L.op != FM_OP_CONVD || L.n_in != 1 || L.k != 1 || L.stride != 1 || L.pad != 0 || L.up == 2) return false;
+    const fm_tensor& ti = ts[L.in[0]];
+    const fm_tensor& to = ts[L.out];
+    if (ti.f32 || to.f32 || ti.h != to.h || ti.w != to.w) return false;
+    const int cs = (L.cout + 7) & ~7;
+    if (L.cin <= 0 || L.cin % 8 || L.cout <= 0 || L.cin > PTRUN_MAX_CHANNELS || cs > PTRUN_MAX_CHANNELS) return false;
+    if (((L.cin + 63) >> 6) >= 8) return false;
+    if (L.in_coff[0] % 8 || L.out_coff % 8 || L.in_coff[0] + L.cin > ti.c || L.out_coff + cs > to.c) return false;
+    if (L.res_mode != FM_RES_NONE) {
+        if (L.res < 0 || L.res >= n_tensors) return false;
+        const fm_tensor& tr = ts[L.res];
+        if (tr.f32 || tr.h != to.h || tr.w != to.w || L.res_coff % 8 || L.res_coff + cs > tr.c) return false;
+    }
+    return true;
+}
+
+bool plan_pool_ok(const fm_tensor* ts, const fm_layer& L) {
+    if (L.op != FM_OP_AVGPOOL || L.n_in != 1 || L.k != 2 || L.stride != 2 || L.pad != 0) return false;
+    const fm_tensor& ti = ts[L.in[0]];
+    const fm_tensor& to = ts[L.out];
+    if (ti.f32 || to.f32 || ti.h % 2 || ti.w % 2 || to.h != ti.h / 2 || to.w != ti.w / 2) return false;
+    if (L.cin <= 0 || L.cin % 8 || L.cin > PTRUN_MAX_CHANNELS) return false;
+    return L.in_coff[0] % 8 == 0 && L.out_coff % 8 == 0 && L.in_coff[0] + L.cin <= ti.c && L.out_coff + L.cin <= to.c;
+}
+
+int plan_out_channels(const fm_layer& L) { return L.op == FM_OP_AVGPOOL || L.op == FM_OP_MAXPOOL ? L.cin : (L.cout + 7) & ~7; }
+
+bool plan_stem_run_ok(const fm_tensor* ts, int n_tensors, const fm_layer* ls, int n_layers, int i) {
+    if (i + 3 > n_layers) return false;
+    const fm_layer &S = ls[i], &M = ls[i + 1], &C = ls[i + 2];
+    if (S.op != FM_OP_STEMCONV || S.n_in != 1 || M.op != FM_OP_MAXPOOL || M.n_in != 1 || !plan_conv_ok(ts, n_tensors, C)) return false;
+    const fm_tensor &ti = ts[S.in[0]], &to = ts[S.out], &tp = ts[M.out];
+    const int cs = (S.cout + 7) & ~7;
+    if (ti.f32 || to.f32 || tp.f32 || !stemrun_supported(S.k, S.stride, cs, (C.cout + 7) & ~7)) return false;
+    if (S.pad < 0 || S.pad > S.k / 2 || to.h != (ti.h + 2 * S.pad - S.k) / S.stride + 1 || to.w != (ti.w + 2 * S.pad - S.k) / S.stride + 1) return false;
+    if (S.in_coff[0] % 4 || S.out_coff % 8 || S.out_coff + cs > to.c) return false;
+    if (M.k != 3 || M.stride != 2 || M.pad != 1 || M.in[0] != S.out || M.in_coff[0] != S.out_coff || M.cin != cs) return false;
+    if (tp.h != (to.h - 1) / 2 + 1 || tp.w != (to.w - 1) / 2 + 1 || M.out_coff % 8 || M.out_coff + cs > tp.c) return false;
+    return C.in[0] == M.out && C.in_coff[0] == M.out_coff && C.cin == cs;
+}
+
+int plan_run_length(const fm_tensor* ts, int n_tensors, const fm_layer* ls, int n_layers, int i, int max_batch, int* level) {
+    static const char* const patterns[] = {"SMC", "CCPC", "CPC", "CC"};
+    for (const char* pat : patterns) {
+        const int n = (int)strlen(pat);
+        if (i + n > n_layers) continue;
+        bool ok = pat[0] != 'S' || plan_stem_run_ok(ts, n_tensors, ls, n_layers, i);
+        for (int s = 0; s < n && ok && pat[0] != 'S'; ++s) {
+            const fm_layer& L = ls[i + s];
+            ok = pat[s] == 'C' ? plan_conv_ok(ts, n_tensors, L) : plan_pool_ok(ts, L);
+            if (ok && s > 0) {
+                const fm_layer& P = ls[i + s - 1];
+                ok = L.in[0] == P.out && L.in_coff[0] == P.out_coff && L.cin == plan_out_channels(P);
+            }
+        }
+        if (!ok) continue;
+        std::vector<ByteRange> reads, writes;
+        reads.push_back(view_range(ts, ls[i].in[0], ls[i].in_coff[0], pat[0] == 'S' ? ts[ls[i].in[0]].c : ls[i].cin, max_batch));
+        for (int s = 0; s < n; ++s) {
+            const fm_layer& L = ls[i + s];
+            if (pat[s] == 'C' && L.res_mode != FM_RES_NONE) reads.push_back(view_range(ts, L.res, L.res_coff, plan_out_channels(L), max_batch));
+            writes.push_back(view_range(ts, L.out, L.out_coff, plan_out_channels(L), max_batch));
+        }
+        for (size_t a = 0; a < writes.size() && ok; ++a) {
+            for (const ByteRange& r : reads) ok = ok && !ranges_clash(writes[a], r);
+            for (size_t b = a + 1; b < writes.size(); ++b) ok = ok && !ranges_clash(writes[a], writes[b]);
+        }
+        if (ok) {
+            *level = strcmp(pat, "CC") ? 1 : 2;
+            return n;
+        }
+    }
+    *level = 0;
+    return 1;
+}
+
+std::vector<PlanStep> build_plan(const fm_tensor* ts, int n_tensors, const fm_layer* ls, int n_layers, int which, int max_batch) {
+    std::vector<PlanStep> plan;
+    for (int i = 0; i < n_layers;) {
+        int level = 0;
+        const int n = which == FM_NET_DETECTOR ? 1 : plan_run_length(ts, n_tensors, ls, n_layers, i, max_batch, &level);
+        plan.push_back(PlanStep{i, n, level});
+        i += n;
+    }
+    return plan;
+}
+
+bool plan_tables_valid(int n_tensors, const fm_tensor* ts, int n_layers, const fm_layer* ls) {
+    for (int t = 0; t < n_tensors; ++t)
+        if (ts[t].h <= 0 || ts[t].w <= 0 || ts[t].c <= 0) return false;
+    for (int i = 0; i < n_layers; ++i) {
+        const fm_layer& L = ls[i];
+        if (L.out < 0 || L.out >= n_tensors || L.n_in < 1 || L.n_in > 4) return false;
+        for (int k = 0; k < L.n_in; ++k)
+            if (L.in[k] < 0 || L.in[k] >= n_tensors) return false;
+    }
+    return true;
+}
+
+}
+
+extern "C" int fm_net_plan_describe(int n_tensors, const fm_tensor* tensors, int n_layers, const fm_layer* layers, int which,
+                                    int max_batch, int level, int* out_step_of_layer) {
+    FM_CHECK_ARG(n_tensors > 0 && tensors && n_layers > 0 && layers && which >= 0 && max_batch > 0 && level >= 0 && out_step_of_layer);
+    FM_CHECK_ARG(plan_tables_valid(n_tensors, tensors, n_layers, layers));
+    const std::vector<PlanStep> plan = build_plan(tensors, n_tensors, layers, n_layers, which, max_batch);
+    int n = 0;
+    for (const PlanStep& st : plan) {
+        const bool fused = st.count > 1 && level >= st.level;
+        for (int l = 0; l < st.count; ++l) out_step_of_layer[st.first + l] = fused ? n : n + l;
+        n += fused ? 1 : st.count;
+    }
+    return n;
+}
+
+void fm_net_plan_changed(fm_ctx* ctx) {
+    fm_net_drop_graphs(ctx->ext_net);
+    for (NetState* n : ctx->ext_net_x) fm_net_drop_graphs(n);
+}
+
 static size_t elem_size(const fm_tensor& t) { return t.f32 ? 4 : 2; }
 
 extern "C" int fm_net_destroy(fm_ctx* ctx, int which) {
@@ -145,6 +284,7 @@
         FM_HIP(hipStreamSynchronize(ctx->s_main));
         if ((rc = fm_emb_reserve(ctx, max_batch))) return rc;
     }
+    net->plan = build_plan(net->tensors.data(), n_tensors, net->layers.data(), n_layers, which, max_batch);
     net_slot(ctx, which) = net.release();
     return 0;
 }
@@ -337,10 +477,67 @@
     }
 }
 
+static void fill_conv_stage(const NetState* net, const fm_layer& L, PtStage& st) {
+    st.pool = 0;
+    st.out = (f16*)net->bufs[L.out]; st.out_cs = net->tensors[L.out].c; st.out_coff = L.out_coff;
+    st.cin = L.cin;
+    st.w = (const f16*)(net->weights + L.w_off);
+    st.bias = (const float*)(net->weights + L.b_off);
+    st.cout = L.cout; st.cout_store = (L.cout + 7) & ~7; st.act = L.act; st.res_mode = L.res_mode;
+    if (L.res_mode != FM_RES_NONE) {
+        st.res = (const f16*)net->bufs[L.res]; st.res_cs = net->tensors[L.res].c; st.res_coff = L.res_coff;
+    }
+}
+
+static int run_stem_step(NetState* net, int first, const StemSrc& src, int B) {
+    const fm_layer &S = net->layers[first], &M = net->layers[first + 1], &C = net->layers[first + 2];
+    const fm_tensor &ti = net->tensors[S.in[0]], &to = net->tensors[S.out], &tp = net->tensors[M.out];
+    StemRun r{};
+    r.H = ti.h; r.W = ti.w; r.Ho = to.h; r.Wo = to.w; r.pad = S.pad;
+    r.w = (const f16*)(net->weights + S.w_off); r.bias = (const float*)(net->weights + S.b_off);
+    r.out = (f16*)net->bufs[S.out]; r.out_cs = to.c; r.out_coff = S.out_coff; r.cout_store = (S.cout + 7) & ~7; r.act = S.act;
+    r.pool_out = (f16*)net->bufs[M.out]; r.pool_cs = tp.c; r.pool_coff = M.out_coff; r.Hp = tp.h; r.Wp = tp.w;
+    fill_conv_stage(net, C, r.conv);
+    return launch_stemrun(src, (const f16*)net->bufs[S.in[0]], ti.c, S.in_coff[0], r, B, net->stream);
+}
+
+static int run_fused_step(NetState* net, int first, int count, int B) {
+    const fm_layer& L0 = net->layers[first];
+    const fm_tensor& t0 = net->tensors[L0.in[0]];
+    if (L0.op == FM_OP_STEMCONV) return run_stem_step(net, first, StemSrc{}, B);
+    PtRun r{};
+    r.in = (const f16*)net->bufs[L0.in[0]]; r.in_cs = t0.c; r.in_coff = L0.in_coff[0];
+    r.N = B; r.H = t0.h; r.W = t0.w;
+    r.n_stages = count;
+    int maxc = L0.cin;
+    for (int s = 0; s < count; ++s) {
+        const fm_layer& L = net->layers[first + s];
+        PtStage& st = r.st[s];
+        if (L.op == FM_OP_AVGPOOL) {
+            st.pool = 1;
+            st.out = (f16*)net->bufs[L.out]; st.out_cs = net->tensors[L.out].c; st.out_coff = L.out_coff;
+            st.cin = L.cin;
+        } else {
+            fill_conv_stage(net, L, st);
+            maxc = std::max(maxc, st.cout_store);
+        }
+    }
+    r.lds_stride = maxc + 8;
+    return launch_ptrun(r, net->stream);
+}
+
 static int run_layers_eager(fm_ctx* ctx, NetState* net, int batch) {
-    for (size_t i = (size_t)net->first; i < net->layers.size(); ++i) {
-        int rc = run_layer(ctx, net, net->layers[i], batch);
-        if (rc) return rc;
+    for (const PlanStep& st : net->plan) {
+        if (st.first + st.count <= net->first) continue;
+        if (st.count > 1 && ctx->opt_net_plan >= st.level && st.first >= net->first) {
+            int rc = run_fused_step(net, st.first, st.count, batch);
+            if (rc) return rc;
+            continue;
+        }
+        for (int i = std::max(st.first, net->first); i < st.first + st.count; ++i) {
+            int rc = run_layer(ctx, net, net->layers[i], batch);
+            if (rc) return rc;
+        }
     }
     return 0;
 }
@@ -375,9 +572,14 @@
                         three ? (const float*)(b2 + (size_t)cout2 * 4) : nullptr, L.act);
 }
 
-int fm_net_run_stem_from(fm_ctx* ctx, NetState* net, const StemSrc& src, int batch) {
-    FM_CHECK_ARG(ctx && net && !net->layers.empty() && batch >= 1 && batch <= net->max_batch);
+int fm_net_run_stem_from(fm_ctx* ctx, NetState* net, const StemSrc& src, int batch, int* covered) {
+    FM_CHECK_ARG(ctx && net && !net->layers.empty() && batch >= 1 && batch <= net->max_batch && covered);
     const fm_layer& L = net->layers[0];
+    *covered = 1;
+    if (!net->plan.empty() && net->plan[0].count > 1 && ctx->opt_net_plan >= net->plan[0].level && L.op == FM_OP_STEMCONV) {
+        *covered = net->plan[0].count;
+        return run_stem_step(net, 0, src, batch);
+    }
     FM_CHECK_ARG(L.op == FM_OP_STEMCONV || L.op == FM_OP_STEM2);
     const fm_tensor& ti = net->tensors[L.in[0]];
     const fm_tensor& to = net->tensors[L.out];
diff --git a/fastmot_amd/csrc/pixel_source.h b/fastmot_amd/csrc/pixel_source.h
--- a/fastmot_amd/csrc/pixel_source.h
+++ b/fastmot_amd/csrc/pixel_source.h
@@ -120,4 +120,4 @@
 bool stem3_supported(int cout2, int cout3);
 int launch_stem2_layer(const fm_layer& L, const StemSrc& src, const NetState* net, int batch, hipStream_t s);
 bool fm_net_stem_fusable(const NetState* net, int input_tensor);
-int fm_net_run_stem_from(fm_ctx* ctx, NetState* net, const StemSrc& src, int batch);
+int fm_net_run_stem_from(fm_ctx* ctx, NetState* net, const StemSrc& src, int batch, int* covered);
diff --git a/fastmot_amd/csrc/ptrun.h b/fastmot_amd/csrc/ptrun.h
--- /dev/null
+++ b/fastmot_amd/csrc/ptrun.h
@@ -0,0 +1,129 @@
+#pragma once
+#include "pixel_source.h"
+#include <algorithm>
+
+constexpr int PTRUN_MAX_STAGES = 4;
+constexpr int PTRUN_MAX_CHANNELS = 128;
+
+struct PtStage {
+    int pool;
+    const f16* w;
+    const float* bias;
+    f16* out;       int out_cs, out_coff;
+    const f16* res; int res_cs, res_coff;
+    int cin, cout, cout_store, act, res_mode;
+};
+
+struct PtRun {
+    const f16* in;  int in_cs, in_coff;
+    int N, H, W;
+    int n_stages, lds_stride;
+    PtStage st[PTRUN_MAX_STAGES];
+};
+
+size_t ptrun_lds_bytes(int max_channels);
+int launch_ptrun(const PtRun& r, hipStream_t s);
+
+struct StemRun {
+    int H, W, Ho, Wo, pad;
+    const f16* w;   const float* bias;
+    f16* out;       int out_cs, out_coff, cout_store, act;
+    f16* pool_out;  int pool_cs, pool_coff, Hp, Wp;
+    PtStage conv;
+};
+bool stemrun_supported(int k, int stride, int cout_store, int conv_cout_store);
+int launch_stemrun(const StemSrc& src, const f16* in, int in_cs, int in_coff, const StemRun& r, int N, hipStream_t s);
+
+#if defined(__HIPCC__)
+__device__ __forceinline__ f16x8 ptrun_zero8() {
+    f16x8 z;
+#pragma unroll
+    for (int e = 0; e < 8; ++e) z[e] = (f16)0.f;
+    return z;
+}
+
+template <int NW>
+struct PtRegs {
+    f16x8 w[NW];
+    float4 b[4];
+    f16x4 r[4];
+};
+struct PtTile { int npix, tw, x0, y0, H, W; };
+
+template <int NW>
+__device__ __forceinline__ void ptrun_fetch(const PtStage& st, PtRegs<NW>& g, int item, int npb, const PtTile& t, int n, int lane) {
+    const int frow = lane & 31, fh = lane >> 5;
+    const int ncb = (st.cout + 31) >> 5, nk = (st.cin + 63) >> 6;
+    const int it = min(item, ncb * npb - 1);
+    const int cb = it / npb, pb = it - cb * npb;
+    const char* wimg = reinterpret_cast<const char*>(st.w) + ((size_t)cb * nk * 32 + frow) * 128;
+    const int swz = (frow >> 1) & 7;
+#pragma unroll
+    for (int i = 0; i < NW; ++i) {
+        const int ic = min(i, nk * 4 - 1);
+        const f16x8 v = *reinterpret_cast<const f16x8*>(wimg + (size_t)(ic >> 2) * 4096 + ((((ic & 3) * 2 + fh) ^ swz) << 4));
+        g.w[i] = i * 16 < st.cin ? v : ptrun_zero8();
+    }
+#pragma unroll
+    for (int q = 0; q < 4; ++q) g.b[q] = *reinterpret_cast<const float4*>(st.bias + cb * 32 + 8 * q + 4 * fh);
+    const int l = min(pb * 32 + frow, t.npix - 1);
+    const int y = min(t.y0 + l / t.tw, t.H - 1), x = min(t.x0 + l % t.tw, t.W - 1);
+    const bool has_res = st.res_mode != RES_NONE;
+    const f16* rp = has_res ? st.res + ((size_t)(n * t.H + y) * t.W + x) * st.res_cs + st.res_coff : reinterpret_cast<const f16*>(st.bias);
+#pragma unroll
+    for (int q = 0; q < 4; ++q) g.r[q] = *reinterpret_cast<const f16x4*>(rp + (has_res ? min(cb * 32 + 8 * q + 4 * fh, st.cout_store - 4) : 8 * q + 4 * fh));
+}
+
+template <int NW>
+__device__ __forceinline__ void ptrun_compute(const PtStage& st, const PtRegs<NW>& g, const f16* cur, f16* nxt, int S, int item, int npb,
+                                              const PtTile& t, int n, int lane) {
+    const int frow = lane & 31, fh = lane >> 5;
+    const int ncb = (st.cout + 31) >> 5, nk = (st.cin + 63) >> 6, cin = st.cin;
+    if (item >= ncb * npb) return;
+    const int cb = item / npb, pb = item - cb * npb;
+    const int l = pb * 32 + frow;
+    const bool lvalid = l < t.npix;
+    const f16* brow = cur + (lvalid ? l : 0) * S;
+    f16x8 bf[NW];
+#pragma unroll
+    for (int i = 0; i < NW; ++i) bf[i] = (2 * i + fh) * 8 < cin ? *reinterpret_cast<const f16x8*>(brow + (2 * i + fh) * 8) : ptrun_zero8();
+    f32x16 acc;
+#pragma unroll
+    for (int q = 0; q < 16; ++q) acc[q] = 0.f;
+#pragma unroll
+    for (int i = 0; i < 8; ++i)
+        if (i < nk * 4) {
+            if (i < NW) acc = __builtin_amdgcn_mfma_f32_32x32x16_f16(g.w[i], bf[i], acc, 0, 0, 0);
+            else acc = __builtin_amdgcn_mfma_f32_32x32x16_f16(ptrun_zero8(), ptrun_zero8(), acc, 0, 0, 0);
+        }
+    const int y = t.y0 + l / t.tw, x = t.x0 + l % t.tw;
+    const bool store = lvalid && y < t.H && x < t.W;
+    const size_t gpix = (size_t)(n * t.H + min(y, t.H - 1)) * t.W + min(x, t.W - 1);
+#pragma unroll
+    for (int q = 0; q < 4; ++q) {
+        const int co = cb * 32 + 8 * q + 4 * fh;
+        if (co >= st.cout_store) continue;
+        const float4 bv = g.b[q];
+        float v[4] = {acc[4 * q + 0] + bv.x, acc[4 * q + 1] + bv.y, acc[4 * q + 2] + bv.z, acc[4 * q + 3] + bv.w};
+        float rr[4] = {0.f, 0.f, 0.f, 0.f};
+        if (st.res_mode != RES_NONE) {
+#pragma unroll
+            for (int e = 0; e < 4; ++e) rr[e] = (float)g.r[q][e];
+        }
+        if (st.res_mode == RES_BEFORE_ACT) {
+#pragma unroll
+            for (int e = 0; e < 4; ++e) v[e] += rr[e];
+        }
+        apply_act_n<4>(v, st.act);
+        if (st.res_mode == RES_AFTER_ACT) {
+#pragma unroll
+            for (int e = 0; e < 4; ++e) v[e] += rr[e];
+        }
+        f16x4 o;
+#pragma unroll
+        for (int e = 0; e < 4; ++e) o[e] = (f16)v[e];
+        if (lvalid && nxt) *reinterpret_cast<f16x4*>(nxt + l * S + co) = o;
+        if (store) *reinterpret_cast<f16x4*>(st.out + gpix * st.out_cs + st.out_coff + co) = o;
+    }
+}
+#endif
diff --git a/fastmot_amd/csrc/ptrun.hip b/fastmot_amd/csrc/ptrun.hip
--- /dev/null
+++ b/fastmot_amd/csrc/ptrun.hip
@@ -0,0 +1,130 @@
+#include "ptrun.h"
+
+namespace {
+
+constexpr int TW = 8, TH = 4, TP = TW * TH;
+constexpr int WAVES = 2;
+
+template <int NW>
+__global__ __launch_bounds__(128, 3) void ptrun_kernel(const PtRun r) {
+    extern __shared__ __attribute__((aligned(16))) f16 lds[];
+    const int S = r.lds_stride;
+    const int lane = threadIdx.x & 63, wave = __builtin_amdgcn_readfirstlane(threadIdx.x >> 6);
+    f16* cur = lds + wave * (2 * TP * S);
+    f16* nxt = cur + TP * S;
+    const int n = blockIdx.y;
+    const int tiles_x = (r.W + TW - 1) / TW, tiles = tiles_x * ((r.H + TH - 1) / TH);
+    const int wt = (int)blockIdx.x * WAVES + wave;
+    if (wt >= tiles) return;
+    const int ty = wt / tiles_x, tx = wt - ty * tiles_x;
+    PtTile t{TP, TW, tx * TW, ty * TH, r.H, r.W};
+
+    PtRegs<NW> ahead;
+    int a_si = 0, a_cb = 0;
+    ptrun_fetch(r.st[0], ahead, 0, 1, t, n, lane);
+    const int c8n = r.st[0].cin >> 3;
+    for (int e0 = 0; e0 < TP * c8n; e0 += 4 * 64) {
+        f16x8 v[4];
+#pragma unroll
+        for (int i = 0; i < 4; ++i) {
+            const int e = min(e0 + i * 64 + lane, TP * c8n - 1), l = e / c8n, c8 = (e - l * c8n) * 8;
+            const int y = min(t.y0 + l / TW, r.H - 1), x = min(t.x0 + l % TW, r.W - 1);
+            v[i] = *reinterpret_cast<const f16x8*>(r.in + ((size_t)(n * r.H + y) * r.W + x) * r.in_cs + r.in_coff + c8);
+        }
+#pragma unroll
+        for (int i = 0; i < 4; ++i) {
+            const int e = min(e0 + i * 64 + lane, TP * c8n - 1), l = e / c8n, c8 = (e - l * c8n) * 8;
+            *reinterpret_cast<f16x8*>(cur + l * S + c8) = v[i];
+        }
+    }
+    __builtin_amdgcn_wave_barrier();
+
+    for (int si = 0; si < r.n_stages; ++si) {
+        const PtStage& st = r.st[si];
+        if (st.pool) {
+            const PtTile h{t.npix / 4, t.tw / 2, t.x0 / 2, t.y0 / 2, t.H / 2, t.W / 2};
+            const int pc8n = st.cin >> 3;
+            for (int e = lane; e < h.npix * pc8n; e += 64) {
+                const int l = e / pc8n, c8 = (e - l * pc8n) * 8;
+                const int py = l / h.tw, px = l - py * h.tw;
+                float acc[8];
+#pragma unroll
+                for (int k = 0; k < 8; ++k) acc[k] = 0.f;
+#pragma unroll
+                for (int dy = 0; dy < 2; ++dy)
+#pragma unroll
+                    for (int dx = 0; dx < 2; ++dx) {
+                        float v[8];
+                        unpack8(*reinterpret_cast<const uint4*>(cur + ((2 * py + dy) * t.tw + 2 * px + dx) * S + c8), v);
+#pragma unroll
+                        for (int k = 0; k < 8; ++k) acc[k] = acc[k] + v[k];
+                    }
+                const float inv = 1.f / (float)4;
+#pragma unroll
+                for (int k = 0; k < 8; ++k) acc[k] *= inv;
+                const uint4 o = pack8(acc);
+                *reinterpret_cast<uint4*>(nxt + l * S + c8) = o;
+                const int y = h.y0 + py, x = h.x0 + px;
+                if (y < h.H && x < h.W)
+                    *reinterpret_cast<uint4*>(st.out + ((size_t)(n * h.H + y) * h.W + x) * st.out_cs + st.out_coff + c8) = o;
+            }
+            t = h;
+        } else {
+            const int ncb = (st.cout + 31) >> 5;
+            for (int cb = 0; cb < ncb; ++cb) {
+                const PtRegs<NW> now = ahead;
+                a_cb = cb + 1; a_si = si;
+                PtTile at = t;
+                if (a_cb == ncb) {
+                    a_cb = 0; a_si = si + 1;
+                    if (a_si < r.n_stages && r.st[a_si].pool) {
+                        at = PtTile{t.npix / 4, t.tw / 2, t.x0 / 2, t.y0 / 2, t.H / 2, t.W / 2};
+                        ++a_si;
+                    }
+                }
+                if (a_si >= r.n_stages) { a_si = si; a_cb = cb; at = t; }
+                ptrun_fetch(r.st[a_si], ahead, a_cb, 1, at, n, lane);
+                ptrun_compute(st, now, cur, si + 1 < r.n_stages ? nxt : nullptr, S, cb, 1, t, n, lane);
+            }
+        }
+        __builtin_amdgcn_wave_barrier();
+        f16* sw = cur; cur = nxt; nxt = sw;
+    }
+}
+
+template <int NW>
+int launch_nw(const PtRun& r, size_t lds, hipStream_t s) {
+    const int tiles = ((r.W + TW - 1) / TW) * ((r.H + TH - 1) / TH);
+    const dim3 grid((unsigned)((tiles + WAVES - 1) / WAVES), (unsigned)r.N), block(64 * WAVES);
+    hipLaunchKernelGGL((ptrun_kernel<NW>), grid, block, lds, s, r);
+    FM_HIP(hipGetLastError());
+    return 0;
+}
+
+}
+
+size_t ptrun_lds_bytes(int max_channels) { return (size_t)WAVES * 2 * TP * (max_channels + 8) * sizeof(f16); }
+
+int launch_ptrun(const PtRun& r, hipStream_t s) {
+    FM_CHECK_ARG(r.n_stages >= 2 && r.n_stages <= PTRUN_MAX_STAGES && r.N >= 1 && r.N <= 65535 && r.H > 0 && r.W > 0);
+    FM_CHECK_ARG(r.in && r.in_cs % 8 == 0 && r.in_coff % 8 == 0 && !r.st[0].pool && !r.st[r.n_stages - 1].pool);
+    int maxc = 0, maxcin = 0, h = r.H, w = r.W, c = r.st[0].cin, pools = 0;
+    for (int i = 0; i < r.n_stages; ++i) {
+        const PtStage& st = r.st[i];
+        FM_CHECK_ARG(st.out && st.out_cs % 8 == 0 && st.out_coff % 8 == 0 && st.cin == c && st.cin % 8 == 0 && st.cin > 0);
+        maxc = std::max(maxc, st.cin);
+        if (st.pool) {
+            FM_CHECK_ARG(h % 2 == 0 && w % 2 == 0 && ++pools == 1 && st.out_coff + st.cin <= st.out_cs);
+            h /= 2; w /= 2;
+        } else {
+            FM_CHECK_ARG(st.w && st.bias && st.cout > 0 && st.cout_store == ((st.cout + 7) & ~7) && st.out_coff + st.cout_store <= st.out_cs);
+            FM_CHECK_ARG(st.res_mode == RES_NONE || (st.res && st.res_cs % 8 == 0 && st.res_coff % 8 == 0 && st.res_coff + st.cout_store <= st.res_cs));
+            c = st.cout_store;
+            maxc = std::max(maxc, c);
+            maxcin = std::max(maxcin, st.cin);
+        }
+    }
+    FM_CHECK_ARG(maxc <= PTRUN_MAX_CHANNELS && r.lds_stride == maxc + 8);
+    const size_t lds = ptrun_lds_bytes(maxc);
+    return maxcin <= 64 ? launch_nw<4>(r, lds, s) : launch_nw<8>(r, lds, s);
+}
diff --git a/fastmot_amd/csrc/stemrun.hip b/fastmot_amd/csrc/stemrun.hip
--- /dev/null
+++ b/fastmot_amd/csrc/stemrun.hip
@@ -0,0 +1,178 @@
+#include "ptrun.h"
+
+namespace {
+
+typedef float f32x16 __attribute__((ext_vector_type(16)));
+
+constexpr int KS = 7, STRIDE = 2, TAPS = KS * KS, KP = (TAPS * 4 + 15) / 16 * 16, NKS = KP / 16;
+constexpr int SO = 17, NSO = SO * SO;
+constexpr int PW = (SO - 1) * STRIDE + KS;
+constexpr int MAXC = 16, SS = MAXC + 8;
+constexpr int NT = (NSO + 31) / 32;
+
+template <int SRC>
+__global__ __launch_bounds__(256, 3) void stem_run_kernel(const StemSrc src, const f16* __restrict__ in, int in_cs, int in_coff,
+                                                       const StemRun r) {
+    __shared__ __attribute__((aligned(16))) uint2 patch[PW * PW];
+    __shared__ __attribute__((aligned(16))) f16 sout[NSO * SS];
+    __shared__ __attribute__((aligned(16))) f16 pooled[64 * SS];
+    __shared__ f16 norm_lut[SRC == 2 ? 3 * 256 : 2];
+    const int tid = threadIdx.x, lane = tid & 63, wave = __builtin_amdgcn_readfirstlane(tid >> 6);
+    const int ox0 = blockIdx.x * 16, oy0 = blockIdx.y * 16;
+    const int n = blockIdx.z;
+    const int H = r.H, W = r.W, Ho = r.Ho, Wo = r.Wo;
+    const uint8_t* frame1 = SRC == 1 ? pick_sample(src.frame, n) : nullptr;
+    const f16* img = in + (long)n * H * W * in_cs + in_coff;
+    if (SRC == 1 && tid < 4 && blockIdx.x == 0 && blockIdx.y == 0) {
+        int32_t* z = pick_sample(src.zero4, n);
+        if (z) z[tid] = 0;
+    }
+    if constexpr (SRC == 2) {
+#pragma unroll
+        for (int i = 0; i < 3; ++i) norm_lut[i * 256 + tid] = crop_normalise(tid, i);
+        __syncthreads();
+    }
+    const int frow = lane & 31, fh = lane >> 5;
+    f16x8 afr[NKS];
+#pragma unroll
+    for (int ks = 0; ks < NKS; ++ks)
+        afr[ks] = *reinterpret_cast<const f16x8*>(r.w + (long)frow * KP + ks * 16 + fh * 8);
+    float4 sbias[4];
+#pragma unroll
+    for (int g = 0; g < 4; ++g) sbias[g] = *reinterpret_cast<const float4*>(r.bias + 8 * g + 4 * fh);
+    const int py0 = oy0 >> 1, px0 = ox0 >> 1;
+    const PtTile ptile{64, 8, px0, py0, r.Hp, r.Wp};
+    PtRegs<1> cregs;
+    ptrun_fetch(r.conv, cregs, wave, 2, ptile, n, lane);
+    constexpr int NIT = (PW * PW + 255) / 256;
+#pragma unroll
+    for (int it = 0; it < NIT; ++it) {
+        const int i = tid + it * 256, ic = min(i, PW * PW - 1);
+        const int iy = (oy0 - 1) * STRIDE - r.pad + ic / PW, ix = (ox0 - 1) * STRIDE - r.pad + ic % PW;
+        const bool inside = iy >= 0 && iy < H && ix >= 0 && ix < W;
+        const int cy = min(max(iy, 0), H - 1), cx = min(max(ix, 0), W - 1);
+        uint2 v;
+        if constexpr (SRC == 0) {
+            v = *reinterpret_cast<const uint2*>(img + ((long)cy * W + cx) * in_cs);
+        } else if constexpr (SRC == 1) {
+            float rgb[3];
+            det_input_pixel(frame1, src.fw, src.fh, cx, cy, src.roi_x, src.roi_y, src.roi_w, src.roi_h, rgb);
+            union { f16 h[4]; uint2 u; } pk;
+            pk.h[0] = (f16)rgb[0]; pk.h[1] = (f16)rgb[1]; pk.h[2] = (f16)rgb[2]; pk.h[3] = (f16)0.f;
+            v = pk.u;
+        } else {
+            int bgr[3];
+            union { f16 h[4]; uint2 u; } pk;
+            pk.u = make_uint2(0u, 0u);
+            if (crop_u8_pixel(src.frame[0], src.fw, src.fh, src.boxes + (long)n * 4, cx, cy, W, H, bgr)) {
+                pk.h[0] = norm_lut[0 * 256 + bgr[2]]; pk.h[1] = norm_lut[1 * 256 + bgr[1]]; pk.h[2] = norm_lut[2 * 256 + bgr[0]];
+            }
+            v = pk.u;
+        }
+        if (!inside) v = make_uint2(0u, 0u);
+        if (i < PW * PW) patch[i] = v;
+    }
+    __syncthreads();
+
+    for (int t = wave; t < NT; t += 4) {
+        const int sp = t * 32 + frow, spc = min(sp, NSO - 1);
+        const int sy = spc / SO, sx = spc - sy * SO;
+        const int base = (sy * STRIDE) * PW + sx * STRIDE;
+        f32x16 acc;
+#pragma unroll
+        for (int q = 0; q < 16; ++q) acc[q] = 0.f;
+#pragma unroll
+        for (int ks = 0; ks < NKS; ++ks) {
+            const int ta0 = 4 * ks, ta1 = 4 * ks + 2;
+            const int t0 = fh ? ta1 : ta0;
+            const int tA = t0 < TAPS ? t0 : TAPS - 1, tB = t0 + 1 < TAPS ? t0 + 1 : TAPS - 1;
+            const uint2 a = patch[base + (tA / KS) * PW + tA % KS];
+            const uint2 b = patch[base + (tB / KS) * PW + tB % KS];
+            uint4 v = make_uint4(a.x, a.y, b.x, b.y);
+            acc = __builtin_amdgcn_mfma_f32_32x32x16_f16(afr[ks], *reinterpret_cast<f16x8*>(&v), acc, 0, 0, 0);
+        }
+        const int oy = oy0 - 1 + sy, ox = ox0 - 1 + sx;
+        const bool own = sp < NSO && sy >= 1 && sx >= 1 && oy < Ho && ox < Wo;
+        f16* dst = r.out + (((long)n * Ho + max(oy, 0)) * Wo + max(ox, 0)) * r.out_cs + r.out_coff;
+#pragma unroll
+        for (int g = 0; g < 4; ++g) {
+            const int co = 8 * g + 4 * fh;
+            if (co < r.cout_store) {
+                const float4 bv = sbias[g];
+                f16x4 o;
+                float a4[4] = {acc[4 * g + 0] + bv.x, acc[4 * g + 1] + bv.y, acc[4 * g + 2] + bv.z, acc[4 * g + 3] + bv.w};
+                apply_act_n<4>(a4, r.act);
+#pragma unroll
+                for (int e = 0; e < 4; ++e) o[e] = (f16)a4[e];
+                if (sp < NSO) *reinterpret_cast<f16x4*>(sout + sp * SS + co) = o;
+                if (own) *reinterpret_cast<f16x4*>(dst + co) = o;
+            }
+        }
+    }
+    __syncthreads();
+
+    {
+        const int c8n = r.cout_store >> 3;
+        for (int e = tid; e < 64 * c8n; e += 256) {
+            const int l = e / c8n, c8 = (e - l * c8n) * 8;
+            const int ly = l >> 3, lx = l & 7;
+            float acc8[8];
+#pragma unroll
+            for (int k = 0; k < 8; ++k) acc8[k] = -65504.f;
+#pragma unroll
+            for (int dy = 0; dy < 3; ++dy) {
+                const int oy = oy0 - 1 + 2 * ly + dy;
+                if (oy < 0 || oy >= Ho) continue;
+#pragma unroll
+                for (int dx = 0; dx < 3; ++dx) {
+                    const int ox = ox0 - 1 + 2 * lx + dx;
+                    if (ox < 0 || ox >= Wo) continue;
+                    float v[8];
+                    unpack8(*reinterpret_cast<const uint4*>(sout + ((2 * ly + dy) * SO + 2 * lx + dx) * SS + c8), v);
+#pragma unroll
+                    for (int k = 0; k < 8; ++k) acc8[k] = fmaxf(acc8[k], v[k]);
+                }
+            }
+            const uint4 o = pack8(acc8);
+            *reinterpret_cast<uint4*>(pooled + l * SS + c8) = o;
+            const int py = py0 + ly, px = px0 + lx;
+            if (py < r.Hp && px < r.Wp)
+                *reinterpret_cast<uint4*>(r.pool_out + (((long)n * r.Hp + py) * r.Wp + px) * r.pool_cs + r.pool_coff + c8) = o;
+        }
+    }
+    __syncthreads();
+
+    ptrun_compute(r.conv, cregs, pooled, nullptr, SS, wave, 2, ptile, n, lane);
+}
+
+template <int SRC>
+int launch_kind(const StemSrc& src, const f16* in, int in_cs, int in_coff, const StemRun& r, int N, hipStream_t s) {
+    const dim3 grid((r.Wo + 15) / 16, (r.Ho + 15) / 16, N), block(256);
+    hipLaunchKernelGGL((stem_run_kernel<SRC>), grid, block, 0, s, src, in, in_cs, in_coff, r);
+    FM_HIP(hipGetLastError());
+    return 0;
+}
+
+}
+
+bool stemrun_supported(int k, int stride, int cout_store, int conv_cout_store) {
+    return k == KS && stride == STRIDE && cout_store >= 8 && cout_store <= MAXC && conv_cout_store >= 8 && conv_cout_store <= 64;
+}
+
+int launch_stemrun(const StemSrc& src, const f16* in, int in_cs, int in_coff, const StemRun& r, int N, hipStream_t s) {
+    FM_CHECK_ARG(N >= 1 && N <= 65535 && in_cs % 4 == 0 && in_coff % 4 == 0 && r.out && r.out_cs % 4 == 0 && r.out_coff % 4 == 0);
+    FM_CHECK_ARG(stemrun_supported(KS, STRIDE, r.cout_store, r.conv.cout_store) && r.cout_store % 8 == 0 && r.out_coff + r.cout_store <= r.out_cs);
+    FM_CHECK_ARG(r.Ho == (r.H + 2 * r.pad - KS) / STRIDE + 1 && r.Wo == (r.W + 2 * r.pad - KS) / STRIDE + 1 && r.pad >= 0 && r.pad <= KS / 2);
+    FM_CHECK_ARG(r.Hp == (r.Ho - 1) / 2 + 1 && r.Wp == (r.Wo - 1) / 2 + 1);
+    FM_CHECK_ARG(r.pool_out && r.pool_cs % 8 == 0 && r.pool_coff % 8 == 0 && r.pool_coff + r.cout_store <= r.pool_cs);
+    const PtStage& c = r.conv;
+    FM_CHECK_ARG(!c.pool && c.w && c.bias && c.out && c.cin == r.cout_store && c.cout > 0 && c.cout_store == ((c.cout + 7) & ~7) &&
+                 c.out_cs % 8 == 0 && c.out_coff % 8 == 0 && c.out_coff + c.cout_store <= c.out_cs);
+    FM_CHECK_ARG(c.res_mode == RES_NONE || (c.res && c.res_cs % 8 == 0 && c.res_coff % 8 == 0 && c.res_coff + c.cout_store <= c.res_cs));
+    FM_CHECK_ARG(src.kind == 0 || (src.frame[0] && src.fw > 0 && src.fh > 0 && (src.kind == 1 || (src.kind == 2 && src.boxes))));
+    FM_CHECK_ARG(src.kind != 1 || N <= FM_MAX_DET_BATCH);
+    for (int i = 0; src.kind == 1 && i < N; ++i) FM_CHECK_ARG(src.frame[i] != nullptr);
+    if (src.kind == 1) return launch_kind<1>(src, in, in_cs, in_coff, r, N, s);
+    if (src.kind == 2) return launch_kind<2>(src, in, in_cs, in_coff, r, N, s);
+    return launch_kind<0>(src, in, in_cs, in_coff, r, N, s);
+}
diff --git a/fastmot_amd/engine.py b/fastmot_amd/engine.py
--- a/fastmot_amd/engine.py
+++ b/fastmot_amd/engine.py
@@ -7,10 +7,26 @@
 NET_DETECTOR, NET_EXTRACTOR, NET_EXTRACTOR_B = 0, 1, 2
 
 
+PLAN_DEFAULT, PLAN_ALL = 1, 2
+
+
+def plan_steps(graph, which, max_batch=1, reuse_buffers=False, runs=(), level=PLAN_DEFAULT):
+    ts, ls, _ = graph.tables(max_batch, reuse_buffers, runs)
+    step_of = (C.c_int * len(ls))()
+    n = _lib.load().fm_net_plan_describe(C.c_int(len(ts)), ts, C.c_int(len(ls)), ls, C.c_int(which), C.c_int(max_batch), C.c_int(level), step_of)
+    if n <= 0:
+        raise _lib.FastMOTHipError(f'fm_net_plan_describe: {_lib.load().fm_last_error().decode()}')
+    steps = [[] for _ in range(n)]
+    for layer, s in enumerate(step_of):
+        steps[s].append(layer)
+    return steps
+
+
 class HipNet:
     def __init__(self, ctx, which, graph, max_batch, reuse_buffers=False):
         self.ctx, self.which, self.graph, self.max_batch = ctx, which, graph, max_batch
-        ts, ls, blob = graph.tables(max_batch, reuse_buffers)
+        runs = [s for s in plan_steps(graph, which, max_batch, level=PLAN_ALL) if len(s) > 1] if reuse_buffers and which != NET_DETECTOR else []
+        ts, ls, blob = graph.tables(max_batch, reuse_buffers, runs)
         self._keep = (ts, ls, blob)
         _lib.check(ctx.lib.fm_net_create(ctx.handle, C.c_int(which), C.c_int(max_batch), C.c_int(len(ts)), ts,
                                          C.c_int(len(ls)), ls, blob, C.c_size_t(len(blob)),
diff --git a/fastmot_amd/models/graph.py b/fastmot_amd/models/graph.py
--- a/fastmot_amd/models/graph.py
+++ b/fastmot_amd/models/graph.py
@@ -586,7 +586,7 @@
                     head_ref=(w16[:, :x.c].astype(np.float32), b))
         return dst
 
-    def plan_arena(self, max_batch, reuse):
+    def plan_arena(self, max_batch, reuse, runs=()):
         n = len(self.tensors)
         size = [ceil_to(max_batch * h * w * c * (4 if f32 else 2), 256) for (h, w, c, f32) in self.tensors]
         first, last = [10**9] * n, [-1] * n
@@ -594,6 +594,11 @@
             touched = [v.tid for v in d['ins']] + [d['out'].tid] + ([d['res'].tid] if d['res'] is not None else [])
             for t in touched:
                 first[t], last[t] = min(first[t], li), max(last[t], li)
+        for run in runs:
+            for li in run:
+                d = self.layers[li]
+                for t in [v.tid for v in d['ins']] + [d['out'].tid] + ([d['res'].tid] if d['res'] is not None else []):
+                    first[t], last[t] = min(first[t], min(run)), max(last[t], max(run))
         persistent = {self.input.tid} | {v.tid for v in self.outputs}
         for t in range(n):
             if t in persistent or not reuse or last[t] < 0:
@@ -617,9 +622,9 @@
         total = max((o + s for (o, s, _) in placed), default=0)
         return offsets, total
 
-    def tables(self, max_batch=1, reuse=False):
+    def tables(self, max_batch=1, reuse=False, runs=()):
         self.check_fusions()
-        offsets, arena = self.plan_arena(max_batch, reuse)
+        offsets, arena = self.plan_arena(max_batch, reuse, runs)
         self.arena_bytes = arena
         ts = (fm_tensor * len(self.tensors))()
         for i, (h, w, c, f32) in enumerate(self.tensors):
diff --git a/include/fastmot_hip.h b/include/fastmot_hip.h
--- a/include/fastmot_hip.h
+++ b/include/fastmot_hip.h
@@ -177,6 +177,8 @@
                    int* n_conv, int* n_other);
 
 int fm_net_profile_layers(fm_ctx* ctx, int which, int batch, int iters, double* out);
+int fm_net_plan_describe(int n_tensors, const fm_tensor* tensors, int n_layers, const fm_layer* layers, int which,
+                         int max_batch, int level, int* out_step_of_layer);
 
 int fm_frame_configure(fm_ctx* ctx, int width, int height, int ring_size);
 int fm_frame_upload(fm_ctx* ctx, const uint8_t* bgr);
```
